# Lakonik/MVEdit

Hardware: AMD Instinct MI355X
Metric: multi-view denoise-steps/sec (32 views, 512^2) (higher is better)
Workload: dtype f16; 1 GPU; 32-view 512x512 get_noise_pred: 64 SD-1.5 UNet forwards (64x64 latents, ctx 77x768) + CFG per step; ControlNet residuals zero; views=32, latent=64, cfg=True, parallelism=views/1

## Files before the change

include/mvedit_amd.h:

```cpp
#ifndef MVEDIT_AMD_H
#define MVEDIT_AMD_H

#include <stdint.h>
#include <stddef.h>

#ifdef __cplusplus
extern "C" {
#endif

#define MVE_API __attribute__((visibility("default")))

typedef enum {
    MVE_OK = 0,
    MVE_ERR_ARG = -1,
    MVE_ERR_HIP = -2,
    MVE_ERR_STATE = -3,
    MVE_ERR_NOMEM = -4
} mve_status;

typedef enum {
    MVE_F32 = 0,
    MVE_F16 = 1,
    MVE_BF16 = 2,
    MVE_I32 = 3,
// ... 238 lines not shown
                             const void* d_ctx, int B, int H, int W, int ctx_len, int num_cross_attn_imgs,
                             const void* const* down_residuals, const void* d_mid_residual, int residuals_nhwc,
                             void* d_out, void* d_workspace, size_t workspace_bytes, float* op_ms, void* stream);
MVE_API int mve_controlnet_create(void** handle, int dtype, int in_channels, int conditioning_channels, int n_levels,
                                  const int* block_out_channels, int layers_per_block, const int* down_attn, const int* num_heads,
                                  const int* transformer_layers, int cross_attention_dim, int norm_num_groups, float norm_eps,
                                  int use_linear_projection);
MVE_API int mve_controlnet_set_cond_repeat(void* handle, int repeat);
MVE_API int mve_controlnet_forward(void* handle, const void* d_sample, int io_dtype, const float* d_timesteps, const void* d_ctx,
                                   const void* d_cond, int B, int H, int W, int ctx_len, float conditioning_scale, int accumulate,
                                   void* const* d_outputs, void* d_workspace, size_t workspace_bytes,
                                   float* op_ms , void* stream);

MVE_API int mve_vae_create(void** handle, int dtype, int half, int in_channels, int out_channels, int n_levels,
                           const int* block_out_channels, int layers_per_block, int norm_num_groups, float norm_eps);
MVE_API int mve_vae_plan(void* handle, int B, int H, int W, int io_dtype, size_t* workspace_bytes, int* n_ops, double* flops);
MVE_API int mve_vae_forward(void* handle, const void* d_in, int io_dtype, int B, int H, int W, void* d_out, void* d_workspace,
                            size_t workspace_bytes, float* op_ms, void* stream);

MVE_API int mve_srvgg_create(void** handle, int dtype, int num_in_ch, int num_out_ch, int num_feat, int num_conv, int upscale);
MVE_API int mve_srvgg_plan(void* handle, int B, int H, int W, int io_dtype, size_t* workspace_bytes, int* n_ops, double* flops);
MVE_API int mve_srvgg_forward(void* handle, const void* d_in, int io_dtype, int B, int H, int W, void* d_out, void* d_workspace,
                              size_t workspace_bytes, float* op_ms, void* stream);
MVE_API int mve_lpips_create(void** handle, int dtype, int normalize_inputs);
MVE_API int mve_lpips_plan(void* handle, int B, int H, int W, int io_dtype, size_t* workspace_bytes, int* n_ops, int* n_forward_ops,
                           double* flops);
MVE_API int mve_lpips_forward(void* handle, const void* d_pred, const void* d_target, int io_dtype, int B, int H, int W, float* d_loss,
                              void* d_workspace, size_t workspace_bytes, void* stream);
MVE_API int mve_lpips_backward(void* handle, const float* d_grad_loss, int io_dtype, int B, int H, int W, void* d_grad_pred,
                               void* d_workspace, size_t workspace_bytes, void* stream);
MVE_API int mve_lpips_scale(int dtype, int io_dtype, const void* d_pred, const void* d_target, int B, int H, int W, const float* d_shift3,
                            const float* d_scale3, int normalize, void* d_out, void* stream);
MVE_API int mve_lpips_input_grad(int dtype, int io_dtype, const void* d_g8, int B, int H, int W, const float* d_scale3, int normalize,
                                 void* d_out, void* stream);
MVE_API int mve_maxpool2x2(int dtype, const void* d_x, int B, int H, int W, int C, void* d_y, void* stream);
MVE_API int mve_maxpool2x2_backward(int dtype, const void* d_x, const void* d_grad_y, int B, int H, int W, int C, void* d_grad_x,
                                    void* stream);
MVE_API int mve_relu_backward(int dtype, void* d_grad, const void* d_out, size_t n, void* stream);
MVE_API size_t mve_lpips_layer_scratch_bytes(int B, int HW);
MVE_API int mve_lpips_layer(int dtype, const void* d_feat, const float* d_lin_w, int B, int HW, int C, int accumulate, float* d_loss,
                            void* d_scratch, void* stream);
MVE_API int mve_lpips_layer_backward(int dtype, const void* d_feat, const float* d_lin_w, const float* d_grad_loss, int B, int HW, int C,
                                     void* d_grad_feat, void* stream);
MVE_API int mve_prelu(int dtype, const void* d_x, const float* d_slope, int C, void* d_y, size_t n, void* stream);
MVE_API int mve_pixel_shuffle_add(int io_dtype, const float* d_src, int ld, const void* d_base, int B, int C, int H, int W, int r,
                                  void* d_out, void* stream);

MVE_API int mve_unet_tune(int fuse_shortcut);
MVE_API int mve_unet_graph(void* handle, int enable);

MVE_API int mve_unet_set_attention(void* handle, int ip_tokens, float ip_scale, int ref_mode, int ref_H, int ref_W, int ref_skip,
                                   void* d_ref_store, size_t ref_store_bytes);
MVE_API int mve_unet_set_residual_mode(void* handle, int pair);
MVE_API int mve_unet_set_addition_embed(void* handle, int addition_type, int addition_time_embed_dim, int projection_input_dim);
MVE_API int mve_unet_bind_added_cond(void* handle, const void* d_text_embeds, int text_dtype, int text_dim, const float* d_time_ids, int n_ids,
                                     int B);
MVE_API size_t mve_unet_ref_store_bytes(void* handle, int B, int ref_H, int ref_W, int ref_skip);

MVE_API int mve_unet_op_info(void* handle, int i, int* cls, double* flops, char* label, int label_len);


MVE_API int mve_hashgrid_mlp_decode(const float* d_xyz, uint32_t M, const float* d_table, int n_levels,
                                    const float* level_scale, const uint32_t* level_res, const uint32_t* level_offset,
                                    const uint32_t* level_size, const float* d_w1, const float* d_b1, const float* d_w2,
                                    const float* d_b2, int hidden, float bound, float blob_density, float blob_radius,
                                    float sigmoid_saturation, float* d_sigmas, float* d_rgbs, void* stream);

MVE_API size_t mve_hashgrid_mlp_backward_workspace_bytes(uint32_t M, int n_levels);
MVE_API int mve_hashgrid_mlp_backward(const float* d_xyz, uint32_t M, const float* d_table, int n_levels, const float* level_scale,
                                      const uint32_t* level_res, const uint32_t* level_offset, const uint32_t* level_size,
                                      const float* d_w1, const float* d_b1, const float* d_w2, const float* d_b2, int hidden, float bound,
                                      float blob_density, float blob_radius, float sigmoid_saturation, const float* d_grad_sigma,
                                      const float* d_grad_rgb, float* d_grad_table, float* d_grad_w1, float* d_grad_b1,
                                      float* d_grad_w2, float* d_grad_b2, void* d_workspace, size_t workspace_bytes, void* stream);
MVE_API int mve_adam_step(float* d_param, const float* d_grad, float* d_exp_avg, float* d_exp_avg_sq, size_t n, float lr, float beta1,
                          float beta2, float eps, int step, void* stream);

MVE_API int mve_nerf_render_rays(const float* d_rays_o, const float* d_rays_d, uint32_t N, const uint8_t* d_bitfield,
                                 uint32_t grid_size, const float* d_aabb, float bound, float min_near, float dt_gamma,
                                 uint32_t max_steps, float T_thresh, const float* d_table, int n_levels,
                                 const float* level_scale, const uint32_t* level_res, const uint32_t* level_offset,
                                 const uint32_t* level_size, const float* d_w1, const float* d_b1, const float* d_w2,
                                 const float* d_b2, int hidden, float blob_density, float blob_radius,
                                 float sigmoid_saturation, float* d_weights_sum, float* d_depth, float* d_image,
                                 int32_t* d_n_samples, void* stream);

MVE_API int mve_camera_rays(const float* d_intrinsics, const float* d_poses, int n_views, int h, int w, float* d_rays_o,
                            float* d_rays_d, float* d_dir_norm, void* stream);

MVE_API int mve_depth_to_normal(const float* d_depth, const float* d_alpha, int alpha_stride, const float* d_intrinsics,
                                int n_views, int h, int w, const float* normal_bg3, float* d_normal_fg, float* d_normal,
                                void* stream);

MVE_API int mve_normalize_depth(const float* d_depths, const float* d_alphas, int n_views, int hw, float far_depth,
                                float alpha_clip, float eps, float* d_out, void* stream);

#define MVE_INTERP_LINEAR 0
#define MVE_INTERP_SMOOTHSTEP 1
MVE_API int mve_hashgrid_encode(const float* d_x, uint32_t N, const float* d_table, uint32_t n_rows, int n_features, int n_levels,
                                const float* level_scale, const uint32_t* level_res, const uint32_t* level_offset,
                                const uint32_t* level_size, int interpolation, float* d_out, void* stream);
MVE_API int mve_hashgrid_encode_backward(const float* d_x, uint32_t N, const float* d_table, uint32_t n_rows, int n_features,
                                         int n_levels, const float* level_scale, const uint32_t* level_res,
                                         const uint32_t* level_offset, const uint32_t* level_size, int interpolation,
                                         const float* d_grad_enc, float* d_grad_table, float* d_grad_x, void* stream);

// ... 146 lines not shown
```

mvedit_amd/csrc/attention.hip:

```cpp
#include "common.h"

#include <stdlib.h>
#include <type_traits>

namespace {

constexpr int NT = 256;

struct AttnParams {
    const void* Q; const void* K; const void* V; const void* K2; const void* V2; void* O;
    int ldq, ldk, ldv, ldk2, ldv2, ldo;
    int B, Lq, Lk, Lk2, heads;
    float scale_log2e;
    int prescaled;
};

template <int DP, bool KSW2> __device__ __forceinline__ int k_perm(int row, int pc) {
    if constexpr (DP == 64) return pc ^ ((row >> 1) & 7);
    else if constexpr (KSW2) return pc ^ (((row >> 3) & 1) << 1);
    else return pc ^ ((row >> 2) & 3);
}
template <int DP, bool KSW2> __device__ __forceinline__ int k_swz(int row, int chunk) {
    return row * (DP * 2) + (k_perm<DP, KSW2>(row, chunk) << 4);
}

typedef __attribute__((address_space(3))) void* lds_ptr_t;
typedef const __attribute__((address_space(1))) void* gbl_ptr_t;
typedef float f32x8 __attribute__((ext_vector_type(8)));

__device__ __attribute__((aligned(16))) unsigned int g_attn_zero_page[4] = {0u, 0u, 0u, 0u};

template <int KB2, bool VSW2> __device__ __forceinline__ int v_swz2(int row, int chunk) {
    if constexpr (KB2 == 128) return row * 256 + ((chunk ^ (row & 15) ^ (VSW2 ? (row >> 3) & 7 : 0)) << 4);
    else return row * 128 + ((chunk ^ ((row >> 1) & 7) ^ (VSW2 ? (row >> 4) & 7 : 0)) << 4);
}

template <class Tag, int D, bool SEG2, int QF = 2, int KB2X = 0, int OCC = 0, bool KSW2 = false, bool VSW2 = false>
__global__ __launch_bounds__(NT, (OCC ? OCC : (D > 80 ? 1 : 2))) void k_attention2(const AttnParams p) {
    constexpr int QB = 64 * QF;
    constexpr int DP = (D + 31) / 32 * 32;
    constexpr int KS = DP / 32;
    constexpr int DC = D / 8;
    constexpr int DVF = (D + 15) / 16;
    constexpr int KB2 = KB2X ? KB2X : (D > 64 ? 64 : 128);
    constexpr int NH = KB2 / 64;
    constexpr int CPR = DP / 8;
    constexpr int KROW = DP * 2;
    constexpr int VROW = KB2 * 2;
    constexpr int K_BYTES = KB2 * KROW;
    constexpr int V_BYTES = DVF * 16 * VROW;
    constexpr int K_INSTR = K_BYTES / 1024 / 4;
    static_assert((K_BYTES / 1024) % 4 == 0, "K tile must split evenly over 4 waves");
    constexpr int V_TASKS = (KB2 / 2) * DC;
    constexpr int V_PER_T = (V_TASKS + NT - 1) / NT;
    constexpr bool ONES = (D % 16) != 0;
    constexpr int L_G = (D % 16) / 4, L_R = (D % 16) % 4;
    typedef typename Tag::V8 V8;
    typedef typename Tag::T T;

    __shared__ __attribute__((aligned(16))) unsigned char smem[2 * K_BYTES + 2 * V_BYTES];
    unsigned char* Kbuf = smem;
    unsigned char* Vbuf = smem + 2 * K_BYTES;

    const int tid = threadIdx.x, lane = tid & 63, wid = tid >> 6;
    const int g = lane >> 4, l16 = lane & 15;

    const int q_tiles = (p.Lq + QB - 1) / QB;
    const unsigned nblk = (unsigned)(q_tiles * p.heads * p.B);
    const unsigned bid = mve_xcd_remap(blockIdx.x, nblk);
    const int qt = bid % q_tiles;
    const int h = (bid / q_tiles) % p.heads;
    const int b = bid / (q_tiles * p.heads);
    const int Ltot = p.Lk + p.Lk2;

    const T* Qp = reinterpret_cast<const T*>(p.Q);
    const T* zero = reinterpret_cast<const T*>(g_attn_zero_page);
    const T* kb1 = reinterpret_cast<const T*>(p.K) + (size_t)b * p.Lk * p.ldk + h * D;
    const T* vb1 = reinterpret_cast<const T*>(p.V) + (size_t)b * p.Lk * p.ldv + h * D;
    const T* kb2 = SEG2 ? reinterpret_cast<const T*>(p.K2) + (size_t)b * p.Lk2 * p.ldk2 + h * D : nullptr;
    const T* vb2 = SEG2 ? reinterpret_cast<const T*>(p.V2) + (size_t)b * p.Lk2 * p.ldv2 + h * D : nullptr;
    auto k_row = [&](int j) -> const T* {
        if constexpr (SEG2) { if (j >= p.Lk) return kb2 + (size_t)(j - p.Lk) * p.ldk2; }
        return kb1 + (size_t)j * p.ldk;
    };
    auto v_row = [&](int j) -> const T* {
        if constexpr (SEG2) { if (j >= p.Lk) return vb2 + (size_t)(j - p.Lk) * p.ldv2; }
        return vb1 + (size_t)j * p.ldv;
    };

    for (int i = tid; i < 2 * V_BYTES / 16; i += NT) reinterpret_cast<u32x4*>(Vbuf)[i] = u32x4{0u, 0u, 0u, 0u};
    __syncthreads();
    if constexpr (ONES) {
        const unsigned short one = __builtin_bit_cast(unsigned short, Tag::from_f32(1.0f));
        const unsigned two = (unsigned)one | ((unsigned)one << 16);
        for (int i = tid; i < 2 * (VROW / 4); i += NT) {
            const int buf = i / (VROW / 4), wofs = i - buf * (VROW / 4);
            *reinterpret_cast<unsigned*>(Vbuf + buf * V_BYTES + D * VROW + wofs * 4) = two;
        }
    }

    V8 qf[QF][KS];
    const int q_base = qt * QB + wid * (16 * QF);
#pragma unroll
    for (int f = 0; f < QF; ++f) {
        int q = q_base + f * 16 + l16;
        q = q < p.Lq ? q : p.Lq - 1;
        const T* row = Qp + ((size_t)b * p.Lq + q) * p.ldq + h * D;
#pragma unroll
        for (int ks = 0; ks < KS; ++ks) {
            const int c = ks * 4 + g;
            u32x4 v = {0u, 0u, 0u, 0u};
            if (c < DC) v = *reinterpret_cast<const u32x4*>(row + c * 8);
            qf[f][ks] = __builtin_bit_cast(V8, v);
        }
    }

    int kd_row[K_INSTR], kd_col[K_INSTR];
#pragma unroll
    for (int i = 0; i < K_INSTR; ++i) {
        const int pos = (wid * K_INSTR + i) * 64 + lane;
        const int row = pos / CPR, pc = pos - row * CPR;
        const int c = k_perm<DP, KSW2>(row, pc);
        kd_row[i] = row;
        kd_col[i] = c < DC ? c * 8 : -1;
    }
// ... 202 lines not shown
        if (q < p.Lq) {
            T* orow = reinterpret_cast<T*>(p.O) + ((size_t)b * p.Lq + q) * p.ldo + h * D;
#pragma unroll
            for (int i = 0; i < DVF; ++i) {
                const int dv = i * 16 + g * 4;
                if (dv < D) {
                    T4 pk;
#pragma unroll
                    for (int r = 0; r < 4; ++r) pk[r] = Tag::from_f32(oacc[i][f][r] * inv);
                    *reinterpret_cast<T4*>(orow + dv) = pk;
                }
            }
        }
    }
}

__device__ __attribute__((aligned(16))) unsigned short g_attn_ones_f16[8] = {0x3C00u, 0, 0, 0, 0, 0, 0, 0};
__device__ __attribute__((aligned(16))) unsigned short g_attn_ones_bf16[8] = {0x3F80u, 0, 0, 0, 0, 0, 0, 0};

__device__ unsigned long long g_attn_prof[4] = {0ull, 0ull, 0ull, 0ull};

typedef short s16x4 __attribute__((ext_vector_type(4)));
typedef short s16x8 __attribute__((ext_vector_type(8)));
typedef float f32x2 __attribute__((ext_vector_type(2)));

__device__ __forceinline__ void attn_dma16(const void* gsrc, unsigned lds_dst) {
    unsigned keep;
    asm volatile("s_mov_b32 %0, m0\n\ts_mov_b32 m0, %2\n\ts_nop 0\n\tglobal_load_lds_dwordx4 %1, off\n\ts_mov_b32 m0, %0"
                 : "=&s"(keep) : "v"(gsrc), "s"(lds_dst) : "memory");
}

template <class Tag, bool SEG2, int NW, int NST, int WPS, bool PRE, bool PIPE, int ABL = 0>
__global__ __launch_bounds__(64 * NW, WPS) void k_attention3(const AttnParams p) {
    constexpr int D = 40, KB = 64, QB = 32 * NW;
    constexpr int K_ROW = 80, V_ROW = 96;
    constexpr int K_BYTES = KB * K_ROW, V_BYTES = KB * V_ROW, STAGE = K_BYTES + V_BYTES;
    constexpr int N_DMA = STAGE / 1024, K_DMA = K_BYTES / 1024, DMA_PER_WAVE = (N_DMA + NW - 1) / NW;
    static_assert(STAGE % 1024 == 0 && K_BYTES % 1024 == 0, "stage must split into whole LDS-DMA instructions");
    static_assert(NST >= 2 && NST <= 4, "2 to 4 LDS stages");
    typedef typename Tag::V8 V8;
    typedef typename Tag::T T;
    typedef T T2 __attribute__((ext_vector_type(2)));
    typedef T T4 __attribute__((ext_vector_type(4)));

    __shared__ __attribute__((aligned(16))) unsigned char smem[NST * STAGE];

    const int tid = threadIdx.x, lane = tid & 63, wid = tid >> 6;
    const int l32 = lane & 31, hi = lane >> 5, l16 = lane & 15, g = lane >> 4;
    unsigned long long prof_t0 = 0, prof_r0 = 0;
    if constexpr ((ABL & 1024) != 0) asm volatile("s_memtime %0\n\ts_memrealtime %1\n\ts_waitcnt lgkmcnt(0)" : "=s"(prof_t0), "=s"(prof_r0) :: "memory");

    const int q_tiles = (p.Lq + QB - 1) / QB;
    const unsigned nblk = (unsigned)(q_tiles * p.heads * p.B);
    const unsigned bid = mve_xcd_remap(blockIdx.x, nblk);
    const int qt = bid % q_tiles;
    const int h = (bid / q_tiles) % p.heads;
    const int b = bid / (q_tiles * p.heads);
    const int Ltot = p.Lk + p.Lk2;

    const T* kb1 = reinterpret_cast<const T*>(p.K) + (size_t)b * p.Lk * p.ldk + h * D;
    const T* vb1 = reinterpret_cast<const T*>(p.V) + (size_t)b * p.Lk * p.ldv + h * D;
    const T* kb2 = SEG2 ? reinterpret_cast<const T*>(p.K2) + (size_t)b * p.Lk2 * p.ldk2 + h * D : nullptr;
    const T* vb2 = SEG2 ? reinterpret_cast<const T*>(p.V2) + (size_t)b * p.Lk2 * p.ldv2 + h * D : nullptr;
    const T* ones = reinterpret_cast<const T*>(std::is_same<T, f16>::value ? g_attn_ones_f16 : g_attn_ones_bf16);
    auto k_row = [&](int j) -> const T* {
        if constexpr (SEG2) { if (j >= p.Lk) return kb2 + (size_t)(j - p.Lk) * p.ldk2; }
        return kb1 + (size_t)j * p.ldk;
    };
    auto v_row = [&](int j) -> const T* {
        if constexpr (SEG2) { if (j >= p.Lk) return vb2 + (size_t)(j - p.Lk) * p.ldv2; }
        return vb1 + (size_t)j * p.ldv;
    };

    const int q_base = qt * QB + wid * 32;
    V8 qf[3];
    {
        int q = q_base + l32;
        q = q < p.Lq ? q : p.Lq - 1;
        const T* row = reinterpret_cast<const T*>(p.Q) + ((size_t)b * p.Lq + q) * p.ldq + h * D;
        qf[0] = __builtin_bit_cast(V8, *reinterpret_cast<const u32x4*>(row + 8 * hi));
        qf[1] = __builtin_bit_cast(V8, *reinterpret_cast<const u32x4*>(row + 16 + 8 * hi));
        u32x4 t = {0u, 0u, 0u, 0u};
        if (hi == 0) t = *reinterpret_cast<const u32x4*>(row + 32);
        qf[2] = __builtin_bit_cast(V8, t);
    }

    const int wv = __builtin_amdgcn_readfirstlane(wid);
    const unsigned smem_base = (unsigned)(uintptr_t)(lds_ptr_t)smem;
    int d_key[DMA_PER_WAVE], d_col[DMA_PER_WAVE];
    const T* d_src[DMA_PER_WAVE];
    int d_ld[DMA_PER_WAVE];
#pragma unroll
    for (int i = 0; i < DMA_PER_WAVE; ++i) {
        const int inst = wv + NW * i;
        const int o = inst * 1024 + lane * 16;
        if (inst < K_DMA) {
            const int c = o >> 4;
            d_key[i] = c / 5; d_col[i] = (c - d_key[i] * 5) * 8;
            d_ld[i] = p.ldk;
            d_src[i] = kb1 + (size_t)d_key[i] * p.ldk + d_col[i];
        } else {
            const int c = (o - K_BYTES) >> 4;
            const int r = c / 6, col = c - r * 6;
            d_key[i] = (r & ~12) | ((r & 4) << 1) | ((r & 8) >> 1);
            d_col[i] = col < 5 ? col * 8 : -1;
            d_ld[i] = col < 5 ? p.ldv : 0;
            d_src[i] = col < 5 ? vb1 + (size_t)d_key[i] * p.ldv + d_col[i] : ones;
        }
    }
    auto dma_fast = [&](int stage_off) {
// ... 368 lines not shown

template <class Tag>
int dispatch_d(const AttnParams& p, int d, hipStream_t s) {
    switch (d) {
        case 40: return launch<Tag, 40>(p, s);
        case 64: return launch<Tag, 64>(p, s);
        case 80: return launch<Tag, 80>(p, s);
        case 160: return launch<Tag, 160>(p, s);
        default:
            mve_set_error("attention: unsupported head dim %d (supported: 40, 64, 80, 160)", d);
            return MVE_ERR_ARG;
    }
}

}

extern "C" int mve_attention_profile(unsigned long long* out4) {
    MVE_CHECK(out4, MVE_ERR_ARG, "attention_profile: null pointer");
#ifndef MVE_ATTN_LAB
    mve_set_error("attention_profile: the timing-only ablation kernels are compiled into development builds only (MVE_ATTN_LAB=1 python -m mvedit_amd.build)");
    return MVE_ERR_STATE;
#endif
    MVE_HIP(hipDeviceSynchronize());
    MVE_HIP(hipMemcpyFromSymbol(out4, HIP_SYMBOL(g_attn_prof), 4 * sizeof(unsigned long long)));
    const unsigned long long z[4] = {0ull, 0ull, 0ull, 0ull};
    MVE_HIP(hipMemcpyToSymbol(HIP_SYMBOL(g_attn_prof), z, sizeof(z)));
    return MVE_OK;
}

extern "C" int mve_attention_tune(int variant) {
    const int old = g_attn_variant | (g_attn_ablate << 8);
#ifndef MVE_ATTN_LAB
    if (variant >= 256) { mve_set_error("attention_tune: ablation bits (8-19) need a development build (MVE_ATTN_LAB=1)"); return MVE_ERR_ARG; }
#endif
    if (variant >= 0) { g_attn_variant = variant & 255; g_attn_ablate = (variant >> 8) & 4095; }
    return old;
}

static int attention_entry(int dtype, const void* Q, int ldq, const void* K, int ldk, const void* V, int ldv,
                           const void* K2, int ldk2, const void* V2, int ldv2, void* O, int ldo, int B, int Lq,
                           int Lk, int Lk2, int heads, int head_dim, float scale, int prescaled, void* stream) {
    if (B == 0 || Lq == 0) return MVE_OK;
    MVE_CHECK(Q && K && V && O, MVE_ERR_ARG, "attention: null pointer");
    MVE_CHECK(Lk > 0 && Lk2 >= 0 && heads > 0, MVE_ERR_ARG, "attention: bad sizes Lk=%d Lk2=%d heads=%d", Lk, Lk2, heads);
    MVE_CHECK(Lk2 == 0 || (K2 && V2), MVE_ERR_ARG, "attention: second KV segment has null pointers");
    MVE_CHECK(ldq % 8 == 0 && ldk % 8 == 0 && ldv % 8 == 0 && ldo % 4 == 0 && (Lk2 == 0 || (ldk2 % 8 == 0 && ldv2 % 8 == 0)),
              MVE_ERR_ARG, "attention: leading dimensions must be multiples of 8");
    AttnParams p;
    p.Q = Q; p.K = K; p.V = V; p.K2 = K2; p.V2 = V2; p.O = O;
    p.ldq = ldq; p.ldk = ldk; p.ldv = ldv; p.ldk2 = ldk2; p.ldv2 = ldv2; p.ldo = ldo;
    p.B = B; p.Lq = Lq; p.Lk = Lk; p.Lk2 = Lk2; p.heads = heads;
    p.scale_log2e = prescaled ? 1.0f : scale * 1.4426950408889634f;
    p.prescaled = prescaled;
    if (dtype == MVE_F16) return dispatch_d<F16Tag>(p, head_dim, (hipStream_t)stream);
    if (dtype == MVE_BF16) return dispatch_d<BF16Tag>(p, head_dim, (hipStream_t)stream);
    mve_set_error("attention: unsupported dtype %d", dtype);
    return MVE_ERR_ARG;
}

extern "C" int mve_attention(int dtype, const void* Q, int ldq, const void* K, int ldk, const void* V, int ldv,
                             const void* K2, int ldk2, const void* V2, int ldv2, void* O, int ldo, int B, int Lq,
                             int Lk, int Lk2, int heads, int head_dim, float scale, void* stream) {
    return attention_entry(dtype, Q, ldq, K, ldk, V, ldv, K2, ldk2, V2, ldv2, O, ldo, B, Lq, Lk, Lk2, heads, head_dim, scale, 0, stream);
}

extern "C" int mve_attention_prescaled(int dtype, const void* Q, int ldq, const void* K, int ldk, const void* V, int ldv,
                                       const void* K2, int ldk2, const void* V2, int ldv2, void* O, int ldo, int B, int Lq,
                                       int Lk, int Lk2, int heads, int head_dim, void* stream) {
    return attention_entry(dtype, Q, ldq, K, ldk, V, ldv, K2, ldk2, V2, ldv2, O, ldo, B, Lq, Lk, Lk2, heads, head_dim, 1.0f, 1, stream);
}
```

mvedit_amd/csrc/builder_unet.h:

```cpp
#pragma once
#include "executor_builder.h"

namespace {

int Builder::build(int B_, int H, int W, int n_img, int has_res, int io_dtype, int res_nhwc) {
    B = B_; dt = c.dtype;
    const int Bb = B_;
    { const AttnOpts keep = pl.ao; pl = Plan(); pl.ao = keep; }
    pl.B = Bb; pl.H = H; pl.W = W; pl.n_img = n_img; pl.has_res = has_res; pl.io_dtype = io_dtype; pl.res_nhwc = res_nhwc;
    pl.add_type = c.add_type;
    const int e = 2, n = c.n_levels, L = c.layers_per_block, T = c.temb_dim();
    const int d = dt;
    ld_temb = u.sum_temb; ld_kv = u.sum_kv;
    MVE_CHECK(Bb % n_img == 0, MVE_ERR_ARG, "unet: batch %d not divisible by num_cross_attn_imgs %d", Bb, n_img);
    MVE_CHECK((H % (1 << (n - 1))) == 0 && (W % (1 << (n - 1))) == 0, MVE_ERR_ARG,
              "unet: latent size %dx%d must be divisible by %d", H, W, 1 << (n - 1));
    for (int i = 0; i < n; ++i) {
        const int hd = c.ch[i] / c.heads[i];
        MVE_CHECK(!c.attn[i] || hd == 40 || hd == 64 || hd == 80 || hd == 160, MVE_ERR_ARG, "unet: unsupported head dim %d", hd);
    }
    const int M0 = Bb * H * W;
    Ref x_in = ws((size_t)M0 * 8 * e);
    {
        Ref src; src.kind = Ref::SAMPLE;
// ... 82 lines not shown
    if (ao.ref_mode) {
        MVE_CHECK(n_img == 1, MVE_ERR_ARG, "unet: reference attention and cross-image attention are exclusive (adapter3d_mixin.py:194)");
        MVE_CHECK(ao.ref_skip >= 0 && ao.ref_skip < Bb, MVE_ERR_ARG, "unet: ref_skip %d out of range", ao.ref_skip);
        if (ao.ref_mode == 2)
            MVE_CHECK(ao.ref_H > 0 && ao.ref_W > 0 && ao.ref_H % (1 << (n - 1)) == 0 && ao.ref_W % (1 << (n - 1)) == 0, MVE_ERR_ARG,
                      "unet: bad reference latent size %dx%d", ao.ref_H, ao.ref_W);
    }
    ctxkv = ws((size_t)ctxB * Lt * ld_kv * e);
    gemm(ctx_in, c.ctx_dim, wt("ctx_kv.w"), c.ctx_dim, ctxkv, ld_kv, ctxB * Lt, ld_kv, c.ctx_dim, Ref(), Ref(), 0, 0, Ref(), 0, 0,
         "cross-attention K,V (all layers, one GEMM)");
    struct Skip { Ref r; int C, H, W; };
    std::vector<Skip> skips;
    Ref x = ws_stream((size_t)M0 * c.ch[0] * e);
    if (c.controlnet) {
        const int Hc = 8 * H, Wc = 8 * W, cc = c.cond_ch;
        const int R = pl.ao.cn_cond_repeat > 1 ? pl.ao.cn_cond_repeat : 1;
        MVE_CHECK(Bb % R == 0, MVE_ERR_ARG, "controlnet: batch %d is not a multiple of the conditioning repeat %d", Bb, R);
        MVE_CHECK(R == 1 || !pl.ao.residual_pair, MVE_ERR_ARG, "controlnet: shared conditioning images are not combined with the residual-pair mode");
        const int Bc = Bb / R;
        Ref cimg = ws((size_t)Bc * Hc * Wc * 8 * e);
        {
            Ref src; src.kind = Ref::CNCOND;
            op(OC_OTHER, 0, "cond nchw->nhwc", [=](const Run& r) { return mve_nchw_to_nhwc(d, io_dtype, r.p(src), Bc, cc, Hc, Wc, 8, r.p(cimg), r.stream); });
        }
        const std::string en = "controlnet_cond_embedding.";
        int hc = Hc, wc = Wc, ci = 8;
        Ref cur = cimg;
        auto emb_conv = [&](const std::string& nm, int co, int stride, bool act) {
            const int ho = (hc - 1) / stride + 1, wo = (wc - 1) / stride + 1;
            Ref y = ws((size_t)Bc * ho * wo * co * e);
            conv(cur, ci, Bc, hc, wc, stride, 0, wt(nm + ".w"), co, y, wt(nm + ".b"), Ref(), 0, Ref(), 0, "cond_embedding.conv");
            rel(cur);
            if (act) {
                const size_t nel = (size_t)Bc * ho * wo * co;
                op(OC_OTHER, 0, "silu", [=](const Run& r) { return mve_silu(d, r.p(y), r.p(y), nel, r.stream); });
            }
            cur = y; hc = ho; wc = wo; ci = co;
        };
        emb_conv(en + "conv_in", CN_EMB[0], 1, true);
        for (int k = 0; k < 6; ++k) emb_conv(en + "blocks." + std::to_string(k), CN_EMB[(k + 1) / 2], (k & 1) ? 2 : 1, true);
        emb_conv(en + "conv_out", c.ch[0], 1, false);
        MVE_CHECK(hc == H && wc == W, MVE_ERR_ARG, "controlnet: conditioning image must be 8x the latent size");
        for (int rep = 0; rep < R; ++rep) {
            Ref xi = x_in, xo = x;
            xi.off += (size_t)rep * Bc * H * W * 8 * e;
            xo.off += (size_t)rep * Bc * H * W * c.ch[0] * e;
            conv(xi, 8, Bc, H, W, 1, 0, wt("conv_in.w"), c.ch[0], xo, wt("conv_in.b"), Ref(), 0, cur, 0, "conv_in + cond_embedding");
        }
        rel(cur);
    } else {
        conv(x_in, 8, Bb, H, W, 1, 0, wt("conv_in.w"), c.ch[0], x, wt("conv_in.b"), Ref(), 0, Ref(), 0, "conv_in");
    }
    rel(x_in);
    skips.push_back({x, c.ch[0], H, W});
    int h = H, w = W, cin = c.ch[0];
    for (int i = 0; i < n; ++i) {
        for (int j = 0; j < L; ++j) {
            const std::string rn = "down_blocks." + std::to_string(i) + ".resnets." + std::to_string(j);
            Ref y = resnet(rn, x, cin, Ref(), 0, c.ch[i], h, w);
            cin = c.ch[i];
            if (c.attn[i]) {
                Ref z = transformer("down_blocks." + std::to_string(i) + ".attentions." + std::to_string(j), y, cin, c.heads[i], c.tlayers[i], h, w);
                rel(y);
                y = z;
            }
            x = y;
            skips.push_back({x, cin, h, w});
        }
        if (i + 1 < n) {
            const std::string dn = "down_blocks." + std::to_string(i) + ".downsamplers.0.conv";
            Ref y = ws_stream((size_t)Bb * (h / 2) * (w / 2) * cin * e);
            conv(x, cin, Bb, h, w, 2, 0, wt(dn + ".w"), cin, y, wt(dn + ".b"), Ref(), 0, Ref(), 0, "downsample");
            h /= 2; w /= 2;
            x = y;
            skips.push_back({x, cin, h, w});
        }
    }
    pl.enc_end = pl.ops.size();
    if (c.controlnet) {
        const int C = c.ch[n - 1];
        for (size_t i = 0; i < skips.size(); ++i)
            zero_conv(skips[i].r, skips[i].C, Bb * skips[i].H * skips[i].W, skips[i].H * skips[i].W, "controlnet_down_blocks." + std::to_string(i), (int)i);
        Ref y = resnet("mid_block.resnets.0", x, C, Ref(), 0, C, h, w);
        Ref z = transformer("mid_block.attentions.0", y, C, c.heads[n - 1], c.tlayers[n - 1], h, w);
        rel(y);
        Ref m = resnet("mid_block.resnets.1", z, C, Ref(), 0, C, h, w);
        rel(z);
        zero_conv(m, C, Bb * h * w, h * w, "controlnet_mid_block", (int)skips.size());
        pl.ws_bytes = ar.peak + 256;
        pl.ref_store_bytes = ref_off;
        if (!u.err.empty()) { mve_set_error("controlnet plan: %s", u.err.c_str()); u.err.clear(); return MVE_ERR_STATE; }
        return MVE_OK;
    }
    if (has_res) {
        for (size_t i = 0; i < skips.size(); ++i) {
            Skip& sk = skips[i];
            const size_t elems = (size_t)Bb * sk.H * sk.W * sk.C;
            Ref src; src.kind = Ref::DOWNRES; src.idx = (int)i;
            Ref sum = ws_stream(elems * e);
            Ref a = sk.r;
            const Ref a_lo = lo(a), sum_lo = lo(sum);
            const int C = sk.C, sh = sk.H, sw = sk.W;
            if (res_nhwc) {
                op(OC_OTHER, 0, "skip += controlnet residual", [=](const Run& r) { return mve_axpy_pair(d, r.p(a), r.p(a_lo), r.p(src), 1.0f, r.p(sum), r.p(sum_lo), elems, r.stream); });
            } else {
                Ref tmp = ws(elems * e);
                op(OC_OTHER, 0, "residual nchw->nhwc", [=](const Run& r) { return mve_nchw_to_nhwc(d, io_dtype, r.p(src), Bb, C, sh, sw, C, r.p(tmp), r.stream); });
                op(OC_OTHER, 0, "skip += controlnet residual", [=](const Run& r) { return mve_axpy_pair(d, r.p(a), r.p(a_lo), r.p(tmp), 1.0f, r.p(sum), r.p(sum_lo), elems, r.stream); });
                rel(tmp);
            }
            sk.r = sum;
        }
    }
    {
        const int C = c.ch[n - 1];
        Ref y = resnet("mid_block.resnets.0", x, C, Ref(), 0, C, h, w);
        Ref z = transformer("mid_block.attentions.0", y, C, c.heads[n - 1], c.tlayers[n - 1], h, w);
        rel(y);
        Ref m = resnet("mid_block.resnets.1", z, C, Ref(), 0, C, h, w);
        rel(z);
        x = m;
        if (has_res) {
            const size_t elems = (size_t)Bb * h * w * C;
            Ref src; src.kind = Ref::MIDRES;
            Ref sum = ws_stream(elems * e);
            const Ref m_lo = lo(m), sum_lo = lo(sum);
            const int hh = h, ww = w;
            if (res_nhwc) {
                op(OC_OTHER, 0, "mid += controlnet residual", [=](const Run& r) { return mve_axpy_pair(d, r.p(m), r.p(m_lo), r.p(src), 1.0f, r.p(sum), r.p(sum_lo), elems, r.stream); });
            } else {
                Ref tmp = ws(elems * e);
                op(OC_OTHER, 0, "residual nchw->nhwc", [=](const Run& r) { return mve_nchw_to_nhwc(d, io_dtype, r.p(src), Bb, C, hh, ww, C, r.p(tmp), r.stream); });
                op(OC_OTHER, 0, "mid += controlnet residual", [=](const Run& r) { return mve_axpy_pair(d, r.p(m), r.p(m_lo), r.p(tmp), 1.0f, r.p(sum), r.p(sum_lo), elems, r.stream); });
                rel(tmp);
            }
            rel(m);
            x = sum;
        }
    }
    int cur = c.ch[n - 1];
    for (int i = 0; i < n; ++i) {
        const int lvl = n - 1 - i, cout = c.ch[lvl];
        for (int j = 0; j < L + 1; ++j) {
            Skip sk = skips.back();
            skips.pop_back();
            const std::string rn = "up_blocks." + std::to_string(i) + ".resnets." + std::to_string(j);
            Ref y = resnet(rn, x, cur, sk.r, sk.C, cout, h, w);
            rel(x);
            if (has_res) rel(sk.r);
            cur = cout;
            if (c.attn[lvl]) {
                Ref z = transformer("up_blocks." + std::to_string(i) + ".attentions." + std::to_string(j), y, cout, c.heads[lvl], c.tlayers[lvl], h, w);
                rel(y);
                y = z;
            }
            x = y;
        }
        if (i + 1 < n) {
            const std::string un = "up_blocks." + std::to_string(i) + ".upsamplers.0.conv";
            Ref y = ws_stream((size_t)Bb * (2 * h) * (2 * w) * cout * e);
            upsample_conv(x, cout, Bb, h, w, un, y);
            rel(x);
            h *= 2; w *= 2;
            x = y;
        }
    }
    Ref hn = ws((size_t)M0 * c.ch[0] * e);
    gn(x, c.ch[0], Ref(), 0, Bb, H * W, c.eps, wt("norm_out.g"), wt("norm_out.b"), 1, hn, "conv_norm_out+silu");
    rel(x);
    Ref o8 = ws((size_t)M0 * 8 * 4);
    conv(hn, c.ch[0], Bb, H, W, 1, 0, wt("conv_out.w"), 8, o8, wt("conv_out.b"), Ref(), 0, Ref(), MVE_GEMM_OUT_F32, "conv_out");
    rel(hn);
    {
        Ref dst; dst.kind = Ref::OUT;
        const int oc = c.out_ch;
        op(OC_OTHER, 0, "nhwc->nchw", [=](const Run& r) { return mve_nhwc_to_nchw(io_dtype, MVE_F32, r.p(o8), 8, Bb, oc, H, W, r.p(dst), r.stream); });
    }
    pl.ws_bytes = ar.peak + 256;
    pl.ref_store_bytes = ref_off;
    if (!u.err.empty()) { mve_set_error("unet plan: %s", u.err.c_str()); u.err.clear(); return MVE_ERR_STATE; }
    return MVE_OK;
}

}
```

mvedit_amd/csrc/common.h:

```cpp
#pragma once
#include <hip/hip_runtime.h>
#include <hip/hip_fp16.h>
#include <hip/hip_bf16.h>
#include <stdint.h>
#include <stdio.h>
#include <stdarg.h>
#include <string.h>

#include "../../include/mvedit_amd.h"

void mve_set_error(const char* fmt, ...);

#define MVE_CHECK(cond, code, ...)                                     \
    do {                                                               \
        if (!(cond)) {                                                 \
            mve_set_error(__VA_ARGS__);                                \
            return (code);                                             \
        }                                                              \
    } while (0)

#define MVE_HIP(expr)                                                  \
    do {                                                               \
        hipError_t _e = (expr);                                        \
        if (_e != hipSuccess) {                                        \
            mve_set_error("%s failed: %s (%s:%d)", #expr,              \
                          hipGetErrorString(_e), __FILE__, __LINE__);  \
            return MVE_ERR_HIP;                                        \
        }                                                              \
    } while (0)

#define MVE_LAUNCH_CHECK()                                             \
    do {                                                               \
        hipError_t _e = hipGetLastError();                             \
        if (_e != hipSuccess) {                                        \
            mve_set_error("kernel launch failed: %s (%s:%d)",          \
                          hipGetErrorString(_e), __FILE__, __LINE__);  \
            return MVE_ERR_HIP;                                        \
        }                                                              \
    } while (0)

static inline unsigned mve_cdiv(unsigned long long a, unsigned long long b) {
    return (unsigned)((a + b - 1) / b);
}

typedef _Float16 f16;
typedef __bf16 bf16;

typedef f16 f16x8 __attribute__((ext_vector_type(8)));
typedef f16 f16x4 __attribute__((ext_vector_type(4)));
typedef bf16 bf16x8 __attribute__((ext_vector_type(8)));
typedef bf16 bf16x4 __attribute__((ext_vector_type(4)));
typedef float f32x4 __attribute__((ext_vector_type(4)));
typedef float f32x16 __attribute__((ext_vector_type(16)));
typedef unsigned short u16;
typedef u16 u16x8 __attribute__((ext_vector_type(8)));
typedef u16 u16x4 __attribute__((ext_vector_type(4)));
typedef unsigned int u32x4 __attribute__((ext_vector_type(4)));
typedef unsigned int u32x2 __attribute__((ext_vector_type(2)));

struct F16Tag {
    typedef f16 T;
    typedef f16x8 V8;
    static constexpr int dtype = MVE_F16;
    static __device__ __forceinline__ float to_f32(T v) { return (float)v; }
    static __device__ __forceinline__ T from_f32(float v) { return (T)v; }
    static __device__ __forceinline__ f32x4 mfma16(V8 a, V8 b, f32x4 c) {
        return __builtin_amdgcn_mfma_f32_16x16x32_f16(a, b, c, 0, 0, 0);
    }
    static __device__ __forceinline__ f32x16 mfma32(V8 a, V8 b, f32x16 c) {
        return __builtin_amdgcn_mfma_f32_32x32x16_f16(a, b, c, 0, 0, 0);
    }
};

struct BF16Tag {
    typedef bf16 T;
    typedef bf16x8 V8;
    static constexpr int dtype = MVE_BF16;
    static __device__ __forceinline__ float to_f32(T v) { return (float)v; }
    static __device__ __forceinline__ T from_f32(float v) { return (T)v; }
    static __device__ __forceinline__ f32x4 mfma16(V8 a, V8 b, f32x4 c) {
        return __builtin_amdgcn_mfma_f32_16x16x32_bf16(a, b, c, 0, 0, 0);
    }
    static __device__ __forceinline__ f32x16 mfma32(V8 a, V8 b, f32x16 c) {
        return __builtin_amdgcn_mfma_f32_32x32x16_bf16(a, b, c, 0, 0, 0);
    }
};

__device__ __forceinline__ float mve_lo8_scaled(float r) {
    const float s = __builtin_amdgcn_fmed3f(r * 256.f, -57344.f, 57344.f);
    return s == s ? s : 0.f;
}
template <bool CLAMP = false>
// ... 2 lines not shown
    if constexpr (CLAMP) {
        p = __builtin_amdgcn_cvt_pk_bf8_f32(mve_lo8_scaled(a), mve_lo8_scaled(b), 0, false);
        p = __builtin_amdgcn_cvt_pk_bf8_f32(mve_lo8_scaled(c), mve_lo8_scaled(d), p, true);
    } else {
        p = __builtin_amdgcn_cvt_pk_bf8_f32(a * 256.f, b * 256.f, 0, false);
        p = __builtin_amdgcn_cvt_pk_bf8_f32(c * 256.f, d * 256.f, p, true);
    }
    return (unsigned)p;
}
__device__ __forceinline__ void mve_lo8_unpack4(unsigned p, float (&o)[4]) {
    const auto a = __builtin_amdgcn_cvt_pk_f32_bf8((int)p, false), b = __builtin_amdgcn_cvt_pk_f32_bf8((int)p, true);
    o[0] = a[0] * 0.00390625f; o[1] = a[1] * 0.00390625f; o[2] = b[0] * 0.00390625f; o[3] = b[1] * 0.00390625f;
}
template <class Tag>
__device__ __forceinline__ void mve_pair_load8(const typename Tag::V8& h, u32x2 l, float (&v)[8]) {
    float a[4], b[4];
    mve_lo8_unpack4(l[0], a);
    mve_lo8_unpack4(l[1], b);
#pragma unroll
    for (int e = 0; e < 4; ++e) { v[e] = Tag::to_f32(h[e]) + a[e]; v[4 + e] = Tag::to_f32(h[4 + e]) + b[e]; }
}
template <class Tag>
__device__ __forceinline__ u32x2 mve_pair_split8(const float (&v)[8], typename Tag::V8& hi) {
#pragma clang fp contract(off)
    float r[8];
#pragma unroll
    for (int e = 0; e < 8; ++e) { hi[e] = Tag::from_f32(v[e]); r[e] = v[e] - Tag::to_f32(hi[e]); }
    constexpr bool CL = Tag::dtype == MVE_BF16;
    return u32x2{mve_lo8_pack4<CL>(r[0], r[1], r[2], r[3]), mve_lo8_pack4<CL>(r[4], r[5], r[6], r[7])};
}

#define MVE_DISPATCH_16(dtype, FN, ...)                                \
    ((dtype) == MVE_F16 ? FN<F16Tag>(__VA_ARGS__)                      \
     : (dtype) == MVE_BF16 ? FN<BF16Tag>(__VA_ARGS__)                  \
                           : (mve_set_error("unsupported dtype %d", (int)(dtype)), MVE_ERR_ARG))

__device__ __forceinline__ float mve_max_xor16(float x) {
    const auto r = __builtin_amdgcn_permlane16_swap(__float_as_uint(x), __float_as_uint(x), false, false);
    return fmaxf(__uint_as_float(r[0]), __uint_as_float(r[1]));
}
__device__ __forceinline__ float mve_max_xor32(float x) {
    const auto r = __builtin_amdgcn_permlane32_swap(__float_as_uint(x), __float_as_uint(x), false, false);
    return fmaxf(__uint_as_float(r[0]), __uint_as_float(r[1]));
}

__device__ __forceinline__ unsigned mve_xcd_remap(unsigned bid, unsigned nblk) {
    const unsigned nx = 8u;
    if (nblk < nx * 2u) return bid;
    const unsigned q = nblk / nx, r = nblk % nx;
    const unsigned xcd = bid % nx, k = bid / nx;
    const unsigned base = (xcd < r) ? xcd * (q + 1u) : r * (q + 1u) + (xcd - r) * q;
    return base + k;
}
```

mvedit_amd/csrc/common.hip:

```cpp
#include "common.h"

static thread_local char g_err[1024] = "";

void mve_set_error(const char* fmt, ...) {
    va_list ap;
    va_start(ap, fmt);
    vsnprintf(g_err, sizeof(g_err), fmt, ap);
    va_end(ap);
}

extern "C" {

const char* mve_last_error(void) { return g_err; }

int mve_version(void) { return 1; }

int mve_device_info(int* n_cu, int* wave_size, char* arch, int arch_len) {
    int dev = 0;
    MVE_HIP(hipGetDevice(&dev));
    hipDeviceProp_t prop;
    MVE_HIP(hipGetDeviceProperties(&prop, dev));
    if (n_cu) *n_cu = prop.multiProcessorCount;
    if (wave_size) *wave_size = prop.warpSize;
    if (arch && arch_len > 0) {
        strncpy(arch, prop.gcnArchName, (size_t)arch_len - 1);
        arch[arch_len - 1] = 0;
    }
    return MVE_OK;
}

}
```

mvedit_amd/csrc/executor.h:

```cpp
#pragma once
#include "common.h"

#include <functional>
#include <map>
#include <memory>
#include <string>
#include <vector>

extern "C" {
int mve_gemm(int, const void*, int, const void*, int, void*, int, int, int, int, const float*, const float*, int, int,
             const void*, int, int, float, void*, size_t, int, void*);
int mve_gemm_pair(int, const void*, int, const void*, int, void*, int, int, int, int, const float*, const float*, int, int,
                  const void*, int, int, float, void*, size_t, int, const void*, void*, void*);
int mve_gemm_pair_ln(int, const void*, int, const void*, int, void*, int, int, int, int, const float*, const void*, int, void*, size_t, int,
                     const void*, void*, void*, int, const float*, const float*, float, void*);
int mve_conv3x3_pair(int, const void*, int, const void*, int, int, int, int, int, int, const void*, int, void*, int,
                     const float*, const float*, int, const void*, int, int, float, void*, size_t, const void*, void*, void*);
int mve_conv3x3_shortcut_pair(int, const void*, int, const void*, int, const void*, int, int, int, int, const void*, int, void*, int,
                              const float*, const float*, int, float, void*, size_t, void*, void*);
int mve_groupnorm_silu_pair(int, const void*, int, const void*, int, int, int, int, float, const float*, const float*, int, void*,
                            void*, const void*, const void*, void*);
int mve_layernorm_pair(int, const void*, int, void*, int, int, int, const float*, const float*, float, const void*, void*);
int mve_axpy_pair(int, const void*, const void*, const void*, float, void*, void*, size_t, void*);
int mve_conv3x3(int, const void*, int, const void*, int, int, int, int, int, int, const void*, int, void*, int,
// ... 104 lines not shown
};

enum OpClass { OC_CONV = 0, OC_LINEAR = 1, OC_ATTN = 2, OC_NORM = 3, OC_OTHER = 4, OC_COUNT = 5 };

struct Ref {
    enum Kind { NUL, WS, WT, SAMPLE, TIMESTEPS, CTX, OUT, DOWNRES, MIDRES, REFSTORE, CNCOND, CNOUT } kind = NUL;
    size_t off = 0;
    int idx = 0;
};

struct Run {
    unsigned char* ws; unsigned char* wt;
    const void* sample; const float* timesteps; const void* ctx; void* out;
    const void* const* down_res; const void* mid_res;
    unsigned char* ref_store;
    const void* cn_cond = nullptr;
    void* const* cn_out = nullptr;
    float cn_scale = 1.0f;
    int cn_accum = 0;
    const void* add_text = nullptr;
    const float* add_ids = nullptr;
    int add_text_dtype = 0, add_text_dim = 0, add_n_ids = 0;
    hipStream_t stream;
    void* p(const Ref& r) const {
        switch (r.kind) {
            case Ref::WS: return ws + r.off;
            case Ref::WT: return wt + r.off;
            case Ref::SAMPLE: return (void*)((const unsigned char*)sample + r.off);
            case Ref::TIMESTEPS: return (void*)timesteps;
            case Ref::CTX: return (void*)((const unsigned char*)ctx + r.off);
            case Ref::OUT: return out;
            case Ref::DOWNRES: return (void*)down_res[r.idx];
            case Ref::MIDRES: return (void*)mid_res;
            case Ref::REFSTORE: return ref_store + r.off;
            case Ref::CNCOND: return (void*)cn_cond;
            case Ref::CNOUT: return cn_out[r.idx];
            default: return nullptr;
        }
    }
};

struct Op {
    int cls;
    double flops;
    const char* what;
    std::function<int(const Run&)> fn;
};

struct AttnOpts {
    int ip_tokens = 0; float ip_scale = 1.0f;
    int ref_mode = 0, ref_H = 0, ref_W = 0, ref_skip = 0;
    int residual_pair = 0;
    int cn_cond_repeat = 1;
    bool operator==(const AttnOpts& o) const {
        return ip_tokens == o.ip_tokens && ip_scale == o.ip_scale && ref_mode == o.ref_mode && ref_H == o.ref_H && ref_W == o.ref_W &&
               ref_skip == o.ref_skip && residual_pair == o.residual_pair && cn_cond_repeat == o.cn_cond_repeat;
    }
};

struct Plan {
    int B = 0, H = 0, W = 0, n_img = 1, has_res = 0, io_dtype = 0, res_nhwc = 0, ctx_len = 0;
    int add_type = 0;
    AttnOpts ao;
    size_t ref_store_bytes = 0;
    unsigned long long last_use = 0;
    unsigned long long uid = 0;
    std::vector<Op> ops;
    size_t enc_end = 0;
    size_t ws_bytes = 0;
    double flops[OC_COUNT] = {0, 0, 0, 0, 0};
};

struct Arena {
    struct Blk { size_t off, size; bool free; };
    std::vector<Blk> b;
    size_t top = 0, peak = 0;
    size_t alloc(size_t bytes) {
        bytes = (bytes + 255) & ~(size_t)255;
        for (size_t i = 0; i < b.size(); ++i)
            if (b[i].free && b[i].size >= bytes) {
                if (b[i].size > bytes) {
                    Blk rest{b[i].off + bytes, b[i].size - bytes, true};
                    b[i].size = bytes;
                    b.insert(b.begin() + i + 1, rest);
                }
                b[i].free = false;
                return b[i].off;
            }
        if (!b.empty() && b.back().free) {
            top += bytes - b.back().size;
            b.back().size = bytes;
            b.back().free = false;
            peak = top > peak ? top : peak;
            return b.back().off;
        }
        b.push_back({top, bytes, false});
        top += bytes;
        peak = top > peak ? top : peak;
        return b.back().off;
    }
    void release(size_t off) {
        for (size_t i = 0; i < b.size(); ++i)
            if (b[i].off == off && !b[i].free) {
                b[i].free = true;
                if (i + 1 < b.size() && b[i + 1].free) { b[i].size += b[i + 1].size; b.erase(b.begin() + i + 1); }
                if (i > 0 && b[i - 1].free) { b[i - 1].size += b[i].size; b.erase(b.begin() + i); }
                return;
            }
    }
};

struct Unet {
    Config cfg;
    std::map<std::string, Param> params;
    std::map<std::string, bool> loaded;
    std::vector<std::string> expected;
    unsigned char* slab = nullptr;
    size_t slab_bytes = 0;
    int sum_temb = 0, sum_kv = 0;
    std::map<std::string, int> temb_off, kv_off;
    std::vector<std::unique_ptr<Plan>> plans;
    Plan* cur = nullptr;
    unsigned long long tick = 0;
    AttnOpts ao;
    unsigned char* ref_store = nullptr;
    size_t ref_store_bytes = 0;
    int n_ip_loaded = 0, n_xf_layers = 0;
    bool fuse_sc = false;
    std::map<std::string, int> sc_cin;
    std::string err;
    struct AddedCond { const void* text = nullptr; const float* ids = nullptr; int text_dtype = 0, text_dim = 0, n_ids = 0, B = 0; } added;
    struct GraphEntry {
        unsigned long long plan_uid = 0;
        int phase = 0, seen = 0;
        std::vector<const void*> ptrs;
        hipGraph_t graph = nullptr;
        hipGraphExec_t exec = nullptr;
        unsigned long long last_use = 0;
    };
    bool graph_mode = false;
    std::vector<GraphEntry> graphs;
    unsigned long long plan_counter = 0;
};

int esz(int dtype) { return dtype == MVE_F32 ? 4 : 2; }

constexpr int VGG_IDX[13] = {0, 2, 5, 7, 10, 12, 14, 17, 19, 21, 24, 26, 28};
constexpr int VGG_CIN[13] = {3, 64, 64, 128, 128, 256, 256, 256, 512, 512, 512, 512, 512};
constexpr int VGG_COUT[13] = {64, 64, 128, 128, 256, 256, 256, 512, 512, 512, 512, 512, 512};
constexpr int VGG_SLICE[13] = {1, 1, 2, 2, 3, 3, 3, 4, 4, 4, 5, 5, 5};
constexpr int VGG_BLK_FIRST[6] = {0, 2, 4, 7, 10, 13};
std::string vgg_name(int i) { return "net.slice" + std::to_string(VGG_SLICE[i]) + "." + std::to_string(VGG_IDX[i]); }

struct ResnetDesc { std::string name; int cin, cout; };
struct XfDesc { std::string name; int c, heads, layers; };

void enumerate(const Config& c, std::vector<ResnetDesc>& rs, std::vector<XfDesc>& xs) {
    const int n = c.n_levels, L = c.layers_per_block;
    if (c.sr || c.lpips) return;
    if (c.vae) {
        const int Cm = c.ch[n - 1];
        if (c.vae == 2) {
            int cin = c.ch[0];
            for (int i = 0; i < n; ++i) {
                for (int j = 0; j < L; ++j)
                    rs.push_back({"down_blocks." + std::to_string(i) + ".resnets." + std::to_string(j), j == 0 ? cin : c.ch[i], c.ch[i]});
                cin = c.ch[i];
            }
        }
        rs.push_back({"mid_block.resnets.0", Cm, Cm});
        rs.push_back({"mid_block.resnets.1", Cm, Cm});
        if (c.vae == 1) {
            int cin = Cm;
            for (int i = 0; i < n; ++i) {
                const int cout = c.ch[n - 1 - i];
                for (int j = 0; j < L + 1; ++j)
                    rs.push_back({"up_blocks." + std::to_string(i) + ".resnets." + std::to_string(j), j == 0 ? cin : cout, cout});
                cin = cout;
            }
        }
        return;
    }
    int cin = c.ch[0];
    for (int i = 0; i < n; ++i) {
        for (int j = 0; j < L; ++j) {
            rs.push_back({"down_blocks." + std::to_string(i) + ".resnets." + std::to_string(j), j == 0 ? cin : c.ch[i], c.ch[i]});
            if (c.attn[i]) xs.push_back({"down_blocks." + std::to_string(i) + ".attentions." + std::to_string(j), c.ch[i], c.heads[i], c.tlayers[i]});
        }
        cin = c.ch[i];
    }
    rs.push_back({"mid_block.resnets.0", c.ch[n - 1], c.ch[n - 1]});
    xs.push_back({"mid_block.attentions.0", c.ch[n - 1], c.heads[n - 1], c.tlayers[n - 1]});
// ... 18 lines not shown
```

mvedit_amd/csrc/executor_builder.h:

```cpp
#pragma once
#include "executor_params.h"

namespace {

struct Builder {
    Unet& u;
    Plan& pl;
    Arena ar;
    const Config& c;
    int B, dt;
    int ld_temb, ld_kv;
    Ref tproj, ctxkv, ipkv;
    int ctx_rows_per_img = 0, ctxB = 0;
    int Lt = 0;
    int H0 = 0;
    size_t ref_off = 0;

    Builder(Unet& u_, Plan& p) : u(u_), pl(p), c(u_.cfg) {}

    Ref ws(size_t bytes) { Ref r; r.kind = Ref::WS; r.off = ar.alloc(bytes); return r; }
    std::map<size_t, Ref> lo_of;
    Ref ws_stream(size_t bytes) {
        Ref r = ws(bytes);
        if (pl.ao.residual_pair) lo_of[r.off] = ws(bytes / 2);
        return r;
    }
    Ref lo(const Ref& r) const {
        if (r.kind != Ref::WS) return Ref();
        auto it = lo_of.find(r.off);
        return it == lo_of.end() ? Ref() : it->second;
    }
    void rel(const Ref& r) {
        if (r.kind != Ref::WS) return;
        auto it = lo_of.find(r.off);
        if (it != lo_of.end()) { ar.release(it->second.off); lo_of.erase(it); }
        ar.release(r.off);
    }
    Ref wt(const std::string& n, size_t elem_off = 0) {
        auto it = u.params.find(n);
        Ref r;
        if (it == u.params.end()) { u.err = "missing packed parameter " + n; return r; }
        r.kind = Ref::WT;
        r.off = it->second.off + elem_off * (it->second.f32 ? 4 : 2);
        return r;
    }
    static Ref at(Ref r, size_t bytes) { r.off += bytes; return r; }
    void live(const Ref& r, const char* what) {
        if (r.kind != Ref::WS) return;
        for (auto& blk : ar.b)
            if (!blk.free && r.off >= blk.off && r.off < blk.off + blk.size) return;
        if (u.err.empty()) u.err = std::string("operand used after release in ") + what;
    }
    void op(int cls, double flops, const char* what, std::function<int(const Run&)> fn) {
        pl.ops.push_back({cls, flops, what, std::move(fn)});
        pl.flops[cls] += flops;
    }

    int rows_img = 0;
    void gemm(Ref A, int lda, Ref W, int ldw, Ref out, int ldc, int M, int N, int K, Ref bias, Ref rowvec, int ldrv,
              int rpv, Ref res, int ldr, int flags, const char* what, float out_scale = 1.0f) {
        const int rimg = rows_img;
        const int d = dt;
        live(A, what); live(out, what); live(res, what); live(rowvec, what);
        const size_t skb = mve_gemm_workspace_bytes(M, N, K, rimg);
        Ref sk = skb ? ws(skb) : Ref();
        const Ref res_lo = lo(res), out_lo = lo(out);
        op(OC_LINEAR, 2.0 * M * N * K, what, [=](const Run& r) {
            return mve_gemm_pair(d, r.p(A), lda, r.p(W), ldw, r.p(out), ldc, M, N, K, (const float*)r.p(bias), (const float*)r.p(rowvec),
                                 ldrv, rpv, r.p(res), ldr, flags, out_scale, r.p(sk), skb, rimg, r.p(res_lo), r.p(out_lo), r.stream);
        });
        rel(sk);
    }
    void gemm_ln(Ref A, int lda, Ref W, int ldw, Ref out, int ldc, int M, int N, int K, Ref bias, Ref res, int ldr, Ref ln_out, Ref ln_g, Ref ln_b,
                 const char* what) {
        const int rimg = rows_img;
        const int d = dt;
        live(A, what); live(out, what); live(res, what); live(ln_out, what);
        const size_t skb = mve_gemm_workspace_bytes(M, N, K, rimg);
        Ref sk = skb ? ws(skb) : Ref();
        const Ref res_lo = lo(res), out_lo = lo(out);
        op(OC_LINEAR, 2.0 * M * N * K, what, [=](const Run& r) {
            return mve_gemm_pair_ln(d, r.p(A), lda, r.p(W), ldw, r.p(out), ldc, M, N, K, (const float*)r.p(bias), r.p(res), ldr, r.p(sk), skb, rimg,
                                    r.p(res_lo), r.p(out_lo), r.p(ln_out), N, (const float*)r.p(ln_g), (const float*)r.p(ln_b), 1e-5f, r.stream);
        });
        rel(sk);
    }
    void conv(Ref x, int C1, int Bn, int H, int W, int stride, int ups, Ref Wt, int Cout, Ref out, Ref bias, Ref rowvec,
              int ldrv, Ref res, int flags, const char* what) {
        const int d = dt;
        const int Hv = ups ? 2 * H : H, Wv = ups ? 2 * W : W;
        const int Ho = (Hv - 1) / stride + 1, Wo = (Wv - 1) / stride + 1;
        live(x, what); live(out, what); live(res, what); live(rowvec, what);
        const int fl = flags | (C1 % 64 == 0 ? MVE_CONV_W_CHUNK64 : 0);
        const size_t skb = mve_gemm_workspace_bytes(Bn * Ho * Wo, Cout, 9 * C1, Ho * Wo);
        Ref sk = skb ? ws(skb) : Ref();
        const Ref res_lo = lo(res), out_lo = (flags & MVE_GEMM_OUT_F32) ? Ref() : lo(out);
        op(OC_CONV, 2.0 * Bn * Ho * Wo * (double)Cout * 9 * C1, what, [=](const Run& r) {
            return mve_conv3x3_pair(d, r.p(x), C1, nullptr, 0, Bn, H, W, stride, ups, r.p(Wt), Cout, r.p(out), Cout,
                                    (const float*)r.p(bias), (const float*)r.p(rowvec), ldrv, r.p(res), Cout, fl, 1.0f, r.p(sk), skb, r.p(res_lo),
                                    r.p(out_lo), r.stream);
        });
        rel(sk);
    }
    static bool upsample_phases_on() {
        static int on = -1;
        if (on < 0) { const char* e = getenv("MVE_UPSAMPLE_PHASES"); on = e ? (atoi(e) != 0) : 1; }
        return on != 0;
    }
// ... 134 lines not shown
            gemm_ln(n0, C, wt(name + ".proj_in.w"), C, h, C, M, C, C, wt(name + ".proj_in.b"), Ref(), 0, n1_first, wt(b0 + ".norm1.g"), wt(b0 + ".norm1.b"),
                    "transformer.proj_in+norm1");
        } else {
            gemm(n0, C, wt(name + ".proj_in.w"), C, h, C, M, C, C, wt(name + ".proj_in.b"), Ref(), 0, 0, Ref(), 0, 0, "transformer.proj_in");
        }
        rel(n0);
        for (int k = 0; k < layers; ++k) {
            const std::string b = name + ".transformer_blocks." + std::to_string(k);
            Ref n1;
            if (fuse_ln && k == 0) n1 = n1_first;
            else {
                n1 = ws((size_t)M * C * e);
                ln(h, n1, M, C, wt(b + ".norm1.g"), wt(b + ".norm1.b"));
            }
            Ref qkv = ws((size_t)M * 3 * C * e);
            gemm(n1, C, wt(b + ".qkv.w"), C, qkv, 3 * C, M, 3 * C, C, Ref(), Ref(), 0, 0, Ref(), 0, 0, "attn1.qkv");
            rel(n1);
            Ref a = ws((size_t)M * C * e);
            const AttnOpts& ao = pl.ao;
            if (ao.ref_mode == 0) {
                attn(prescaled(qkv, b + ".qkv.w", hd), 3 * C, at(qkv, (size_t)C * e), 3 * C, at(qkv, (size_t)2 * C * e), 3 * C, a, C, nb, L, L, heads, hd);
            } else {
                const int div = H0 / H;
                const int Lref = ao.ref_mode == 1 ? L : (ao.ref_H / div) * (ao.ref_W / div);
                const int skip = ao.ref_skip, nr = nb - skip;
                Ref st; st.kind = Ref::REFSTORE; st.off = ref_off;
                ref_off += (size_t)nr * Lref * 2 * C * e;
                if (ao.ref_mode == 1) {
                    attn(prescaled(qkv, b + ".qkv.w", hd), 3 * C, at(qkv, (size_t)C * e), 3 * C, at(qkv, (size_t)2 * C * e), 3 * C, a, C, nb, L, L, heads, hd);
                    copy2d(st, (size_t)2 * C * e, at(qkv, ((size_t)skip * L * 3 * C + C) * e), (size_t)3 * C * e, (size_t)2 * C * e,
                           (size_t)nr * L, "reference K,V -> store");
                } else {
                    attn(prescaled(qkv, b + ".qkv.w", hd), 3 * C, at(qkv, (size_t)C * e), 3 * C, at(qkv, (size_t)2 * C * e), 3 * C, a, C, skip, L, L, heads, hd);
                    const size_t o = (size_t)skip * L * 3 * C * e;
                    attn(prescaled(at(qkv, o), b + ".qkv.w", hd), 3 * C, at(qkv, o + (size_t)C * e), 3 * C, at(qkv, o + (size_t)2 * C * e), 3 * C,
                         at(a, (size_t)skip * L * C * e), C, nr, L, L, heads, hd, st, 2 * C, at(st, (size_t)C * e), 2 * C, Lref,
                         "attention (+reference tokens)");
                }
            }
            rel(qkv);
            Ref h2 = ws_stream((size_t)M * C * e);
            Ref n2 = ws((size_t)M * C * e);
            if (fuse_ln) {
                gemm_ln(a, C, wt(b + ".o1.w"), C, h2, C, M, C, C, wt(b + ".o1.b"), h, C, n2, wt(b + ".norm2.g"), wt(b + ".norm2.b"), "attn1.to_out+residual+norm2");
                rel(a); rel(h); h = h2;
            } else {
                gemm(a, C, wt(b + ".o1.w"), C, h2, C, M, C, C, wt(b + ".o1.b"), Ref(), 0, 0, h, C, 0, "attn1.to_out+residual");
                rel(a); rel(h); h = h2;
                ln(h, n2, M, C, wt(b + ".norm2.g"), wt(b + ".norm2.b"));
            }
            Ref q = ws((size_t)M * C * e);
            gemm(n2, C, wt(b + ".q2.w"), C, q, C, M, C, C, Ref(), Ref(), 0, 0, Ref(), 0, 0, "attn2.to_q");
            rel(n2);
            Ref a2 = ws((size_t)M * C * e);
            const size_t ko = (size_t)u.kv_off[b] * e;
            attn(prescaled(q, b + ".q2.w", hd), C, at(ctxkv, ko), ld_kv, at(ctxkv, ko + (size_t)C * e), ld_kv, a2, C, nb, L, Lt, heads, hd);
            if (ao.ip_tokens > 0) {
                Ref aip = ws((size_t)M * C * e);
                attn(prescaled(q, b + ".q2.w", hd), C, at(ipkv, ko), ld_kv, at(ipkv, ko + (size_t)C * e), ld_kv, aip, C, nb, L, ao.ip_tokens, heads, hd, Ref(), 0, Ref(), 0,
                     0, "attention (ip tokens)");
                const int d = dt;
                const float sc = ao.ip_scale;
                const size_t nel = (size_t)M * C;
                op(OC_OTHER, 0, "attn2 += scale * ip", [=](const Run& r) { return mve_axpy(d, r.p(a2), r.p(aip), sc, r.p(a2), nel, r.stream); });
                rel(aip);
            }
            rel(q);
            Ref h3 = ws_stream((size_t)M * C * e);
            Ref n3 = ws((size_t)M * C * e);
            if (fuse_ln) {
                gemm_ln(a2, C, wt(b + ".o2.w"), C, h3, C, M, C, C, wt(b + ".o2.b"), h, C, n3, wt(b + ".norm3.g"), wt(b + ".norm3.b"), "attn2.to_out+residual+norm3");
                rel(a2); rel(h); h = h3;
            } else {
                gemm(a2, C, wt(b + ".o2.w"), C, h3, C, M, C, C, wt(b + ".o2.b"), Ref(), 0, 0, h, C, 0, "attn2.to_out+residual");
                rel(a2); rel(h); h = h3;
                ln(h, n3, M, C, wt(b + ".norm3.g"), wt(b + ".norm3.b"));
            }
            Ref f = ws((size_t)M * 4 * C * e);
            gemm(n3, C, wt(b + ".ff1.w"), C, f, 4 * C, M, 8 * C, C, wt(b + ".ff1.b"), Ref(), 0, 0, Ref(), 0, MVE_GEMM_GEGLU, "ff.geglu");
            rel(n3);
            Ref h4 = ws_stream((size_t)M * C * e);
            gemm(f, 4 * C, wt(b + ".ff2.w"), 4 * C, h4, C, M, C, 4 * C, wt(b + ".ff2.b"), Ref(), 0, 0, h, C, 0, "ff.out+residual");
            rel(f); rel(h); h = h4;
        }
        Ref out = ws_stream((size_t)M * C * e);
        gemm(h, C, wt(name + ".proj_out.w"), C, out, C, M, C, C, wt(name + ".proj_out.b"), Ref(), 0, 0, x, C, 0, "transformer.proj_out+residual");
        rel(h);
        return out;
    }

    Ref vae_attention(const std::string& name, Ref x, int C, int H, int W);
    int build_lpips(int B_, int H, int W, int io_dtype);
    int build_sr(int B_, int H, int W, int io_dtype);
    int build_vae(int B_, int H, int W, int io_dtype);
    int build(int B_, int H, int W, int n_img, int has_res, int io_dtype, int res_nhwc);
};

}
```

mvedit_amd/csrc/gemm.hip:

```cpp
#include "common.h"

#include <stdlib.h>

#include <map>
#include <mutex>
#include <utility>

#include "gemm_shared.h"

namespace {

constexpr int BM = 128;

}
long long mve_gemm_big_blocks(int M, int N, int splitk);
int mve_gemm_big_launch(int dtype, int mode, const void* params, void* stream);
int mve_gemm_pp_launch(int dtype, int mode, const void* params, void* stream);
void mve_gemm_pp_old_swizzle(int on);
bool mve_gemm_pp_ln_fused();
int mve_gemm_pp_ln_fuse_tune(int on);
extern "C" int mve_layernorm_pair(int, const void*, int, void*, int, int, int, const float*, const float*, float, const void*, void*);
namespace {

template <class Tag, int BN, int MODE, int NST, int BM = 128>
__device__ __forceinline__ void gemm_body(const GemmParams& p, unsigned char* smem) {
    static_assert(BM == 128 || BM == 64, "tile rows");
    constexpr int WN = BN / 2;
    constexpr int NF = WN / 16;
    constexpr int WM = BM / 2;
    constexpr int MF = WM / 16;
    constexpr int ROWS_PER_PASS = NT / 8;
    constexpr int A_PASSES = BM / ROWS_PER_PASS;
    constexpr int B_PASSES = BN / ROWS_PER_PASS;
    constexpr int A_STAGE = BM * ROW_BYTES;
    constexpr int B_STAGE = BN * ROW_BYTES;
    constexpr int STAGE = A_STAGE + B_STAGE;
    constexpr int CS_LD = BN + 4;
    typedef typename Tag::V8 V8;
    typedef typename Tag::T T;

    const int tid = threadIdx.x, lane = tid & 63, wid = tid >> 6;
    const int wm = wid >> 1, wn = wid & 1;

    const int tiles_n = (p.N + BN - 1) / BN;
    const int tiles_m = (p.M + BM - 1) / BM;
    const int S = p.splitk > 1 ? p.splitk : 1;
    const unsigned lin = mve_xcd_remap(blockIdx.x, (unsigned)(tiles_m * tiles_n * S));
    int kslice, tm, tn;
    if (p.w_major) {
        tm = (int)(lin % (unsigned)tiles_m);
        const unsigned rest = lin / (unsigned)tiles_m;
        kslice = (int)(rest % (unsigned)S);
        tn = (int)(rest / (unsigned)S);
    } else {
        kslice = lin % S;
        const unsigned tile = lin / S;
        tm = tile / tiles_n; tn = tile % tiles_n;
    }
    const int m0 = tm * BM, n0 = tn * BN;

    const int lr = tid >> 3;
    const int lc = (tid & 7) ^ ((lr >> 1) & 7);
    const T* __restrict__ Wp = reinterpret_cast<const T*>(p.W);

    const T* a_row[A_PASSES];
    int cb[A_PASSES], cy[A_PASSES], cx[A_PASSES];
    if constexpr (MODE == 0) {
#pragma unroll
        for (int j = 0; j < A_PASSES; ++j) {
            int m = m0 + lr + j * ROWS_PER_PASS;
            m = m < p.M ? m : p.M - 1;
            a_row[j] = reinterpret_cast<const T*>(p.A) + (size_t)m * p.lda;
        }
    } else {
        const int hw = p.g.Ho * p.g.Wo;
#pragma unroll
        for (int j = 0; j < A_PASSES; ++j) {
            int m = m0 + lr + j * ROWS_PER_PASS;
            m = m < p.M ? m : p.M - 1;
            const int b = m / hw, r = m - b * hw;
            const int y = r / p.g.Wo;
            cb[j] = b;
            cy[j] = y * p.g.stride - p.g.pad;
            cx[j] = (r - y * p.g.Wo) * p.g.stride - p.g.pad_x;
        }
    }
    const T* w_row[B_PASSES];
#pragma unroll
    for (int j = 0; j < B_PASSES; ++j) {
        int n = n0 + lr + j * ROWS_PER_PASS;
        n = n < p.N ? n : p.N - 1;
        w_row[j] = Wp + (size_t)n * p.ldw;
    }

    const int nk_all = (p.K + BK - 1) / BK;
    const int kt_begin = (int)((long long)nk_all * kslice / S), kt_end = (int)((long long)nk_all * (kslice + 1) / S);
    const int Ctot = p.g.C1 + p.g.C2;
    int tap = 0, cin = 0;
    if constexpr (MODE == 1) {
        if (!p.g.chunk64) {
            const int k0 = kt_begin * BK + lc * 8;
            tap = k0 / Ctot;
            cin = k0 - tap * Ctot;
        }
    }
    const T* zero = reinterpret_cast<const T*>(g_zero_page);

    auto a_src = [&](int kt, int j, bool kin) -> const T* {
        if constexpr (MODE == 0) {
            return kin ? a_row[j] + kt * BK + lc * 8 : nullptr;
        } else {
            int t_ = tap, c_ = cin;
// ... 203 lines not shown
#pragma unroll
                for (int e = 0; e < 4; ++e) { v[e] = lo[e]; v[4 + e] = hi[e]; }
                if (p.splitk > 1 && p.sk_sync) {
                    const unsigned off = (unsigned)((((size_t)kslice * p.M + m) * p.N + n) * 4);
                    const __amdgpu_buffer_rsrc_t rs = __builtin_amdgcn_make_buffer_rsrc(p.partial, 0, (int)0xFFFFFFF0u, 0x00020000);
                    __builtin_amdgcn_raw_buffer_store_b128(u32x4{__float_as_uint(v[0]), __float_as_uint(v[1]), __float_as_uint(v[2]), __float_as_uint(v[3])}, rs, off, 0, 16);
                    __builtin_amdgcn_raw_buffer_store_b128(u32x4{__float_as_uint(v[4]), __float_as_uint(v[5]), __float_as_uint(v[6]), __float_as_uint(v[7])}, rs, off + 16, 0, 16);
                    continue;
                }
                if (p.splitk > 1) {
                    float* pp = p.partial + ((size_t)kslice * p.M + m) * p.N + n;
                    *reinterpret_cast<f32x4*>(pp) = f32x4{v[0], v[1], v[2], v[3]};
                    *reinterpret_cast<f32x4*>(pp + 4) = f32x4{v[4], v[5], v[6], v[7]};
                    continue;
                }
                gemm_epilogue_store<Tag>(p, m, n, v, res_in_acc);
            }
            __syncthreads();
        }
    }
    if (p.splitk > 1 && p.sk_sync) gemm_reduce_slices<Tag, BN, BM, NT>(p, (unsigned)(tm * tiles_n + tn), kslice, S, m0, n0, tid);
}

template <int BN, int NST, int BMT = BM>
constexpr int gemm_smem_bytes() {
    return (NST * (BMT + BN) * ROW_BYTES > 64 * (BN + 4) * 4) ? NST * (BMT + BN) * ROW_BYTES : 64 * (BN + 4) * 4;
}

template <class Tag, int BN, int MODE>
__global__ __launch_bounds__(NT, 2) void k_gemm(const GemmParams p) {
    __shared__ __attribute__((aligned(16))) unsigned char smem[gemm_smem_bytes<BN, 2>()];
    gemm_body<Tag, BN, MODE, 2>(p, smem);
}

template <class Tag, int BN, int MODE>
__global__ __launch_bounds__(NT, 2) void k_gemm64(const GemmParams p) {
    __shared__ __attribute__((aligned(16))) unsigned char smem[gemm_smem_bytes<BN, 2, 64>()];
    gemm_body<Tag, BN, MODE, 2, 64>(p, smem);
}

constexpr int DEEP_NST = 4;
template <class Tag, int BN, int MODE>
__global__ __launch_bounds__(NT, 1) void k_gemm_deep(const GemmParams p) {
    extern __shared__ __attribute__((aligned(16))) unsigned char dyn_smem[];
    gemm_body<Tag, BN, MODE, DEEP_NST>(p, dyn_smem);
}

template <class Tag>
__global__ __launch_bounds__(256) void k_splitk_reduce(const GemmParams p) {
    const size_t chunks_n = p.N / 8;
    const size_t i = (size_t)blockIdx.x * 256 + threadIdx.x;
    if (i >= (size_t)p.M * chunks_n) return;
    const int m = (int)(i / chunks_n), n = (int)(i - (size_t)m * chunks_n) * 8;
    float v[8] = {0.f, 0.f, 0.f, 0.f, 0.f, 0.f, 0.f, 0.f};
    for (int s = 0; s < p.splitk; ++s) {
        const float* pp = p.partial + ((size_t)s * p.M + m) * p.N + n;
        const f32x4 lo = *reinterpret_cast<const f32x4*>(pp), hi = *reinterpret_cast<const f32x4*>(pp + 4);
#pragma unroll
        for (int e = 0; e < 4; ++e) { v[e] += lo[e]; v[4 + e] += hi[e]; }
    }
    gemm_epilogue_store<Tag>(p, m, n, v);
}

template <class Tag>
int splitk_reduce_launch(const GemmParams& p, hipStream_t s) {
    if (p.splitk > 1 && !p.sk_sync) {
        k_splitk_reduce<Tag><<<mve_cdiv((size_t)p.M * (p.N / 8), 256), 256, 0, s>>>(p);
        MVE_LAUNCH_CHECK();
    }
    return MVE_OK;
}

int g_splitk_policy = -1;
int choose_splitk(int rows_per_image, int N, int K) {
    if (g_splitk_policy < 0) {
        const char* e = getenv("MVE_GEMM_SPLITK");
        g_splitk_policy = e ? atoi(e) : 1;
    }
    if (rows_per_image <= 0 || g_splitk_policy == 0) return 1;
    const int bn = (N % 160 == 0) ? 160 : (N % 128 == 0 ? 128 : (N <= 64 ? 64 : 128));
    const long long t1 = (long long)mve_cdiv(rows_per_image, BM) * mve_cdiv(N, bn);
    const int nk = (K + BK - 1) / BK;
    long long s = (64 + t1 - 1) / t1;
    if (s > nk / 8) s = nk / 8;
    if (s > 16) s = 16;
    return s < 2 ? 1 : (int)s;
}

int gemm_red_mode();
int* gemm_sk_sync(hipStream_t s);
constexpr int SK_SYNC_TILES = 8192;

int g_w_major = -1;
bool gemm_w_major_on() {
    if (g_w_major < 0) {
        const char* e = getenv("MVE_GEMM_WMAJOR");
        g_w_major = e ? atoi(e) : 1;
    }
    return g_w_major != 0;
}

int g_small_bn = -1, g_small_bn_max = -1;
int gemm_small_bn() {
    if (g_small_bn < 0) {
        const char* e = getenv("MVE_GEMM_SMALL_BN");
        g_small_bn = e ? atoi(e) : 64;
// ... 392 lines not shown
             float out_scale, void* workspace, size_t workspace_bytes, int rows_per_image, void* stream) {
    return mve_gemm_pair(dtype, A, lda, W, ldw, out, ldc, M, N, K, bias, rowvec, ldrv, rows_per_vec, residual, ldr, flags, out_scale, workspace,
                         workspace_bytes, rows_per_image, nullptr, nullptr, stream);
}

static int gemm_pair_impl(int dtype, const void* A, int lda, const void* W, int ldw, void* out, int ldc, int M, int N, int K,
                          const float* bias, const float* rowvec, int ldrv, int rows_per_vec, const void* residual, int ldr, int flags,
                          float out_scale, void* workspace, size_t workspace_bytes, int rows_per_image, const void* residual_lo, void* out_lo,
                          void* stream, void* ln_out, int ld_ln, const float* ln_gamma, const float* ln_beta, float ln_eps);

int mve_gemm_pair(int dtype, const void* A, int lda, const void* W, int ldw, void* out, int ldc, int M, int N, int K,
                  const float* bias, const float* rowvec, int ldrv, int rows_per_vec, const void* residual, int ldr, int flags,
                  float out_scale, void* workspace, size_t workspace_bytes, int rows_per_image, const void* residual_lo, void* out_lo,
                  void* stream) {
    return gemm_pair_impl(dtype, A, lda, W, ldw, out, ldc, M, N, K, bias, rowvec, ldrv, rows_per_vec, residual, ldr, flags, out_scale, workspace,
                          workspace_bytes, rows_per_image, residual_lo, out_lo, stream, nullptr, 0, nullptr, nullptr, 0.f);
}

int mve_gemm_pair_ln(int dtype, const void* A, int lda, const void* W, int ldw, void* out, int ldc, int M, int N, int K,
                     const float* bias, const void* residual, int ldr, void* workspace, size_t workspace_bytes, int rows_per_image,
                     const void* residual_lo, void* out_lo, void* ln_out, int ld_ln, const float* ln_gamma, const float* ln_beta, float ln_eps,
                     void* stream) {
    MVE_CHECK(ln_out && ln_gamma && ln_beta && ld_ln >= N && ld_ln % 8 == 0, MVE_ERR_ARG, "gemm_pair_ln: LayerNorm output / parameters missing or ld_ln (%d) bad", ld_ln);
    (void)mve_gemm_pp_ln_fused();
    const int rc = gemm_pair_impl(dtype, A, lda, W, ldw, out, ldc, M, N, K, bias, nullptr, 0, 0, residual, ldr, 0, 1.0f, workspace, workspace_bytes,
                                  rows_per_image, residual_lo, out_lo, stream, ln_out, ld_ln, ln_gamma, ln_beta, ln_eps);
    if (rc != MVE_OK || M == 0) return rc;
    if (mve_gemm_pp_ln_fused()) return MVE_OK;
    return mve_layernorm_pair(dtype, out, ldc, ln_out, ld_ln, M, N, ln_gamma, ln_beta, ln_eps, out_lo, stream);
}

int mve_gemm_ln_fuse_tune(int on) { return mve_gemm_pp_ln_fuse_tune(on); }

static int gemm_pair_impl(int dtype, const void* A, int lda, const void* W, int ldw, void* out, int ldc, int M, int N, int K,
                          const float* bias, const float* rowvec, int ldrv, int rows_per_vec, const void* residual, int ldr, int flags,
                          float out_scale, void* workspace, size_t workspace_bytes, int rows_per_image, const void* residual_lo, void* out_lo,
                          void* stream, void* ln_out, int ld_ln, const float* ln_gamma, const float* ln_beta, float ln_eps) {
    GemmParams p;
    memset(&p, 0, sizeof(p));
    p.ln_out = ln_out; p.ld_ln = ld_ln; p.ln_gamma = ln_gamma; p.ln_beta = ln_beta; p.ln_eps = ln_eps;
    p.A = A; p.W = W; p.out = out; p.bias = bias; p.rowvec = rowvec; p.residual = residual;
    p.residual_lo = residual_lo; p.out_lo = out_lo;
    p.M = M; p.N = N; p.K = K; p.lda = lda; p.ldw = ldw; p.ldc = ldc; p.ldr = ldr; p.ldrv = ldrv;
    p.rows_per_vec = rows_per_vec;
    p.geglu = (flags & MVE_GEMM_GEGLU) ? 1 : 0;
    p.out_f32 = (flags & MVE_GEMM_OUT_F32) ? 1 : 0;
    p.out_scale = out_scale;
    p.res_after_scale = (flags & MVE_GEMM_RES_AFTER_SCALE) ? 1 : 0;
    if (M == 0) return MVE_OK;
    int rc = check_common(p, "gemm");
    if (rc) return rc;
    MVE_CHECK(A && lda % 8 == 0 && lda >= K, MVE_ERR_ARG, "gemm: bad A/lda (%d)", lda);
    p.w_major = gemm_w_major_on() && M < N;
    p.splitk = 1;
    if (workspace && !(flags & MVE_GEMM_NO_SPLITK)) {
        const int sk = choose_splitk(rows_per_image, N, K);
        if (sk > 1 && workspace_bytes >= (size_t)sk * M * N * sizeof(float)) { p.splitk = sk; p.partial = (float*)workspace; }
    }
    if (dtype == MVE_F16) return launch_gemm<F16Tag, 0>(p, (hipStream_t)stream);
    if (dtype == MVE_BF16) return launch_gemm<BF16Tag, 0>(p, (hipStream_t)stream);
    mve_set_error("gemm: unsupported dtype %d", dtype);
    return MVE_ERR_ARG;
}

static int conv3x3_impl(int dtype, const void* x1, int C1, const void* x2, int C2, const void* x3, int C3, const void* x4, int C4, int B,
                        int Hs, int Ws, int stride, int upsample, const void* W, int Cout, void* out, int ldc, const float* bias,
                        const float* rowvec, int ldrv, const void* residual, int ldr, int flags, float out_scale, void* workspace,
                        size_t workspace_bytes, void* stream, const void* residual_lo = nullptr, void* out_lo = nullptr) {
    GemmParams p;
    memset(&p, 0, sizeof(p));
    MVE_CHECK(stride == 1 || stride == 2, MVE_ERR_ARG, "conv3x3: stride must be 1 or 2");
    MVE_CHECK(!(upsample && stride != 1), MVE_ERR_ARG, "conv3x3: upsample requires stride 1");
    MVE_CHECK(C1 > 0 && C1 % 8 == 0 && C2 >= 0 && C2 % 8 == 0, MVE_ERR_ARG,
              "conv3x3: channel counts must be multiples of 8 (C1=%d C2=%d)", C1, C2);
    MVE_CHECK(x1 && (C2 == 0 || x2), MVE_ERR_ARG, "conv3x3: null input");
    if (B == 0) return MVE_OK;
    p.g.Hs = Hs; p.g.Ws = Ws;
    p.g.ups = upsample ? 1 : 0;
    p.g.Hv = Hs << p.g.ups; p.g.Wv = Ws << p.g.ups;
    p.g.stride = stride;
    p.g.pad = p.g.pad_x = (flags & MVE_CONV_PAD_BR) ? 0 : 1;
    MVE_CHECK(p.g.pad == 1 || (stride == 2 && !upsample && Hs % 2 == 0 && Ws % 2 == 0), MVE_ERR_ARG,
              "conv3x3: MVE_CONV_PAD_BR is the stride-2 downsampler of an even-sized input");
    p.g.Ho = (p.g.Hv + 2 - 3) / stride + 1;
    p.g.Wo = (p.g.Wv + 2 - 3) / stride + 1;
    p.g.C1 = C1; p.g.C2 = C2;
    p.g.chunk64 = (flags & MVE_CONV_W_CHUNK64) ? 1 : 0;
    MVE_CHECK(!p.g.chunk64 || (C1 % 64 == 0 && C2 % 64 == 0), MVE_ERR_ARG,
              "conv3x3: MVE_CONV_W_CHUNK64 needs channel counts that are multiples of 64 (C1=%d C2=%d)", C1, C2);
    p.A = x1; p.A2 = x2; p.W = W; p.out = out; p.bias = bias; p.rowvec = rowvec; p.residual = residual;
    p.residual_lo = residual_lo; p.out_lo = out_lo;
    p.M = B * p.g.Ho * p.g.Wo; p.N = Cout; p.K = 9 * (C1 + C2);
    if (C3 > 0) {
        MVE_CHECK(p.g.chunk64 && !upsample && stride == 1 && C3 % 64 == 0 && C4 >= 0 && C4 % 64 == 0 && x3 && (C4 == 0 || x4), MVE_ERR_ARG,
                  "conv3x3_shortcut: needs MVE_CONV_W_CHUNK64, stride 1, no upsample and shortcut channel counts that are multiples of 64");
        p.g.nk_main = p.K / BK;
        p.g.C3 = C3; p.g.C4 = C4;
        p.A3 = x3; p.A4 = x4;
        p.K += C3 + C4;
    }
    p.ldc = ldc; p.ldr = ldr; p.ldrv = ldrv; p.ldw = p.K;
    p.rows_per_vec = p.g.Ho * p.g.Wo;
    p.geglu = 0;
    p.out_f32 = (flags & MVE_GEMM_OUT_F32) ? 1 : 0;
    p.out_scale = out_scale;
    p.res_after_scale = (flags & MVE_GEMM_RES_AFTER_SCALE) ? 1 : 0;
    int rc = check_common(p, "conv3x3");
    if (rc) return rc;
    p.w_major = gemm_w_major_on() && (long long)p.M * (C1 + C2) < (long long)p.N * p.K;
    p.splitk = 1;
    if (workspace && !(flags & MVE_GEMM_NO_SPLITK)) {
        const int sk = choose_splitk(p.g.Ho * p.g.Wo, p.N, p.K);
        if (sk > 1 && workspace_bytes >= (size_t)sk * p.M * p.N * sizeof(float)) { p.splitk = sk; p.partial = (float*)workspace; }
    }
    if (dtype == MVE_F16) return launch_gemm<F16Tag, 1>(p, (hipStream_t)stream);
    if (dtype == MVE_BF16) return launch_gemm<BF16Tag, 1>(p, (hipStream_t)stream);
    mve_set_error("conv3x3: unsupported dtype %d", dtype);
    return MVE_ERR_ARG;
}

int mve_conv3x3(int dtype, const void* x1, int C1, const void* x2, int C2, int B, int Hs, int Ws, int stride,
                int upsample, const void* W, int Cout, void* out, int ldc, const float* bias, const float* rowvec,
                int ldrv, const void* residual, int ldr, int flags, float out_scale, void* workspace, size_t workspace_bytes,
                void* stream) {
    return conv3x3_impl(dtype, x1, C1, x2, C2, nullptr, 0, nullptr, 0, B, Hs, Ws, stride, upsample, W, Cout, out, ldc, bias, rowvec, ldrv,
                        residual, ldr, flags, out_scale, workspace, workspace_bytes, stream);
}

int mve_conv3x3_pair(int dtype, const void* x1, int C1, const void* x2, int C2, int B, int Hs, int Ws, int stride,
                     int upsample, const void* W, int Cout, void* out, int ldc, const float* bias, const float* rowvec,
                     int ldrv, const void* residual, int ldr, int flags, float out_scale, void* workspace, size_t workspace_bytes,
                     const void* residual_lo, void* out_lo, void* stream) {
    return conv3x3_impl(dtype, x1, C1, x2, C2, nullptr, 0, nullptr, 0, B, Hs, Ws, stride, upsample, W, Cout, out, ldc, bias, rowvec, ldrv,
                        residual, ldr, flags, out_scale, workspace, workspace_bytes, stream, residual_lo, out_lo);
}


int mve_pack_upsample_phase_weights(int src_dtype, int dst_dtype, const void* w_oihw, int Cout, int C, void* W4, void* stream) {
    MVE_CHECK(w_oihw && W4 && Cout > 0 && C > 0 && C % 64 == 0, MVE_ERR_ARG, "pack_upsample_phase_weights: needs C %% 64 == 0 (Cout=%d C=%d)", Cout, C);
    const size_t n = (size_t)16 * Cout * C;
    const unsigned grid = (unsigned)mve_cdiv(n, 256);
    hipStream_t s = (hipStream_t)stream;
#define MVE_PPW(ST, TAG) k_pack_phase_weights<ST, TAG><<<grid, 256, 0, s>>>((const ST*)w_oihw, (typename TAG::T*)W4, Cout, C)
    if (dst_dtype == MVE_F16) {
        if (src_dtype == MVE_F32) MVE_PPW(float, F16Tag); else if (src_dtype == MVE_F16) MVE_PPW(f16, F16Tag); else if (src_dtype == MVE_BF16) MVE_PPW(bf16, F16Tag);
        else { mve_set_error("pack_upsample_phase_weights: unsupported source dtype %d", src_dtype); return MVE_ERR_ARG; }
    } else if (dst_dtype == MVE_BF16) {
        if (src_dtype == MVE_F32) MVE_PPW(float, BF16Tag); else if (src_dtype == MVE_F16) MVE_PPW(f16, BF16Tag); else if (src_dtype == MVE_BF16) MVE_PPW(bf16, BF16Tag);
        else { mve_set_error("pack_upsample_phase_weights: unsupported source dtype %d", src_dtype); return MVE_ERR_ARG; }
    } else { mve_set_error("pack_upsample_phase_weights: unsupported destination dtype %d", dst_dtype); return MVE_ERR_ARG; }
#undef MVE_PPW
    MVE_LAUNCH_CHECK();
    return MVE_OK;
}

int mve_upsample_conv_phases_supported(int C, int Cout, int B, int Hs, int Ws) {
    if (C <= 0 || C % 64 != 0 || Cout <= 0 || B <= 0 || Hs <= 0 || Ws <= 0 || (Ws & (Ws - 1)) != 0) return 0;
    if (Cout % 320 != 0 && Cout % 256 != 0 && Cout % 128 != 0) return 0;
    if (!gemm_pp_on() || (long long)B * Hs * Ws < 64 || (long long)B * Hs * Ws > 0x7fffffffll / 4) return 0;
    const unsigned long long lim = 0xFFFFFF00ull - 65536ull;
    if (((unsigned long long)B * Hs * Ws + 2ull * Ws + 4) * (unsigned long long)C * 2 >= lim) return 0;
    if ((unsigned long long)Cout * 4 * C * 2 >= lim) return 0;
// ... 80 lines not shown
```

mvedit_amd/csrc/gemm_big.hip:

```cpp
#include "common.h"

#include "gemm_shared.h"
#include "gemm_big_epilogue.h"

namespace {

constexpr int BM2 = 256, NTH = 512;
constexpr int WAVES_N = 4;
constexpr int WTM = 128;
constexpr int MF = WTM / 16;
constexpr int RPP = NTH / 8;
constexpr int A_PASSES = BM2 / RPP;
constexpr int A_STAGE = BM2 * ROW_BYTES;
constexpr int smem_big(int bn2) { return 2 * (A_STAGE + bn2 * ROW_BYTES); }
static_assert(64 * (320 + 4) * 4 <= smem_big(320) && 64 * (256 + 4) * 4 <= smem_big(256), "epilogue staging must fit");

template <class Tag, int MODE, bool SEQ, bool FAST, int BN2>
__global__ __launch_bounds__(NTH, 2) void k_gemm_big(const GemmParams p) {
    typedef typename Tag::V8 V8;
    typedef typename Tag::T T;
    constexpr int WTN = BN2 / WAVES_N, NF = WTN / 16;
    constexpr int B_PASSES = BN2 / RPP;
    constexpr int STAGE = A_STAGE + BN2 * ROW_BYTES;
    extern __shared__ __attribute__((aligned(16))) unsigned char smem[];

    const int tid = threadIdx.x, lane = tid & 63, wid = tid >> 6;
    const int wm = wid / WAVES_N, wn = wid % WAVES_N;

    const int tiles_n = (p.N + BN2 - 1) / BN2;
    const int tiles_m = (p.M + BM2 - 1) / BM2;
    const int S = p.splitk > 1 ? p.splitk : 1;
    const unsigned lin = mve_xcd_remap(blockIdx.x, (unsigned)(tiles_m * tiles_n * S));
    const int kslice = lin % S;
    const unsigned tile = lin / S;
    const int tm = tile / tiles_n, tn = tile % tiles_n;
    const int m0 = tm * BM2, n0 = tn * BN2;

    const int lr = tid >> 3;
    const int lc = (tid & 7) ^ ((lr >> 1) & 7);
    const T* __restrict__ Wp = reinterpret_cast<const T*>(p.W);

    const T* a_row[A_PASSES];
    int cb[A_PASSES], cy[A_PASSES], cx[A_PASSES];
    int pix[A_PASSES];
    unsigned vmask[A_PASSES];
    if constexpr (MODE == 0) {
#pragma unroll
        for (int j = 0; j < A_PASSES; ++j) {
            int m = m0 + lr + j * RPP;
            m = m < p.M ? m : p.M - 1;
            a_row[j] = reinterpret_cast<const T*>(p.A) + (size_t)m * p.lda;
        }
    } else {
        const int hw = p.g.Ho * p.g.Wo;
#pragma unroll
        for (int j = 0; j < A_PASSES; ++j) {
            int m = m0 + lr + j * RPP;
            m = m < p.M ? m : p.M - 1;
            const int b = m / hw, r = m - b * hw;
            const int y = r / p.g.Wo;
            cb[j] = b;
            cy[j] = y * p.g.stride - p.g.pad;
            cx[j] = (r - y * p.g.Wo) * p.g.stride - p.g.pad_x;
            if constexpr (FAST) {
                pix[j] = (cb[j] * p.g.Hs + (cy[j] >> p.g.ups)) * p.g.Ws + (cx[j] >> p.g.ups);
                unsigned mk = 0;
#pragma unroll
                for (int t = 0; t < 9; ++t) {
                    const int yi = cy[j] + t / 3, xi = cx[j] + t % 3;
                    if (yi >= 0 && yi < p.g.Hv && xi >= 0 && xi < p.g.Wv) mk |= 1u << t;
                }
                if (p.g.ups) mk |= ((unsigned)(cy[j] & 1) << 9) | ((unsigned)(cx[j] & 1) << 10);
                vmask[j] = mk;
            }
        }
    }
    const T* w_row[B_PASSES];
#pragma unroll
    for (int j = 0; j < B_PASSES; ++j) {
        int n = n0 + lr + j * RPP;
        n = n < p.N ? n : p.N - 1;
        w_row[j] = Wp + (size_t)n * p.ldw;
    }

    const int nk_all = (p.K + BK - 1) / BK;
    const int kt_begin = (int)((long long)nk_all * kslice / S), kt_end = (int)((long long)nk_all * (kslice + 1) / S);
    const int Ctot = p.g.C1 + p.g.C2;
    int tap = 0, cin = 0;
    if constexpr (MODE == 1) {
// ... 167 lines not shown
```

mvedit_amd/csrc/gemm_pp.hip:

```cpp
#include "common.h"

#include <type_traits>

#include "gemm_shared.h"
#include "gemm_big_epilogue.h"

namespace {

typedef int i32x4 __attribute__((ext_vector_type(4)));

constexpr int PBM = 256, PNTH = 512;
constexpr int PROWB = 64;
constexpr int PNSLOT = 4;
constexpr int P_A_SLOT = PBM * PROWB;
constexpr unsigned P_NUMREC = 0xFFFFFF00u;
constexpr int pp_slot_bytes(int bn) { return P_A_SLOT + bn * PROWB; }
constexpr int pp_smem(int bn, int nsl = PNSLOT) { return nsl * pp_slot_bytes(bn) + (bn == 160 ? 1024 : 0); }
static_assert(2 * pp_smem(160, 3) <= 160 * 1024, "two blocks of the three-slot 256 x 160 tile per CU");
static_assert(64 * (320 + 4) * 4 <= pp_smem(320) && 64 * (256 + 4) * 4 <= pp_smem(256) && 64 * (128 + 4) * 4 <= pp_smem(128) &&
              64 * (160 + 4) * 4 <= pp_smem(160), "epilogue staging must fit");

__device__ __forceinline__ i32x4 pp_rsrc(unsigned long long base, bool live) {
    i32x4 r;
    r[0] = __builtin_amdgcn_readfirstlane((int)(unsigned)base);
// ... 107 lines not shown
            for (int j = 0; j < NF; ++j)
                *reinterpret_cast<f32x4*>(Cs + (lane & 15) * P2_CS_LD + j * 16 + (lane >> 4) * 4) = acc[j][i];
#pragma unroll
            for (int k = 0; k < 3; ++k) {
                const int rel = k == 0 ? 0 : (k == 1 ? 6 : rel2);
                const bool ok = act && (k < 2 || r0 < 4);
                const float* cs = Cs + (r0 + rel) * P2_CS_LD + ch * 8;
                const f32x4 lo = *reinterpret_cast<const f32x4*>(cs), hi = *reinterpret_cast<const f32x4*>(cs + 4);
                float v[8];
#pragma unroll
                for (int e = 0; e < 4; ++e) { v[e] = lo[e] + fb0[e]; v[4 + e] = hi[e] + fb1[e]; }
                if constexpr (RES) {
                    const V8 res = fr[k];
                    if (i + 1 < MF) fr[k] = *reinterpret_cast<const V8*>(resb + (size_t)((i + 1) * 16 + rel) * p.ldr);
#pragma unroll
                    for (int e = 0; e < 8; ++e) v[e] += Tag::to_f32(res[e]);
                }
                V8 pk;
#pragma unroll
                for (int e = 0; e < 8; ++e) pk[e] = Tag::from_f32(v[e]);
                if (ok) *reinterpret_cast<V8*>(outb + (size_t)(i * 16 + rel) * p.ldc) = pk;
            }
        }
    };
    if (has_res) run(std::true_type()); else run(std::false_type());
}

__device__ unsigned long long* g_pp_prof = nullptr;

template <int V> struct PInt { static constexpr int value = V; };

template <class Tag, int MODE, bool SEQ, int BN2, bool PROF = false, int NSL = PNSLOT, bool PAIR = false, bool RED = false, bool LNF = false>
__global__ __launch_bounds__(PNTH, NSL == 3 ? 4 : 2) void k_gemm_pp(const GemmParams p) {
    typedef typename Tag::V8 V8;
    constexpr int WAVES_N = (BN2 == 128 || BN2 == 160) ? 2 : 4, WAVES_M = 8 / WAVES_N;
    constexpr int WTM = PBM / WAVES_M, MF = WTM / 16;
    constexpr int WTN = BN2 / WAVES_N, NF = WTN / 16;
    constexpr int NPB_ALL = BN2 / 16, NPB_BASE = NPB_ALL / 4, NPB_REM = NPB_ALL % 4;
    constexpr int NPB = NPB_BASE + (NPB_REM ? 1 : 0);
    constexpr int NPA = 4;
    constexpr int SLOT = pp_slot_bytes(BN2);
    constexpr int DIST = NSL - 1;
    static_assert(NSL == 4 || (NSL == 3 && BN2 == 160 && MODE == 0 && !SEQ), "three slots: the two-blocks-per-CU GEMM tile only");
    extern __shared__ __attribute__((aligned(16))) unsigned char smem[];

    const int tid = threadIdx.x, lane = tid & 63;
    const int wid = __builtin_amdgcn_readfirstlane(tid >> 6);
    const int role = wid >> 2, widx = wid & 3;
    const int wm = wid / WAVES_N, wn = wid % WAVES_N;

    const int tiles_n = (p.N + BN2 - 1) / BN2;
    const int tiles_m = (p.M + PBM - 1) / PBM;
    const int S = p.splitk > 1 ? p.splitk : 1;
    const unsigned lin = mve_xcd_remap(blockIdx.x, (unsigned)(tiles_m * tiles_n * S));
    int kslice, tm, tn;
    if (p.w_major) {
        tm = __builtin_amdgcn_readfirstlane((int)(lin % (unsigned)tiles_m));
        const unsigned rest = lin / (unsigned)tiles_m;
        kslice = __builtin_amdgcn_readfirstlane((int)(rest % (unsigned)S));
        tn = __builtin_amdgcn_readfirstlane((int)(rest / (unsigned)S));
    } else {
        kslice = lin % S;
        const unsigned t_ = lin / S;
        tm = t_ / tiles_n; tn = t_ % tiles_n;
    }
    const unsigned tile = (unsigned)(tm * tiles_n + tn);
    const int m0 = tm * PBM, n0 = tn * BN2;

    const int nk_all = p.K / BK;
    const int kt_begin = __builtin_amdgcn_readfirstlane((int)((long long)nk_all * kslice / S));
    const int kt_end = __builtin_amdgcn_readfirstlane((int)((long long)nk_all * (kslice + 1) / S));
    const int nsteps = 2 * (kt_end - kt_begin);

    f32x4 acc[NF][MF];
#pragma unroll
    for (int j = 0; j < NF; ++j)
#pragma unroll
        for (int i = 0; i < MF; ++i) acc[j][i] = f32x4{0.f, 0.f, 0.f, 0.f};
    unsigned long long prof_v[8] = {0, 0, 0, 0, 0, 0, 0, 0}, prof_start = 0, prof_loop0 = 0, prof_end_loop = 0;
    if constexpr (PROF) prof_start = __builtin_readcyclecounter();
    auto run = [&](auto role_c) {
    constexpr int ROLE = decltype(role_c)::value;
    if constexpr (PAIR) {
        if (p.residual && p.splitk <= 1) {
            typedef typename Tag::T T;
            typedef T T4 __attribute__((ext_vector_type(4)));
            const T* rh = reinterpret_cast<const T*>(p.residual);
            const unsigned char* rl = reinterpret_cast<const unsigned char*>(p.residual_lo);
            const int col = n0 + wn * WTN + (lane >> 4) * 4;
#pragma unroll
            for (int i = 0; i < MF; ++i) {
                int m = m0 + wm * WTM + i * 16 + (lane & 15);
                m = m < p.M ? m : p.M - 1;
                const size_t ro = (size_t)m * p.ldr + col;
                T4 h[NF];
                unsigned l[NF];
#pragma unroll
                for (int j = 0; j < NF; ++j) {
                    h[j] = *reinterpret_cast<const T4*>(rh + ro + j * 16);
                    l[j] = rl ? *reinterpret_cast<const unsigned*>(rl + ro + j * 16) : 0u;
                }
#pragma unroll
                for (int j = 0; j < NF; ++j) {
                    f32x4 a;
                    float lf[4];
                    mve_lo8_unpack4(l[j], lf);
#pragma unroll
                    for (int e = 0; e < 4; ++e) a[e] = Tag::to_f32(h[j][e]) + lf[e];
                    acc[j][i] = a;
                }
                __builtin_amdgcn_sched_barrier(0);
                asm volatile("" ::: "memory");
                __builtin_amdgcn_sched_barrier(0);
            }
            asm volatile("s_waitcnt vmcnt(0)" ::: "memory");
        }
    }
    constexpr int NPM = ROLE == 0 ? NPB : NPA;
    const int prow = lane >> 2;
    const unsigned c16 = (unsigned)(((lane & 3) ^ ((lane >> (p.old_swizzle ? 4 : 3)) & 3)) << 4);
// ... 441 lines not shown
```

mvedit_amd/csrc/gemm_shared.h:

```cpp
#pragma once
#include "common.h"

namespace {

constexpr int BK = 64;
constexpr int NT = 256;
constexpr int ROW_BYTES = BK * 2;

typedef __attribute__((address_space(3))) void* lds_ptr_t;
typedef const __attribute__((address_space(1))) void* gbl_ptr_t;

__device__ __attribute__((aligned(16))) unsigned int g_zero_page[4] = {0u, 0u, 0u, 0u};

struct ConvGeom {
    int Hs, Ws, Hv, Wv, Ho, Wo;
    int C1, C2;
    int stride;
    int pad;
    int ups;
    int chunk64;
    int nk_main, C3, C4;
    int kw;
    int pad_x;
    int phase_rows;
};

__device__ __forceinline__ int conv_phase_of(int m, int R) { return R > 0 ? (int)(m >= R) + (int)(m >= 2 * R) + (int)(m >= 3 * R) : 0; }

struct GemmParams {
    const void* A;
    const void* A2;
    const void* A3;
    const void* A4;
    const void* W;
    void* out;
    const float* bias;
    const float* rowvec;
    const void* residual;
    const void* residual_lo;
    void* out_lo;
    int M, N, K;
    int lda, ldw, ldc, ldr, ldrv;
    int rows_per_vec;
    int geglu;
    int out_f32;
    float out_scale;
    int res_after_scale;
    int splitk;
    float* partial;
    int splitk_seq;
    int tile_n;
    int old_swizzle;
    int dbg;
    int orow_shift, orow_extra;
    int* sk_sync;
    int w_major;
    void* ln_out;
    const float* ln_gamma;
    const float* ln_beta;
    float ln_eps;
    int ld_ln;
    ConvGeom g;
};

__device__ __forceinline__ int swz(int row, int chunk) { return row * ROW_BYTES + ((chunk ^ ((row >> 1) & 7)) << 4); }

__device__ __forceinline__ float gelu_erf(float x) {
    const float t = __builtin_amdgcn_fmed3f(x, -5.0f, 5.0f);
    const float u = t * t;
    const float P = __builtin_fmaf(__builtin_fmaf(__builtin_fmaf(2.99665181e-05f, u, 0.00375327937f), u, 0.0294303672f), u, 0.398879537f);
    const float Q = __builtin_fmaf(__builtin_fmaf(__builtin_fmaf(0.00109351574f, u, 0.0246359949f), u, 0.240117083f), u, 1.0f);
    return x * __builtin_fmaf(t * P, __builtin_amdgcn_rcpf(Q), 0.5f);
}

template <class T>
__device__ __forceinline__ const T* conv_src(const GemmParams& p, int cb, int cy, int cx, int tap, int cin, bool kin) {
    const int dy = tap / 3, dx = tap - dy * 3;
    const int yi = cy + dy, xi = cx + dx;
    const bool ok = kin && yi >= 0 && yi < p.g.Hv && xi >= 0 && xi < p.g.Wv;
    if (!ok) return nullptr;
    const bool second = cin >= p.g.C1;
    const T* src = reinterpret_cast<const T*>(second ? p.A2 : p.A);
    const int cs = second ? p.g.C2 : p.g.C1;
    const int ch = second ? cin - p.g.C1 : cin;
    const int ys = yi >> p.g.ups, xs = xi >> p.g.ups;
    return src + (((size_t)cb * p.g.Hs + ys) * p.g.Ws + xs) * cs + ch;
}


template <class Tag, bool PAIR = true, bool RES_DONE = false>
__device__ __forceinline__ void gemm_epilogue_tail(const GemmParams& p, int m, int n, float (&v)[8], const typename Tag::V8& rr, bool ok = true) {
#pragma clang fp contract(off)
    typedef typename Tag::T T;
    typedef typename Tag::V8 V8;
    if (!RES_DONE && p.residual && !p.res_after_scale) {
        if (PAIR && p.residual_lo) {
            const u32x2 rl = *reinterpret_cast<const u32x2*>(reinterpret_cast<const unsigned char*>(p.residual_lo) + (size_t)m * p.ldr + n);
            float r8[8];
            mve_pair_load8<Tag>(rr, rl, r8);
#pragma unroll
            for (int e = 0; e < 8; ++e) v[e] += r8[e];
        } else {
#pragma unroll
            for (int e = 0; e < 8; ++e) v[e] += Tag::to_f32(rr[e]);
        }
    }
    if (p.out_scale != 1.0f) {
#pragma unroll
        for (int e = 0; e < 8; ++e) v[e] *= p.out_scale;
    }
    if (!RES_DONE && p.residual && p.res_after_scale) {
#pragma unroll
        for (int e = 0; e < 8; ++e) v[e] += Tag::to_f32(rr[e]);
    }
    size_t orow;
    if (p.g.phase_rows > 0) {
// ... 108 lines not shown
```

mvedit_amd/csrc/norm.hip:

```cpp
#include "common.h"
#include "ln_core.h"

namespace {

constexpr int GN_THREADS = 256;

template <class Tag>
__device__ __forceinline__ void load8(const typename Tag::T* p, float (&v)[8]) {
    const typename Tag::V8 x = *reinterpret_cast<const typename Tag::V8*>(p);
#pragma unroll
    for (int e = 0; e < 8; ++e) v[e] = Tag::to_f32(x[e]);
}

struct GNSrc {
    const void* x1; const void* x2;
    int C1, C2;
    int HW, B;
    const void* x1_lo; const void* x2_lo;
};

template <class Tag>
__device__ __forceinline__ const typename Tag::T* gn_chunk_ptr(const GNSrc& s, int b, int r, int chunk) {
    typedef typename Tag::T T;
    const int ch = chunk * 8;
    if (ch < s.C1) return reinterpret_cast<const T*>(s.x1) + ((size_t)b * s.HW + r) * s.C1 + ch;
    return reinterpret_cast<const T*>(s.x2) + ((size_t)b * s.HW + r) * s.C2 + (ch - s.C1);
}

template <class Tag, bool PAIR>
__device__ __forceinline__ void gn_load8(const GNSrc& s, int b, int r, int chunk, float (&v)[8]) {
    typedef typename Tag::T T;
    const T* ph = gn_chunk_ptr<Tag>(s, b, r, chunk);
    load8<Tag>(ph, v);
    if constexpr (PAIR) {
        const int ch = chunk * 8;
        const T* base_h = reinterpret_cast<const T*>(ch < s.C1 ? s.x1 : s.x2);
        const unsigned char* base_l = reinterpret_cast<const unsigned char*>(ch < s.C1 ? s.x1_lo : s.x2_lo);
        if (base_l) {
            const u32x2 l = *reinterpret_cast<const u32x2*>(base_l + (ph - base_h));
            float a[4], b[4];
            mve_lo8_unpack4(l[0], a);
            mve_lo8_unpack4(l[1], b);
#pragma unroll
            for (int e = 0; e < 4; ++e) { v[e] += a[e]; v[4 + e] += b[e]; }
        }
    }
}

template <class Tag, int GN_TX, bool PAIR = false>
__global__ __launch_bounds__(GN_THREADS) void k_gn_partial(GNSrc s, int nsplit, float* __restrict__ partial) {
    constexpr int GN_TY = GN_THREADS / GN_TX;
    __shared__ float red[GN_TY][GN_TX][16];
    const int C = s.C1 + s.C2;
    const int chunk = blockIdx.y * GN_TX + threadIdx.x;
    const int b = blockIdx.z, split = blockIdx.x;
    const int rows_per = (s.HW + nsplit - 1) / nsplit;
    const int r0 = split * rows_per, r1 = min(s.HW, r0 + rows_per);
    float sum[8], sq[8];
#pragma unroll
    for (int e = 0; e < 8; ++e) { sum[e] = 0.f; sq[e] = 0.f; }
    const bool active = chunk * 8 < C;
    if (active) {
        int r = r0 + threadIdx.y;
        for (; r + 3 * GN_TY < r1; r += 4 * GN_TY) {
            float v[4][8];
#pragma unroll
            for (int k = 0; k < 4; ++k) gn_load8<Tag, PAIR>(s, b, r + k * GN_TY, chunk, v[k]);
#pragma unroll
            for (int k = 0; k < 4; ++k)
#pragma unroll
                for (int e = 0; e < 8; ++e) { sum[e] += v[k][e]; sq[e] += v[k][e] * v[k][e]; }
        }
        for (; r < r1; r += GN_TY) {
            float v[8];
            gn_load8<Tag, PAIR>(s, b, r, chunk, v);
#pragma unroll
            for (int e = 0; e < 8; ++e) { sum[e] += v[e]; sq[e] += v[e] * v[e]; }
        }
    }
#pragma unroll
    for (int e = 0; e < 8; ++e) { red[threadIdx.y][threadIdx.x][e] = sum[e]; red[threadIdx.y][threadIdx.x][8 + e] = sq[e]; }
    __syncthreads();
    if (threadIdx.y == 0 && active) {
        float* out = partial + (((size_t)b * nsplit + split) * C + chunk * 8) * 2;
#pragma unroll
        for (int e = 0; e < 8; ++e) {
            float a = 0.f, q = 0.f;
#pragma unroll
            for (int y = 0; y < GN_TY; ++y) { a += red[y][threadIdx.x][e]; q += red[y][threadIdx.x][8 + e]; }
            out[2 * e] = a;
            out[2 * e + 1] = q;
        }
    }
}

__global__ void k_gn_finalize(const float* __restrict__ partial, int B, int nsplit, int C, int G, int HW, float eps,
                              float* __restrict__ stats ) {
    const int i = blockIdx.x * (blockDim.x >> 6) + (threadIdx.x >> 6);
    if (i >= B * G) return;
    const int lane = threadIdx.x & 63;
    const int b = i / G, g = i - b * G, cpg = C / G;
    double a = 0.0, q = 0.0;
    for (int t = lane; t < nsplit * cpg; t += 64) {
        const int sp = t / cpg, c = t - sp * cpg;
        const float* p = partial + (((size_t)b * nsplit + sp) * C + (size_t)g * cpg + c) * 2;
        a += (double)p[0];
        q += (double)p[1];
    }
#pragma unroll
    for (int d = 32; d >= 1; d >>= 1) { a += __shfl_xor(a, d, 64); q += __shfl_xor(q, d, 64); }
    if (lane != 0) return;
    const double n = (double)cpg * HW;
    const double mean = a / n;
    double var = q / n - mean * mean;
    var = var > 0.0 ? var : 0.0;
    stats[2 * i] = (float)mean;
    stats[2 * i + 1] = (float)(1.0 / sqrt(var + (double)eps));
}

template <class Tag, int GN_TX, bool PAIR = false>
__global__ __launch_bounds__(GN_THREADS) void k_gn_apply(GNSrc s, int nsplit, int G, const float* __restrict__ stats,
                                                         const float* __restrict__ gamma, const float* __restrict__ beta,
                                                         int silu, void* __restrict__ out) {
    constexpr int GN_TY = GN_THREADS / GN_TX;
    typedef typename Tag::T T;
    typedef typename Tag::V8 V8;
    const int C = s.C1 + s.C2;
    const int chunk = blockIdx.y * GN_TX + threadIdx.x;
    if (chunk * 8 >= C) return;
    const int b = (int)gridDim.z - 1 - (int)blockIdx.z, split = (int)gridDim.x - 1 - (int)blockIdx.x;
    const int rows_per = (s.HW + nsplit - 1) / nsplit;
    const int r0 = split * rows_per, r1 = min(s.HW, r0 + rows_per);
    const int cpg = C / G;
    float sc[8], sh[8];
#pragma unroll
    for (int e = 0; e < 8; ++e) {
        const int c = chunk * 8 + e;
        const int g = c / cpg;
        const float mean = stats[2 * (b * G + g)], rstd = stats[2 * (b * G + g) + 1];
        sc[e] = rstd * gamma[c];
        sh[e] = beta[c] - mean * sc[e];
    }
    T* o = reinterpret_cast<T*>(out);
    auto finish = [&](const float (&v)[8], int r) {
        V8 pk;
#pragma unroll
        for (int e = 0; e < 8; ++e) {
            float y = v[e] * sc[e] + sh[e];
            if (silu) y = y / (1.0f + __expf(-y));
            pk[e] = Tag::from_f32(y);
        }
        *reinterpret_cast<V8*>(o + ((size_t)b * s.HW + r) * C + chunk * 8) = pk;
    };
    int r = r0 + threadIdx.y;
    for (; r + 3 * GN_TY < r1; r += 4 * GN_TY) {
        float v[4][8];
#pragma unroll
        for (int k = 0; k < 4; ++k) gn_load8<Tag, PAIR>(s, b, r + k * GN_TY, chunk, v[k]);
#pragma unroll
        for (int k = 0; k < 4; ++k) finish(v[k], r + k * GN_TY);
    }
    for (; r < r1; r += GN_TY) {
        float v[8];
        gn_load8<Tag, PAIR>(s, b, r, chunk, v);
        finish(v, r);
    }
}

constexpr int GNF_MAX_GROUPS = 4;

template <int NT>
__device__ __forceinline__ void gnf_block_sum(float (&v)[GNF_MAX_GROUPS], float* red ) {
#pragma unroll
    for (int g = 0; g < GNF_MAX_GROUPS; ++g) {
#pragma unroll
        for (int d = 32; d >= 1; d >>= 1) v[g] += __shfl_xor(v[g], d, 64);
    }
    __syncthreads();
    if ((threadIdx.x & 63) == 0) {
#pragma unroll
        for (int g = 0; g < GNF_MAX_GROUPS; ++g) red[(threadIdx.x >> 6) * GNF_MAX_GROUPS + g] = v[g];
    }
    __syncthreads();
#pragma unroll
    for (int g = 0; g < GNF_MAX_GROUPS; ++g) {
        float a = 0.f;
        for (int w = 0; w < NT / 64; ++w) a += red[w * GNF_MAX_GROUPS + g];
        v[g] = a;
    }
}

template <class Tag, int NT, int MAXI, bool PAIR = false>
__global__ __launch_bounds__(NT) void k_gn_fused(GNSrc s, int G, int W8, int nchunk, int xcd_map, float eps, const float* __restrict__ gamma,
                                                 const float* __restrict__ beta, int silu, void* __restrict__ out) {
    typedef typename Tag::T T;
    typedef typename Tag::V8 V8;
    __shared__ float red[(NT / 64) * GNF_MAX_GROUPS];
    __shared__ float tab[2][128];
    const int C = s.C1 + s.C2, cpg = C / G, cg = W8 * 8 / cpg;
    int b, chunk;
    if (xcd_map) {
        const int id = blockIdx.x;
        b = 8 * (id / (8 * nchunk)) + (id & 7);
        chunk = (id >> 3) % nchunk;
    } else {
        b = blockIdx.x / nchunk;
        chunk = blockIdx.x - b * nchunk;
    }
    const int total = s.HW * W8;
    V8 raw[MAXI];
    auto vals = [&](int it, int row, int c8, float (&v)[8]) {
#pragma unroll
        for (int e = 0; e < 8; ++e) v[e] = Tag::to_f32(raw[it][e]);
        if constexpr (PAIR) {
            const int ch = (chunk * W8 + c8) * 8;
            const bool first = ch < s.C1;
            const unsigned char* base = reinterpret_cast<const unsigned char*>(first ? s.x1_lo : s.x2_lo);
            if (base) {
                const u32x2 l = *reinterpret_cast<const u32x2*>(base + ((size_t)b * s.HW + row) * (first ? s.C1 : s.C2) + (first ? ch : ch - s.C1));
                float a4[4], b4[4];
                mve_lo8_unpack4(l[0], a4);
                mve_lo8_unpack4(l[1], b4);
#pragma unroll
                for (int e = 0; e < 4; ++e) { v[e] += a4[e]; v[4 + e] += b4[e]; }
            }
        }
    };
    float acc[GNF_MAX_GROUPS] = {0.f, 0.f, 0.f, 0.f};
#pragma unroll
    for (int it = 0; it < MAXI; ++it) {
        const int i = threadIdx.x + it * NT;
        if (i < total) {
            const int row = i / W8, c8 = i - row * W8;
            raw[it] = *reinterpret_cast<const V8*>(gn_chunk_ptr<Tag>(s, b, row, chunk * W8 + c8));
            const int g0 = (c8 * 8) / cpg, eb = (g0 + 1) * cpg - c8 * 8;
            float lo = 0.f, hi = 0.f;
            float x8[8];
            vals(it, row, c8, x8);
#pragma unroll
            for (int e = 0; e < 8; ++e) { const float v = x8[e]; if (e < eb) lo += v; else hi += v; }
#pragma unroll
            for (int g = 0; g < GNF_MAX_GROUPS; ++g) acc[g] += (g == g0 ? lo : 0.f) + (g == g0 + 1 ? hi : 0.f);
        }
    }
    gnf_block_sum<NT>(acc, red);
    const float inv_n = 1.0f / ((float)cpg * (float)s.HW);
    float mean[GNF_MAX_GROUPS];
#pragma unroll
    for (int g = 0; g < GNF_MAX_GROUPS; ++g) { mean[g] = acc[g] * inv_n; acc[g] = 0.f; }
#pragma unroll
    for (int it = 0; it < MAXI; ++it) {
        const int i = threadIdx.x + it * NT;
        if (i < total) {
            const int row = i / W8, c8 = i - row * W8;
            const int g0 = (c8 * 8) / cpg, eb = (g0 + 1) * cpg - c8 * 8;
            float m0 = 0.f, m1 = 0.f;
#pragma unroll
            for (int g = 0; g < GNF_MAX_GROUPS; ++g) { m0 = g == g0 ? mean[g] : m0; m1 = g == g0 + 1 ? mean[g] : m1; }
            float lo = 0.f, hi = 0.f;
            float x8[8];
            vals(it, row, c8, x8);
// ... 21 lines not shown
    T* o = reinterpret_cast<T*>(out);
#pragma unroll
    for (int it = 0; it < MAXI; ++it) {
        const int i = threadIdx.x + it * NT;
        if (i < total) {
            const int row = i / W8, c8 = i - row * W8;
            V8 pk;
            float x8[8];
            vals(it, row, c8, x8);
#pragma unroll
            for (int e = 0; e < 8; ++e) {
                float y = __builtin_fmaf(x8[e], tab[0][c8 * 8 + e], tab[1][c8 * 8 + e]);
                if (silu) y = y / (1.0f + __expf(-y));
                pk[e] = Tag::from_f32(y);
            }
            *reinterpret_cast<V8*>(o + ((size_t)b * s.HW + row) * C + (size_t)(chunk * W8 + c8) * 8) = pk;
        }
    }
}

int g_gn_fused_max_hw = -1;
int g_gn_fused_pair_max_hw = -1;
int gn_fused_pair_max_hw() {
    if (g_gn_fused_pair_max_hw < 0) {
        const char* e = getenv("MVE_GN_FUSED_PAIR_MAX_HW");
        g_gn_fused_pair_max_hw = e ? atoi(e) : 256;
    }
    return g_gn_fused_pair_max_hw;
}

int gnf_plan(int HW, int C, int G, int* nt, int* maxi) {
    if (g_gn_fused_max_hw < 0) {
        const char* e = getenv("MVE_GN_FUSED_MAX_HW");
        g_gn_fused_max_hw = e ? atoi(e) : 1024;
    }
    if (HW > g_gn_fused_max_hw || G <= 0 || C % G) return 0;
    const int cpg = C / G;
    int ch = cpg;
    while (ch % 8) ch += cpg;
    if (cpg < 8 || ch > 128 || C % ch || ch / cpg > GNF_MAX_GROUPS) return 0;
    const int W8 = ch / 8;
    const long long total = (long long)HW * W8;
    if (total <= 256 * 20) *nt = 256;
    else if (total <= 1024 * 20) *nt = 1024;
    else return 0;
    const int per = (int)((total + *nt - 1) / *nt);
    *maxi = per <= 4 ? 4 : (per <= 8 ? 8 : (per <= 12 ? 12 : (per <= 16 ? 16 : 20)));
    return W8;
}

template <class Tag, int NT, bool PAIR = false>
int gnf_launch(const GNSrc& s, int G, int W8, int maxi, float eps, const float* gamma, const float* beta, int silu, void* out, hipStream_t st) {
    const int nchunk = (s.C1 + s.C2) / (W8 * 8);
    const int xcd = (s.B % 8 == 0) ? 1 : 0;
    const unsigned grid = (unsigned)(s.B * nchunk);
    switch (maxi) {
        case 4: k_gn_fused<Tag, NT, 4, PAIR><<<grid, NT, 0, st>>>(s, G, W8, nchunk, xcd, eps, gamma, beta, silu, out); break;
        case 8: k_gn_fused<Tag, NT, 8, PAIR><<<grid, NT, 0, st>>>(s, G, W8, nchunk, xcd, eps, gamma, beta, silu, out); break;
        case 12: k_gn_fused<Tag, NT, 12, PAIR><<<grid, NT, 0, st>>>(s, G, W8, nchunk, xcd, eps, gamma, beta, silu, out); break;
        case 16: k_gn_fused<Tag, NT, 16, PAIR><<<grid, NT, 0, st>>>(s, G, W8, nchunk, xcd, eps, gamma, beta, silu, out); break;
        default: k_gn_fused<Tag, NT, 20, PAIR><<<grid, NT, 0, st>>>(s, G, W8, nchunk, xcd, eps, gamma, beta, silu, out); break;
    }
    MVE_LAUNCH_CHECK();
    return MVE_OK;
}

template <class Tag, int MAXC8, int R>
__global__ __launch_bounds__(256) void k_layernorm(const void* __restrict__ x, int ldx, void* __restrict__ y, int ldy, int M,
                                                   int C, const float* __restrict__ gamma, const float* __restrict__ beta,
                                                   float eps, const void* __restrict__ x_lo) {
    typedef typename Tag::T T;
    typedef typename Tag::V8 V8;
    const int lane = threadIdx.x & 63;
    const int row0 = (blockIdx.x * 4 + (threadIdx.x >> 6)) * R;
    if (row0 >= M) return;
    const int nchunk = C / 8;
    V8 raw[R][MAXC8];
    u32x2 rawl[R][MAXC8];
#pragma unroll
    for (int r = 0; r < R; ++r) {
        const int row = row0 + r < M ? row0 + r : M - 1;
#pragma unroll
        for (int i = 0; i < MAXC8; ++i) {
            const int c = lane + i * 64;
            if (c < nchunk) {
                raw[r][i] = *reinterpret_cast<const V8*>(reinterpret_cast<const T*>(x) + (size_t)row * ldx + c * 8);
                if (x_lo) rawl[r][i] = *reinterpret_cast<const u32x2*>(reinterpret_cast<const unsigned char*>(x_lo) + (size_t)row * ldx + c * 8);
            }
        }
    }
#pragma unroll
    for (int r = 0; r < R; ++r) {
        const int row = row0 + r;
        if (row >= M) break;
        float v[MAXC8][8];
        float s = 0.f;
#pragma unroll
        for (int i = 0; i < MAXC8; ++i) {
            const int c = lane + i * 64;
            if (c < nchunk) {
#pragma unroll
                for (int e = 0; e < 8; ++e) v[i][e] = Tag::to_f32(raw[r][i][e]);
                if (x_lo) {
                    float a[4], b[4];
                    mve_lo8_unpack4(rawl[r][i][0], a);
                    mve_lo8_unpack4(rawl[r][i][1], b);
#pragma unroll
                    for (int e = 0; e < 4; ++e) { v[i][e] += a[e]; v[i][4 + e] += b[e]; }
                }
                s = mve_ln_sum8(v[i], s);
            }
        }
        s = mve_ln_wave_sum(s);
        const float mean = s / (float)C;
        float q = 0.f;
#pragma unroll
        for (int i = 0; i < MAXC8; ++i) {
            const int c = lane + i * 64;
            if (c < nchunk) q = mve_ln_sq8(v[i], mean, q);
        }
        q = mve_ln_wave_sum(q);
        const float rstd = rsqrtf(q / (float)C + eps);
        T* yr = reinterpret_cast<T*>(y) + (size_t)row * ldy;
#pragma unroll
        for (int i = 0; i < MAXC8; ++i) {
            const int c = lane + i * 64;
            if (c < nchunk) *reinterpret_cast<V8*>(yr + c * 8) = mve_ln_out8<Tag>(v[i], mean, rstd, gamma + c * 8, beta + c * 8);
        }
    }
}

int gn_tx(int C) {
    if (C <= 128) return 16;
    if (C <= 256) return 32;
    const int ch = C / 8;
    return ch % 64 == 0 ? 64 : (ch % 32 == 0 ? 32 : (ch % 40 == 0 ? 40 : (ch % 16 == 0 ? 16 : 64)));
}

int gn_nsplit(int B, int HW, int C) {
    if (C <= 256) {
        const int ns = HW / 512;
        return ns < 1 ? 1 : (ns > 512 ? 512 : ns);
    }
    (void)B;
    const int ns = HW / (16 * (GN_THREADS / gn_tx(C)));
    return ns < 1 ? 1 : (ns > 64 ? 64 : ns);
}

template <class Tag>
int gn_run(const GNSrc& s, int G, float eps, const float* gamma, const float* beta, int silu, void* out, float* ws,
           hipStream_t st) {
    const int C = s.C1 + s.C2;
    int nt = 0, maxi = 0;
    const bool pair = s.x1_lo || s.x2_lo;
    if (pair) {
        const int W8 = s.HW <= gn_fused_pair_max_hw() ? gnf_plan(s.HW, C, G, &nt, &maxi) : 0;
        if (W8 && !(nt == 1024 && maxi > 8))
            return nt == 256 ? gnf_launch<Tag, 256, true>(s, G, W8, maxi, eps, gamma, beta, silu, out, st)
                             : gnf_launch<Tag, 1024, true>(s, G, W8, maxi, eps, gamma, beta, silu, out, st);
        const int tx = gn_tx(C);
        const int ncg = (C / 8 + tx - 1) / tx;
        const int ns = gn_nsplit(s.B, s.HW, C);
        float* partial = ws;
        float* stats = ws + (size_t)s.B * ns * C * 2;
        dim3 grid(ns, ncg, s.B), block(tx, GN_THREADS / tx);
        if (tx == 40) k_gn_partial<Tag, 40, true><<<grid, block, 0, st>>>(s, ns, partial);
        else if (tx == 16) k_gn_partial<Tag, 16, true><<<grid, block, 0, st>>>(s, ns, partial);
        else if (tx == 32) k_gn_partial<Tag, 32, true><<<grid, block, 0, st>>>(s, ns, partial);
        else k_gn_partial<Tag, 64, true><<<grid, block, 0, st>>>(s, ns, partial);
        MVE_LAUNCH_CHECK();
        k_gn_finalize<<<mve_cdiv(s.B * G, 4), 256, 0, st>>>(partial, s.B, ns, C, G, s.HW, eps, stats);
        MVE_LAUNCH_CHECK();
        if (tx == 40) k_gn_apply<Tag, 40, true><<<grid, block, 0, st>>>(s, ns, G, stats, gamma, beta, silu, out);
        else if (tx == 16) k_gn_apply<Tag, 16, true><<<grid, block, 0, st>>>(s, ns, G, stats, gamma, beta, silu, out);
        else if (tx == 32) k_gn_apply<Tag, 32, true><<<grid, block, 0, st>>>(s, ns, G, stats, gamma, beta, silu, out);
        else k_gn_apply<Tag, 64, true><<<grid, block, 0, st>>>(s, ns, G, stats, gamma, beta, silu, out);
        MVE_LAUNCH_CHECK();
        return MVE_OK;
    }
    if (const int W8 = gnf_plan(s.HW, C, G, &nt, &maxi))
        return nt == 256 ? gnf_launch<Tag, 256>(s, G, W8, maxi, eps, gamma, beta, silu, out, st)
                         : gnf_launch<Tag, 1024>(s, G, W8, maxi, eps, gamma, beta, silu, out, st);
    const int tx = gn_tx(C);
    const int ncg = (C / 8 + tx - 1) / tx;
    const int ns = gn_nsplit(s.B, s.HW, C);
    float* partial = ws;
    float* stats = ws + (size_t)s.B * ns * C * 2;
    dim3 grid(ns, ncg, s.B), block(tx, GN_THREADS / tx);
    if (tx == 40) k_gn_partial<Tag, 40><<<grid, block, 0, st>>>(s, ns, partial);
    else if (tx == 16) k_gn_partial<Tag, 16><<<grid, block, 0, st>>>(s, ns, partial);
    else if (tx == 32) k_gn_partial<Tag, 32><<<grid, block, 0, st>>>(s, ns, partial);
    else k_gn_partial<Tag, 64><<<grid, block, 0, st>>>(s, ns, partial);
    MVE_LAUNCH_CHECK();
    k_gn_finalize<<<mve_cdiv(s.B * G, 4), 256, 0, st>>>(partial, s.B, ns, C, G, s.HW, eps, stats);
    MVE_LAUNCH_CHECK();
    if (tx == 40) k_gn_apply<Tag, 40><<<grid, block, 0, st>>>(s, ns, G, stats, gamma, beta, silu, out);
    else if (tx == 16) k_gn_apply<Tag, 16><<<grid, block, 0, st>>>(s, ns, G, stats, gamma, beta, silu, out);
    else if (tx == 32) k_gn_apply<Tag, 32><<<grid, block, 0, st>>>(s, ns, G, stats, gamma, beta, silu, out);
    else k_gn_apply<Tag, 64><<<grid, block, 0, st>>>(s, ns, G, stats, gamma, beta, silu, out);
    MVE_LAUNCH_CHECK();
    return MVE_OK;
}

template <class Tag>
int ln_run(const void* x, int ldx, void* y, int ldy, int M, int C, const float* gamma, const float* beta, float eps,
           hipStream_t st, const void* x_lo) {
    const int per_lane = (C / 8 + 63) / 64;
    if (per_lane <= 1) k_layernorm<Tag, 1, 4><<<mve_cdiv(M, 16), 256, 0, st>>>(x, ldx, y, ldy, M, C, gamma, beta, eps, x_lo);
    else if (per_lane == 2) k_layernorm<Tag, 2, 2><<<mve_cdiv(M, 8), 256, 0, st>>>(x, ldx, y, ldy, M, C, gamma, beta, eps, x_lo);
    else if (per_lane == 3) k_layernorm<Tag, 3, 1><<<mve_cdiv(M, 4), 256, 0, st>>>(x, ldx, y, ldy, M, C, gamma, beta, eps, x_lo);
    else k_layernorm<Tag, 4, 1><<<mve_cdiv(M, 4), 256, 0, st>>>(x, ldx, y, ldy, M, C, gamma, beta, eps, x_lo);
    MVE_LAUNCH_CHECK();
    return MVE_OK;
}

}

extern "C" {

int mve_groupnorm_tune(int fused_max_hw) {
    int nt, maxi;
    (void)gnf_plan(1, 8, 1, &nt, &maxi);
    const int prev = g_gn_fused_max_hw;
    if (fused_max_hw >= 0) g_gn_fused_max_hw = fused_max_hw;
    return prev;
}

size_t mve_groupnorm_workspace_bytes(int B, int HW, int C, int G) {
    if (B <= 0 || HW <= 0 || C <= 0) return 64;
    const int ns = gn_nsplit(B, HW, C);
    return sizeof(float) * ((size_t)B * ns * C * 2 + (size_t)B * G * 2 + 16);
}

int mve_groupnorm_silu(int dtype, const void* x1, int C1, const void* x2, int C2, int B, int HW, int G, float eps,
                       const float* gamma, const float* beta, int silu, void* out, void* workspace, void* stream) {
    return mve_groupnorm_silu_pair(dtype, x1, C1, x2, C2, B, HW, G, eps, gamma, beta, silu, out, workspace, nullptr, nullptr, stream);
}

int mve_groupnorm_silu_pair(int dtype, const void* x1, int C1, const void* x2, int C2, int B, int HW, int G, float eps,
                            const float* gamma, const float* beta, int silu, void* out, void* workspace, const void* x1_lo, const void* x2_lo,
                            void* stream) {
    if (B == 0 || HW == 0) return MVE_OK;
    const int C = C1 + C2;
    MVE_CHECK(x1 && out && gamma && beta && workspace && (C2 == 0 || x2), MVE_ERR_ARG, "groupnorm: null pointer");
    MVE_CHECK(C1 % 8 == 0 && C2 % 8 == 0 && G > 0 && C % G == 0, MVE_ERR_ARG,
              "groupnorm: C1=%d C2=%d must be multiples of 8 and C divisible by G=%d", C1, C2, G);
    GNSrc s;
    s.x1 = x1; s.x2 = x2; s.C1 = C1; s.C2 = C2; s.HW = HW; s.B = B;
    s.x1_lo = x1_lo; s.x2_lo = C2 ? x2_lo : nullptr;
    if (dtype == MVE_F16) return gn_run<F16Tag>(s, G, eps, gamma, beta, silu, out, (float*)workspace, (hipStream_t)stream);
    if (dtype == MVE_BF16) return gn_run<BF16Tag>(s, G, eps, gamma, beta, silu, out, (float*)workspace, (hipStream_t)stream);
    mve_set_error("groupnorm: unsupported dtype %d", dtype);
    return MVE_ERR_ARG;
}

int mve_layernorm(int dtype, const void* x, int ldx, void* y, int ldy, int M, int C, const float* gamma, const float* beta,
                  float eps, void* stream) {
    return mve_layernorm_pair(dtype, x, ldx, y, ldy, M, C, gamma, beta, eps, nullptr, stream);
}

int mve_layernorm_pair(int dtype, const void* x, int ldx, void* y, int ldy, int M, int C, const float* gamma, const float* beta,
                       float eps, const void* x_lo, void* stream) {
    if (M == 0) return MVE_OK;
    MVE_CHECK(x && y && gamma && beta, MVE_ERR_ARG, "layernorm: null pointer");
    MVE_CHECK(C % 8 == 0 && C <= 2048 && ldx % 8 == 0 && ldy % 8 == 0, MVE_ERR_ARG,
              "layernorm: C=%d must be a multiple of 8 and <= 2048", C);
    if (dtype == MVE_F16) return ln_run<F16Tag>(x, ldx, y, ldy, M, C, gamma, beta, eps, (hipStream_t)stream, x_lo);
    if (dtype == MVE_BF16) return ln_run<BF16Tag>(x, ldx, y, ldy, M, C, gamma, beta, eps, (hipStream_t)stream, x_lo);
    mve_set_error("layernorm: unsupported dtype %d", dtype);
    return MVE_ERR_ARG;
}

}
```

mvedit_amd/csrc/unet.hip:

```cpp
#include "executor_builder.h"
#include "builder_unet.h"
#include "builder_vae.h"
#include "builder_sr.h"
#include "builder_lpips.h"

namespace {

int ensure_plan(Unet& u, int B, int H, int W, int n_img, int has_res, int io_dtype, int res_nhwc, int ctx_len) {
    ++u.tick;
    for (auto& pp : u.plans) {
        const Plan& p = *pp;
        if (p.B == B && p.H == H && p.W == W && p.n_img == n_img && p.has_res == has_res && p.io_dtype == io_dtype &&
            p.res_nhwc == res_nhwc && p.ctx_len == ctx_len && p.add_type == u.cfg.add_type && p.ao == u.ao) {
            pp->last_use = u.tick;
            u.cur = pp.get();
            return MVE_OK;
        }
    }
    std::unique_ptr<Plan> np(new Plan());
    np->ao = u.ao;
    Builder b(u, *np);
    b.ctx_rows_per_img = ctx_len;
    u.cur = nullptr;
    const int rc = u.cfg.lpips ? b.build_lpips(B, H, W, io_dtype) : u.cfg.sr ? b.build_sr(B, H, W, io_dtype) : u.cfg.vae ? b.build_vae(B, H, W, io_dtype) : b.build(B, H, W, n_img, has_res, io_dtype, res_nhwc);
// ... 350 lines not shown
int mve_unet_missing_params(void* handle, char* buf, int buf_len) {
    MVE_CHECK(handle, MVE_ERR_ARG, "unet_missing_params: null handle");
    Unet* u = (Unet*)handle;
    int missing = 0;
    std::string first;
    for (auto& n : u->expected)
        if (!u->loaded.count(n)) { if (!missing) first = n; ++missing; }
    if (buf && buf_len > 0) { strncpy(buf, first.c_str(), (size_t)buf_len - 1); buf[buf_len - 1] = 0; }
    return missing;
}

int mve_unet_plan(void* handle, int B, int H, int W, int ctx_len, int num_cross_attn_imgs, int has_residuals, int io_dtype,
                  int residuals_nhwc, size_t* workspace_bytes, int* n_ops, double* flops ) {
    MVE_CHECK(handle && B > 0 && H > 0 && W > 0 && ctx_len > 0 && num_cross_attn_imgs >= 1, MVE_ERR_ARG, "unet_plan: bad arguments");
    Unet* u = (Unet*)handle;
    int rc = ensure_plan(*u, B, H, W, num_cross_attn_imgs, has_residuals, io_dtype, residuals_nhwc, ctx_len);
    if (rc) return rc;
    if (workspace_bytes) *workspace_bytes = u->cur->ws_bytes;
    if (n_ops) *n_ops = (int)u->cur->ops.size();
    if (flops) for (int i = 0; i < OC_COUNT; ++i) flops[i] = u->cur->flops[i];
    return MVE_OK;
}

int mve_unet_forward(void* handle, int phase, const void* d_sample, int io_dtype, const float* d_timesteps, const void* d_ctx,
                     int B, int H, int W, int ctx_len, int num_cross_attn_imgs, const void* const* down_residuals,
                     const void* d_mid_residual, int residuals_nhwc, void* d_out, void* d_workspace, size_t workspace_bytes,
                     float* op_ms , void* stream) {
    MVE_CHECK(handle, MVE_ERR_ARG, "unet_forward: null handle");
    Unet* u = (Unet*)handle;
    MVE_CHECK(!u->cfg.controlnet && !u->cfg.vae && !u->cfg.sr && !u->cfg.lpips, MVE_ERR_ARG, "unet_forward: handle is a ControlNet / VAE / SRVGG (use their own forward calls)");
    {
        char first[256];
        const int miss = mve_unet_missing_params(handle, first, sizeof(first));
        MVE_CHECK(miss == 0, MVE_ERR_STATE, "unet_forward: %d parameters not loaded (first: %s)", miss, first);
    }
    const int has_res = (down_residuals && d_mid_residual) ? 1 : 0;
    int rc = ensure_plan(*u, B, H, W, num_cross_attn_imgs, has_res, io_dtype, residuals_nhwc, ctx_len);
    if (rc) return rc;
    const Plan& pl = *u->cur;
    MVE_CHECK(d_workspace && workspace_bytes >= pl.ws_bytes, MVE_ERR_NOMEM, "unet_forward: workspace %zu < required %zu",
              workspace_bytes, pl.ws_bytes);
    MVE_CHECK(d_timesteps && d_ctx && (phase == 1 || d_out) && (phase == 2 || d_sample), MVE_ERR_ARG, "unet_forward: null pointer");
    Run r;
    r.ws = (unsigned char*)d_workspace; r.wt = u->slab;
    r.sample = d_sample; r.timesteps = d_timesteps; r.ctx = d_ctx; r.out = d_out;
    r.down_res = down_residuals; r.mid_res = d_mid_residual;
    r.ref_store = u->ref_store;
    MVE_CHECK(pl.ref_store_bytes == 0 || (u->ref_store && u->ref_store_bytes >= pl.ref_store_bytes), MVE_ERR_NOMEM,
              "unet_forward: reference store %zu < required %zu bytes", u->ref_store_bytes, pl.ref_store_bytes);
    r.stream = (hipStream_t)stream;
    if (phase != 2) {
        rc = take_added_cond(*u, B, r, "unet_forward");
        if (rc) return rc;
    }
    const size_t lo = phase == 2 ? pl.enc_end : 0, hi = phase == 1 ? pl.enc_end : pl.ops.size();
    if (u->graph_mode && !op_ms) {
        MVE_CHECK(stream != nullptr, MVE_ERR_ARG,
                  "unet_forward: hipGraph replay cannot capture the legacy default stream -- run under a non-default stream (torch.cuda.stream(...))");
        std::vector<const void*> key = {d_sample, d_timesteps, d_ctx, d_out, d_workspace, d_mid_residual, u->ref_store, stream};
        if (has_res) for (int i = 0; i < u->cfg.n_levels * (u->cfg.layers_per_block + 1); ++i) key.push_back(down_residuals[i]);
        if (r.add_text) {
            key.push_back(r.add_text); key.push_back(r.add_ids);
            key.push_back((const void*)(size_t)(((size_t)r.add_text_dim << 32) | ((size_t)r.add_n_ids << 8) | (size_t)r.add_text_dtype));
        }
        Unet::GraphEntry* ge = nullptr;
        for (auto& g : u->graphs)
            if (g.plan_uid == pl.uid && g.phase == phase && g.ptrs == key) { ge = &g; break; }
        if (ge && ge->exec) {
            ge->last_use = u->tick;
            MVE_HIP(hipGraphLaunch(ge->exec, r.stream));
            return MVE_OK;
        }
        if (ge) {
            MVE_HIP(hipStreamBeginCapture(r.stream, hipStreamCaptureModeRelaxed));
            for (size_t i = lo; i < hi && rc == MVE_OK; ++i) rc = pl.ops[i].fn(r);
            hipGraph_t graph = nullptr;
            const hipError_t ce = hipStreamEndCapture(r.stream, &graph);
            if (rc) { if (graph) (void)hipGraphDestroy(graph); return rc; }
            MVE_HIP(ce);
            MVE_HIP(hipGraphInstantiate(&ge->exec, graph, nullptr, nullptr, 0));
            ge->graph = graph;
            ge->last_use = u->tick;
            MVE_HIP(hipGraphLaunch(ge->exec, r.stream));
            return MVE_OK;
        }
        if (u->graphs.size() >= 8) {
            size_t lru = 0;
            for (size_t i = 1; i < u->graphs.size(); ++i) if (u->graphs[i].last_use < u->graphs[lru].last_use) lru = i;
            if (u->graphs[lru].exec) (void)hipGraphExecDestroy(u->graphs[lru].exec);
            if (u->graphs[lru].graph) (void)hipGraphDestroy(u->graphs[lru].graph);
            u->graphs.erase(u->graphs.begin() + lru);
        }
        Unet::GraphEntry ne;
        ne.plan_uid = pl.uid; ne.phase = phase; ne.seen = 1; ne.ptrs = key; ne.last_use = u->tick;
        u->graphs.push_back(ne);
    }
    std::vector<hipEvent_t> ev;
    if (op_ms) {
        ev.resize(hi - lo + 1);
        for (auto& e : ev) MVE_HIP(hipEventCreate(&e));
        MVE_HIP(hipEventRecord(ev[0], r.stream));
    }
    for (size_t i = lo; i < hi; ++i) {
        rc = pl.ops[i].fn(r);
        if (rc) return rc;
        if (op_ms) MVE_HIP(hipEventRecord(ev[i - lo + 1], r.stream));
    }
    if (op_ms) {
        MVE_HIP(hipStreamSynchronize(r.stream));
        for (size_t i = lo; i < hi; ++i) MVE_HIP(hipEventElapsedTime(&op_ms[i], ev[i - lo], ev[i - lo + 1]));
        for (auto& e : ev) (void)hipEventDestroy(e);
    }
    return MVE_OK;
}

int mve_unet_graph(void* handle, int enable) {
    MVE_CHECK(handle, MVE_ERR_ARG, "unet_graph: null handle");
    Unet* u = (Unet*)handle;
    const int old = u->graph_mode ? 1 : 0;
    if (enable >= 0) {
        u->graph_mode = enable != 0;
        if (!u->graph_mode) {
            for (auto& g : u->graphs) { if (g.exec) (void)hipGraphExecDestroy(g.exec); if (g.graph) (void)hipGraphDestroy(g.graph); }
            u->graphs.clear();
        }
    }
    return old;
}

int mve_unet_set_attention(void* handle, int ip_tokens, float ip_scale, int ref_mode, int ref_H, int ref_W, int ref_skip,
                           void* d_ref_store, size_t ref_store_bytes) {
    MVE_CHECK(handle && ip_tokens >= 0 && ref_mode >= 0 && ref_mode <= 2 && ref_skip >= 0, MVE_ERR_ARG, "unet_set_attention: bad arguments");
    Unet* u = (Unet*)handle;
    u->ao.ip_tokens = ip_tokens; u->ao.ip_scale = ip_tokens ? ip_scale : 1.0f;
    u->ao.ref_mode = ref_mode; u->ao.ref_skip = ref_mode ? ref_skip : 0;
    u->ao.ref_H = ref_mode == 2 ? ref_H : 0; u->ao.ref_W = ref_mode == 2 ? ref_W : 0;
    u->ref_store = (unsigned char*)d_ref_store; u->ref_store_bytes = ref_store_bytes;
    return MVE_OK;
}

int mve_unet_set_residual_mode(void* handle, int pair) {
    MVE_CHECK(handle, MVE_ERR_ARG, "unet_set_residual_mode: null handle");
    Unet* u = (Unet*)handle;
    MVE_CHECK(!u->cfg.vae && !u->cfg.sr && !u->cfg.lpips, MVE_ERR_ARG, "unet_set_residual_mode: a UNet / ControlNet handle is needed");
    const int old = u->ao.residual_pair;
    if (pair >= 0) u->ao.residual_pair = pair ? 1 : 0;
    return old;
}

int mve_unet_set_addition_embed(void* handle, int addition_type, int addition_time_embed_dim, int projection_input_dim) {
    MVE_CHECK(handle, MVE_ERR_ARG, "unet_set_addition_embed: null handle");
    Unet* u = (Unet*)handle;
    Config& c = u->cfg;
    MVE_CHECK(!c.vae && !c.sr && !c.lpips, MVE_ERR_ARG, "unet_set_addition_embed: a UNet / ControlNet handle is needed");
    MVE_CHECK(addition_type == 0 || addition_type == 1, MVE_ERR_ARG, "unet_set_addition_embed: addition type %d (0 = none, 1 = text_time)", addition_type);
    MVE_CHECK(!u->slab && u->loaded.empty(), MVE_ERR_STATE, "unet_set_addition_embed: parameters are already loaded; declare the embedding right after create");
    MVE_CHECK(!c.add_type, MVE_ERR_STATE, "unet_set_addition_embed: the handle already has an addition embedding");
    if (addition_type == 0) return MVE_OK;
    MVE_CHECK(addition_time_embed_dim > 0 && addition_time_embed_dim % 2 == 0, MVE_ERR_ARG, "unet_set_addition_embed: addition_time_embed_dim %d must be even",
              addition_time_embed_dim);
    MVE_CHECK(projection_input_dim > addition_time_embed_dim && projection_input_dim % 8 == 0, MVE_ERR_ARG,
              "unet_set_addition_embed: projection input width %d must be a multiple of 8 above addition_time_embed_dim", projection_input_dim);
    c.add_type = addition_type; c.add_time_dim = addition_time_embed_dim; c.add_P = projection_input_dim;
    layout_addition_embed(*u);
    return MVE_OK;
}

int mve_unet_bind_added_cond(void* handle, const void* d_text_embeds, int text_dtype, int text_dim, const float* d_time_ids, int n_ids, int B) {
    MVE_CHECK(handle, MVE_ERR_ARG, "unet_bind_added_cond: null handle");
    Unet* u = (Unet*)handle;
    const Config& c = u->cfg;
    MVE_CHECK(c.add_type == 1, MVE_ERR_STATE, "unet_bind_added_cond: the handle has no addition embedding (mve_unet_set_addition_embed)");
    if (!d_text_embeds && !d_time_ids) { u->added = Unet::AddedCond(); return MVE_OK; }
    MVE_CHECK(d_text_embeds && d_time_ids, MVE_ERR_ARG, "unet_bind_added_cond: text_embeds and time_ids come together");
    MVE_CHECK(text_dtype == MVE_F32 || text_dtype == MVE_F16 || text_dtype == MVE_BF16, MVE_ERR_ARG, "unet_bind_added_cond: bad text_embeds dtype %d", text_dtype);
    MVE_CHECK(B > 0 && text_dim > 0 && n_ids > 0, MVE_ERR_ARG, "unet_bind_added_cond: bad shape");
    MVE_CHECK((long long)text_dim + (long long)n_ids * c.add_time_dim == c.add_P, MVE_ERR_ARG,
              "unet_bind_added_cond: text width %d + %d time ids x %d != projection input width %d", text_dim, n_ids, c.add_time_dim, c.add_P);
    u->added.text = d_text_embeds; u->added.ids = d_time_ids; u->added.text_dtype = text_dtype; u->added.text_dim = text_dim;
    u->added.n_ids = n_ids; u->added.B = B;
    return MVE_OK;
}

int mve_controlnet_set_cond_repeat(void* handle, int repeat) {
    MVE_CHECK(handle, MVE_ERR_ARG, "controlnet_set_cond_repeat: null handle");
    Unet* u = (Unet*)handle;
    MVE_CHECK(u->cfg.controlnet, MVE_ERR_ARG, "controlnet_set_cond_repeat: a ControlNet handle is needed");
    const int old = u->ao.cn_cond_repeat;
    if (repeat >= 1) u->ao.cn_cond_repeat = repeat;
    return old;
}

size_t mve_unet_ref_store_bytes(void* handle, int B, int ref_H, int ref_W, int ref_skip) {
    if (!handle || B <= ref_skip) return 0;
    const Config& c = ((Unet*)handle)->cfg;
    std::vector<ResnetDesc> rs;
    std::vector<XfDesc> xs;
    enumerate(c, rs, xs);
    size_t total = 0;
    for (auto& x : xs) {
// ... 23 lines not shown
```

mvedit_amd/unet.py:

```python
import ctypes
import os
from types import SimpleNamespace

import torch

from . import _lib
from .ops import dt as _dt

SD15_CONFIG = dict(
    in_channels=4, out_channels=4, block_out_channels=(320, 640, 1280, 1280), layers_per_block=2,
    down_attn=(True, True, True, False), num_heads=(8, 8, 8, 8), cross_attention_dim=768, norm_num_groups=32,
    norm_eps=1e-5, transformer_layers=(1, 1, 1, 1), use_linear_projection=False)

SD21_CONFIG = dict(
    in_channels=4, out_channels=4, block_out_channels=(320, 640, 1280, 1280), layers_per_block=2,
    down_attn=(True, True, True, False), num_heads=(5, 10, 20, 20), cross_attention_dim=1024, norm_num_groups=32,
    norm_eps=1e-5, transformer_layers=(1, 1, 1, 1), use_linear_projection=True)

SDXL_CONFIG = dict(
    in_channels=4, out_channels=4, block_out_channels=(320, 640, 1280), layers_per_block=2,
    down_attn=(False, True, True), num_heads=(5, 10, 20), cross_attention_dim=2048, norm_num_groups=32,
    norm_eps=1e-5, transformer_layers=(0, 2, 10), use_linear_projection=True,
    addition_embed_type='text_time', addition_time_embed_dim=256, projection_class_embeddings_input_dim=2816)

# ... 57 lines not shown

    def _declare_addition_embed(self):
        add = self.cfg.get('addition_embed_type')
        if add not in ADDITION_TYPES:
            raise NotImplementedError(f'addition_embed_type={add!r} is not implemented by the engine')
        self._ack_keep = None
        if add is not None:
            _lib.call('mve_unet_set_addition_embed', self._h, ADDITION_TYPES[add], int(self.cfg['addition_time_embed_dim']),
                      int(self.cfg['projection_class_embeddings_input_dim']))

    def _bind_added_cond(self, added_cond_kwargs, B):
        add = self.cfg.get('addition_embed_type')
        if add is None:
            if added_cond_kwargs:
                raise ValueError('added_cond_kwargs given to an engine without an addition embedding (config addition_embed_type is None)')
            return
        if not added_cond_kwargs:
            raise ValueError("this engine has addition_embed_type='text_time': added_cond_kwargs={'text_embeds', 'time_ids'} is required")
        for key in ('text_embeds', 'time_ids'):
            if key not in added_cond_kwargs:
                raise ValueError(f"added_cond_kwargs lacks '{key}' (addition_embed_type='text_time' needs text_embeds and time_ids)")
        text, ids = added_cond_kwargs['text_embeds'], added_cond_kwargs['time_ids']
        td, P = int(self.cfg['addition_time_embed_dim']), int(self.cfg['projection_class_embeddings_input_dim'])
        for key, t in (('text_embeds', text), ('time_ids', ids)):
            if not torch.is_tensor(t) or t.dim() != 2 or not t.is_floating_point():
                raise ValueError(f"added_cond_kwargs['{key}'] must be a 2-D floating-point tensor [batch, width]")
            if t.shape[0] != B:
                raise ValueError(f"added_cond_kwargs['{key}'] has batch {t.shape[0]}, the sample has {B}")
        if text.shape[1] + ids.shape[1] * td != P:
            raise ValueError(f'added_cond_kwargs widths: text_embeds {text.shape[1]} + time_ids {ids.shape[1]} x {td} != '
                             f'projection_class_embeddings_input_dim {P}')
        if text.dtype not in (torch.float32, torch.float16, torch.bfloat16):
            text = text.float()
        text = text.to(self.device).contiguous()
        ids = ids.to(device=self.device, dtype=torch.float32).contiguous()
        self._ack_keep = (text, ids)
        _lib.call('mve_unet_bind_added_cond', self._h, _lib.ptr(text), _dt(text), text.shape[1], _lib.ptr(ids), ids.shape[1], B)

    def __del__(self):
        h = getattr(self, '_h', None)
        if h:
            try:
                _lib.raw('mve_unet_destroy')(h)
            except Exception:
                pass
            self._h = None

    def set_residual_pair(self, flag=True):
        return bool(_lib.raw('mve_unet_set_residual_mode')(self._h, int(bool(flag))))

    @property
    def residual_pair(self):
        return bool(_lib.raw('mve_unet_set_residual_mode')(self._h, -1))

    def enable_graph(self, flag=True):
        return bool(_lib.raw('mve_unet_graph')(self._h, int(bool(flag))))

    @classmethod
    def from_state_dict(cls, state_dict, config=None, dtype=torch.float16, device='cuda'):
        eng = cls(config, dtype, device)
        eng.load_state_dict(state_dict)
        return eng

    def load_state_dict(self, state_dict, strict=True):
        with torch.cuda.device(self.device):
            s = _lib.stream_ptr(self.device)
            for name, t in state_dict.items():
                t = t.detach()
                if t.dtype not in (torch.float32, torch.float16, torch.bfloat16):
                    t = t.float()
                t = t.to(self.device).contiguous()
                shape = (ctypes.c_longlong * t.dim())(*t.shape)
                _lib.call('mve_unet_load_param', self._h, name.encode(), _lib.ptr(t), _dt(t), t.dim(), shape, s)
            torch.cuda.current_stream(self.device).synchronize()
        if strict:
            buf = ctypes.create_string_buffer(256)
            missing = _lib.raw('mve_unet_missing_params')(self._h, buf, 256)
            if missing:
                raise KeyError(f'{missing} UNet parameters missing from the state dict (first: {buf.value.decode()})')
        return self

    _REF_KEY = '__mvedit_amd_ref_store__'

    def set_ip_adapter(self, num_tokens=16, scale=1.0):
        self._ip = (int(num_tokens), float(scale))

    def _set_attention(self, cak, B, H, W):
        cak = cak or {}
        mode, ref_dict = cak.get('mode'), cak.get('ref_dict')
        skip = 1 if cak.get('is_cfg_guidance') else 0
        store, ref_mode, rH, rW = None, 0, 0, 0
        if mode is not None and ref_dict is not None:
            if mode == 'w':
                nbytes = _lib.raw('mve_unet_ref_store_bytes')(self._h, B, H, W, skip)
                store = torch.empty(nbytes, dtype=torch.uint8, device=self.device)
                ref_dict[self._REF_KEY] = (store, B, H, W, skip)
                ref_mode = 1
            elif mode in ('r', 'm'):
                store, Bs, rH, rW, sk = ref_dict.pop(self._REF_KEY) if mode == 'r' else ref_dict[self._REF_KEY]
                assert Bs == B and sk == skip, 'reference pass and read pass must have the same batch layout'
                ref_mode = 2
            else:
                raise AssertionError(mode)
        self._ref_keep = store
        _lib.call('mve_unet_set_attention', self._h, self._ip[0], self._ip[1], ref_mode, rH, rW, skip, _lib.ptr(store),
                  store.numel() if store is not None else 0)
# ... 155 lines not shown
```

Baseline: 16.40 denoise-steps/s.

## Skip duplicated CFG half in UNet prefix before first cross-attention

Under classifier-free guidance the conditional and unconditional halves of the batch share the same latent and timestep. The UNet prefix up to the first cross-attention query projection is therefore identical for both halves. A device-side probe compares the two halves of the sample and time embedding and sets a flag. While the flag is set, the GEMM, conv, norm and attention kernels in that prefix early-exit for blocks in the second half, and a broadcast kernel then copies the live boundary tensors from the first half to the second. This trades a probe, some broadcast copies and extra per-block predicate checks for skipping half of the early high-resolution work, including self-attention at 4096 tokens.

```diff
diff --git a/include/mvedit_amd.h b/include/mvedit_amd.h
--- a/include/mvedit_amd.h
+++ b/include/mvedit_amd.h
@@ -314,6 +314,8 @@
 MVE_API int mve_unet_set_attention(void* handle, int ip_tokens, float ip_scale, int ref_mode, int ref_H, int ref_W, int ref_skip,
                                    void* d_ref_store, size_t ref_store_bytes);
 MVE_API int mve_unet_set_residual_mode(void* handle, int pair);
+MVE_API int mve_unet_tune_cfg_prefix(void* handle, int on);
+MVE_API int mve_unet_cfg_prefix_state(void* handle);
 MVE_API int mve_unet_set_addition_embed(void* handle, int addition_type, int addition_time_embed_dim, int projection_input_dim);
 MVE_API int mve_unet_bind_added_cond(void* handle, const void* d_text_embeds, int text_dtype, int text_dim, const float* d_time_ids, int n_ids,
                                      int B);
diff --git a/mvedit_amd/csrc/attention.hip b/mvedit_amd/csrc/attention.hip
--- a/mvedit_amd/csrc/attention.hip
+++ b/mvedit_amd/csrc/attention.hip
@@ -13,6 +13,7 @@
     int B, Lq, Lk, Lk2, heads;
     float scale_log2e;
     int prescaled;
+    const int* skip_if;
 };
 
 template <int DP, bool KSW2> __device__ __forceinline__ int k_perm(int row, int pc) {
@@ -67,10 +68,11 @@
 
     const int q_tiles = (p.Lq + QB - 1) / QB;
     const unsigned nblk = (unsigned)(q_tiles * p.heads * p.B);
-    const unsigned bid = mve_xcd_remap(blockIdx.x, nblk);
+    const unsigned bid = p.skip_if ? mve_xcd_remap_halves(blockIdx.x, nblk, nblk / 2) : mve_xcd_remap(blockIdx.x, nblk);
     const int qt = bid % q_tiles;
     const int h = (bid / q_tiles) % p.heads;
     const int b = bid / (q_tiles * p.heads);
+    if (mve_second_half_skipped(p.skip_if, 2 * b >= p.B)) return;
     const int Ltot = p.Lk + p.Lk2;
 
     const T* Qp = reinterpret_cast<const T*>(p.Q);
@@ -379,10 +381,11 @@
 
     const int q_tiles = (p.Lq + QB - 1) / QB;
     const unsigned nblk = (unsigned)(q_tiles * p.heads * p.B);
-    const unsigned bid = mve_xcd_remap(blockIdx.x, nblk);
+    const unsigned bid = p.skip_if ? mve_xcd_remap_halves(blockIdx.x, nblk, nblk / 2) : mve_xcd_remap(blockIdx.x, nblk);
     const int qt = bid % q_tiles;
     const int h = (bid / q_tiles) % p.heads;
     const int b = bid / (q_tiles * p.heads);
+    if (mve_second_half_skipped(p.skip_if, 2 * b >= p.B)) return;
     const int Ltot = p.Lk + p.Lk2;
 
     const T* kb1 = reinterpret_cast<const T*>(p.K) + (size_t)b * p.Lk * p.ldk + h * D;
@@ -857,6 +860,8 @@
     p.B = B; p.Lq = Lq; p.Lk = Lk; p.Lk2 = Lk2; p.heads = heads;
     p.scale_log2e = prescaled ? 1.0f : scale * 1.4426950408889634f;
     p.prescaled = prescaled;
+    p.skip_if = mve_skip_second_half();
+    MVE_CHECK(!p.skip_if || B % 2 == 0, MVE_ERR_ARG, "attention: the second-half predicate needs an even batch (B=%d)", B);
     if (dtype == MVE_F16) return dispatch_d<F16Tag>(p, head_dim, (hipStream_t)stream);
     if (dtype == MVE_BF16) return dispatch_d<BF16Tag>(p, head_dim, (hipStream_t)stream);
     mve_set_error("attention: unsupported dtype %d", dtype);
diff --git a/mvedit_amd/csrc/builder_unet.h b/mvedit_amd/csrc/builder_unet.h
--- a/mvedit_amd/csrc/builder_unet.h
+++ b/mvedit_amd/csrc/builder_unet.h
@@ -158,6 +158,8 @@
         conv(x_in, 8, Bb, H, W, 1, 0, wt("conv_in.w"), c.ch[0], x, wt("conv_in.b"), Ref(), 0, Ref(), 0, "conv_in");
     }
     rel(x_in);
+    if (!c.controlnet && pl.ao.cfg_prefix && Bb % 2 == 0 && (Bb / 2) % n_img == 0 && pl.ao.ref_mode == 0)
+        begin_prefix((size_t)(Bb / 2) * c.in_ch * H * W * esz(io_dtype), (size_t)(Bb / 2) * ld_temb * 4);
     skips.push_back({x, c.ch[0], H, W});
     int h = H, w = W, cin = c.ch[0];
     for (int i = 0; i < n; ++i) {
@@ -182,6 +184,7 @@
             skips.push_back({x, cin, h, w});
         }
     }
+    end_prefix();
     pl.enc_end = pl.ops.size();
     if (c.controlnet) {
         const int C = c.ch[n - 1];
@@ -283,6 +286,7 @@
         op(OC_OTHER, 0, "nhwc->nchw", [=](const Run& r) { return mve_nhwc_to_nchw(io_dtype, MVE_F32, r.p(o8), 8, Bb, oc, H, W, r.p(dst), r.stream); });
     }
     pl.ws_bytes = ar.peak + 256;
+    if (pl.cfg_prefix) { *pfx_flag = ar.peak; pl.cfg_flag_off = ar.peak; }
     pl.ref_store_bytes = ref_off;
     if (!u.err.empty()) { mve_set_error("unet plan: %s", u.err.c_str()); u.err.clear(); return MVE_ERR_STATE; }
     return MVE_OK;
diff --git a/mvedit_amd/csrc/common.h b/mvedit_amd/csrc/common.h
--- a/mvedit_amd/csrc/common.h
+++ b/mvedit_amd/csrc/common.h
@@ -38,6 +38,15 @@
             return MVE_ERR_HIP;                                        \
         }                                                              \
     } while (0)
+
+const int* mve_skip_second_half();
+void mve_set_skip_second_half(const int* d_flag);
+struct MveSkipScope {
+    explicit MveSkipScope(const int* d_flag) { mve_set_skip_second_half(d_flag); }
+    ~MveSkipScope() { mve_set_skip_second_half(nullptr); }
+    MveSkipScope(const MveSkipScope&) = delete;
+    MveSkipScope& operator=(const MveSkipScope&) = delete;
+};
 
 static inline unsigned mve_cdiv(unsigned long long a, unsigned long long b) {
     return (unsigned)((a + b - 1) / b);
@@ -146,3 +155,12 @@
     const unsigned base = (xcd < r) ? xcd * (q + 1u) : r * (q + 1u) + (xcd - r) * q;
     return base + k;
 }
+
+__device__ __forceinline__ unsigned mve_xcd_remap_halves(unsigned bid, unsigned nblk, unsigned n1) {
+    return bid < n1 ? mve_xcd_remap(bid, n1) : n1 + mve_xcd_remap(bid - n1, nblk - n1);
+}
+
+__device__ __forceinline__ bool mve_second_half_skipped(const int* skip_if, bool in_second_half) {
+    if (!skip_if || !__builtin_amdgcn_readfirstlane((int)in_second_half)) return false;
+    return __builtin_amdgcn_readfirstlane(*skip_if) != 0;
+}
diff --git a/mvedit_amd/csrc/common.hip b/mvedit_amd/csrc/common.hip
--- a/mvedit_amd/csrc/common.hip
+++ b/mvedit_amd/csrc/common.hip
@@ -8,6 +8,10 @@
     vsnprintf(g_err, sizeof(g_err), fmt, ap);
     va_end(ap);
 }
+
+static thread_local const int* g_skip_flag = nullptr;
+const int* mve_skip_second_half() { return g_skip_flag; }
+void mve_set_skip_second_half(const int* d_flag) { g_skip_flag = d_flag; }
 
 extern "C" {
 
diff --git a/mvedit_amd/csrc/executor.h b/mvedit_amd/csrc/executor.h
--- a/mvedit_amd/csrc/executor.h
+++ b/mvedit_amd/csrc/executor.h
@@ -180,9 +180,10 @@
     int ref_mode = 0, ref_H = 0, ref_W = 0, ref_skip = 0;
     int residual_pair = 0;
     int cn_cond_repeat = 1;
+    int cfg_prefix = 1;
     bool operator==(const AttnOpts& o) const {
         return ip_tokens == o.ip_tokens && ip_scale == o.ip_scale && ref_mode == o.ref_mode && ref_H == o.ref_H && ref_W == o.ref_W &&
-               ref_skip == o.ref_skip && residual_pair == o.residual_pair && cn_cond_repeat == o.cn_cond_repeat;
+               ref_skip == o.ref_skip && residual_pair == o.residual_pair && cn_cond_repeat == o.cn_cond_repeat && cfg_prefix == o.cfg_prefix;
     }
 };
 
@@ -196,6 +197,8 @@
     std::vector<Op> ops;
     size_t enc_end = 0;
     size_t ws_bytes = 0;
+    bool cfg_prefix = false;
+    size_t cfg_flag_off = 0;
     double flops[OC_COUNT] = {0, 0, 0, 0, 0};
 };
 
@@ -266,6 +269,8 @@
         hipGraphExec_t exec = nullptr;
         unsigned long long last_use = 0;
     };
+    const int* cfg_flag = nullptr;
+    hipStream_t cfg_stream = nullptr;
     bool graph_mode = false;
     std::vector<GraphEntry> graphs;
     unsigned long long plan_counter = 0;
diff --git a/mvedit_amd/csrc/executor_builder.h b/mvedit_amd/csrc/executor_builder.h
--- a/mvedit_amd/csrc/executor_builder.h
+++ b/mvedit_amd/csrc/executor_builder.h
@@ -2,6 +2,41 @@
 #include "executor_params.h"
 
 namespace {
+
+__global__ void k_cfg_probe_init(int* __restrict__ flag) { *flag = 1; }
+
+__device__ __forceinline__ bool cfg_halves_differ(const unsigned char* __restrict__ x, size_t half, size_t t, size_t nt) {
+    const unsigned char* y = x + half;
+    unsigned d = 0;
+    if ((((size_t)x | half) & 15) == 0) {
+        const u32x4* X = reinterpret_cast<const u32x4*>(x);
+        const u32x4* Y = reinterpret_cast<const u32x4*>(y);
+        for (size_t i = t; i < half / 16; i += nt) {
+            const u32x4 a = X[i], b = Y[i];
+            d |= (a[0] ^ b[0]) | (a[1] ^ b[1]) | (a[2] ^ b[2]) | (a[3] ^ b[3]);
+        }
+    } else {
+        for (size_t i = t; i < half; i += nt) d |= (unsigned)(x[i] ^ y[i]);
+    }
+    return d != 0;
+}
+
+__global__ __launch_bounds__(256) void k_cfg_probe(const unsigned char* __restrict__ sample, size_t sample_half, const unsigned char* __restrict__ tproj,
+                                                   size_t tproj_half, int* __restrict__ flag) {
+    const size_t t = (size_t)blockIdx.x * 256 + threadIdx.x, nt = (size_t)gridDim.x * 256;
+    if (cfg_halves_differ(sample, sample_half, t, nt) || cfg_halves_differ(tproj, tproj_half, t, nt)) *flag = 0;
+}
+
+constexpr int CFG_BCAST_MAX = 8;
+struct CfgBcast { unsigned char* p[CFG_BCAST_MAX]; unsigned long long half[CFG_BCAST_MAX]; };
+
+__global__ __launch_bounds__(256) void k_cfg_broadcast(const CfgBcast c, const int* __restrict__ flag) {
+    if (__builtin_amdgcn_readfirstlane(*flag) == 0) return;
+    const unsigned long long half = c.half[blockIdx.y], n16 = half / 16;
+    const u32x4* __restrict__ src = reinterpret_cast<const u32x4*>(c.p[blockIdx.y]);
+    u32x4* __restrict__ dst = reinterpret_cast<u32x4*>(c.p[blockIdx.y] + half);
+    for (unsigned long long i = (unsigned long long)blockIdx.x * 256 + threadIdx.x; i < n16; i += (unsigned long long)gridDim.x * 256) dst[i] = src[i];
+}
 
 struct Builder {
     Unet& u;
@@ -18,7 +53,11 @@
 
     Builder(Unet& u_, Plan& p) : u(u_), pl(p), c(u_.cfg) {}
 
-    Ref ws(size_t bytes) { Ref r; r.kind = Ref::WS; r.off = ar.alloc(bytes); return r; }
+    Ref ws(size_t bytes) {
+        Ref r; r.kind = Ref::WS; r.off = ar.alloc(bytes);
+        if (pfx_on) pfx_live[r.off] = bytes;
+        return r;
+    }
     std::map<size_t, Ref> lo_of;
     Ref ws_stream(size_t bytes) {
         Ref r = ws(bytes);
@@ -33,8 +72,9 @@
     void rel(const Ref& r) {
         if (r.kind != Ref::WS) return;
         auto it = lo_of.find(r.off);
-        if (it != lo_of.end()) { ar.release(it->second.off); lo_of.erase(it); }
+        if (it != lo_of.end()) { ar.release(it->second.off); pfx_live.erase(it->second.off); lo_of.erase(it); }
         ar.release(r.off);
+        pfx_live.erase(r.off);
     }
     Ref wt(const std::string& n, size_t elem_off = 0) {
         auto it = u.params.find(n);
@@ -54,6 +94,66 @@
     void op(int cls, double flops, const char* what, std::function<int(const Run&)> fn) {
         pl.ops.push_back({cls, flops, what, std::move(fn)});
         pl.flops[cls] += flops;
+    }
+
+    bool pfx_on = false;
+    size_t pfx_first = 0;
+    std::map<size_t, size_t> pfx_live;
+    std::shared_ptr<size_t> pfx_flag;
+    size_t pfx_sample_half = 0, pfx_tproj_half = 0;
+    void begin_prefix(size_t sample_half_bytes, size_t tproj_half_bytes) {
+        pfx_on = true;
+        pfx_first = pl.ops.size();
+        pfx_live.clear();
+        pfx_flag = std::make_shared<size_t>(0);
+        pfx_sample_half = sample_half_bytes; pfx_tproj_half = tproj_half_bytes;
+    }
+    void end_prefix() {
+        if (!pfx_on) return;
+        pfx_on = false;
+        const size_t first = pfx_first, end = pl.ops.size();
+        if (end == first) return;
+        std::vector<std::pair<Ref, size_t>> bt;
+        for (auto& kv : pfx_live) {
+            if (kv.second % 32 != 0 && u.err.empty()) u.err = "cfg prefix: a boundary tensor does not split into 16-byte aligned halves";
+            Ref r; r.kind = Ref::WS; r.off = kv.first;
+            bt.push_back({r, kv.second / 2});
+        }
+        pfx_live.clear();
+        pl.cfg_prefix = true;
+        const std::shared_ptr<size_t> fo = pfx_flag;
+        const Ref tp = tproj;
+        const size_t sh = pfx_sample_half, th = pfx_tproj_half;
+        for (size_t i = first; i < end; ++i) {
+            const std::function<int(const Run&)> inner = std::move(pl.ops[i].fn);
+            const bool is_first = i == first, is_last = i + 1 == end;
+            pl.ops[i].fn = [=](const Run& r) -> int {
+                int* flag = reinterpret_cast<int*>(r.ws + *fo);
+                if (is_first) {
+                    const size_t units = (sh > th ? sh : th) / 16 + 1;
+                    k_cfg_probe_init<<<1, 1, 0, r.stream>>>(flag);
+                    k_cfg_probe<<<units > 64 * 256 ? 64u : mve_cdiv(units, 256), 256, 0, r.stream>>>((const unsigned char*)r.sample, sh, (const unsigned char*)r.p(tp), th, flag);
+                    MVE_LAUNCH_CHECK();
+                }
+                int rc;
+                { MveSkipScope scope(flag); rc = inner(r); }
+                if (rc || !is_last) return rc;
+                for (size_t j = 0; j < bt.size(); j += CFG_BCAST_MAX) {
+                    CfgBcast cb;
+                    memset(&cb, 0, sizeof(cb));
+                    const size_t n = bt.size() - j < (size_t)CFG_BCAST_MAX ? bt.size() - j : (size_t)CFG_BCAST_MAX;
+                    size_t most = 0;
+                    for (size_t k = 0; k < n; ++k) {
+                        cb.p[k] = (unsigned char*)r.p(bt[j + k].first); cb.half[k] = bt[j + k].second;
+                        most = bt[j + k].second > most ? bt[j + k].second : most;
+                    }
+                    const unsigned gx = most / 16 > 2048ull * 256 ? 2048u : mve_cdiv(most / 16 + 1, 256);
+                    k_cfg_broadcast<<<dim3(gx, (unsigned)n), 256, 0, r.stream>>>(cb, flag);
+                    MVE_LAUNCH_CHECK();
+                }
+                return (int)MVE_OK;
+            };
+        }
     }
 
     int rows_img = 0;
@@ -294,6 +394,7 @@
             Ref q = ws((size_t)M * C * e);
             gemm(n2, C, wt(b + ".q2.w"), C, q, C, M, C, C, Ref(), Ref(), 0, 0, Ref(), 0, 0, "attn2.to_q");
             rel(n2);
+            end_prefix();
             Ref a2 = ws((size_t)M * C * e);
             const size_t ko = (size_t)u.kv_off[b] * e;
             attn(prescaled(q, b + ".q2.w", hd), C, at(ctxkv, ko), ld_kv, at(ctxkv, ko + (size_t)C * e), ld_kv, a2, C, nb, L, Lt, heads, hd);
diff --git a/mvedit_amd/csrc/gemm.hip b/mvedit_amd/csrc/gemm.hip
--- a/mvedit_amd/csrc/gemm.hip
+++ b/mvedit_amd/csrc/gemm.hip
@@ -45,7 +45,7 @@
     const int tiles_n = (p.N + BN - 1) / BN;
     const int tiles_m = (p.M + BM - 1) / BM;
     const int S = p.splitk > 1 ? p.splitk : 1;
-    const unsigned lin = mve_xcd_remap(blockIdx.x, (unsigned)(tiles_m * tiles_n * S));
+    const unsigned lin = gemm_block_lin(p, (unsigned)(tiles_m * tiles_n * S), tiles_n, S, BM);
     int kslice, tm, tn;
     if (p.w_major) {
         tm = (int)(lin % (unsigned)tiles_m);
@@ -58,6 +58,7 @@
         tm = tile / tiles_n; tn = tile % tiles_n;
     }
     const int m0 = tm * BM, n0 = tn * BN;
+    if (mve_second_half_skipped(p.skip_if, m0 >= p.skip_from)) return;
 
     const int lr = tid >> 3;
     const int lc = (tid & 7) ^ ((lr >> 1) & 7);
@@ -367,6 +368,7 @@
     const size_t i = (size_t)blockIdx.x * 256 + threadIdx.x;
     if (i >= (size_t)p.M * chunks_n) return;
     const int m = (int)(i / chunks_n), n = (int)(i - (size_t)m * chunks_n) * 8;
+    if (p.skip_if && m >= p.skip_from && *p.skip_if != 0) return;
     float v[8] = {0.f, 0.f, 0.f, 0.f, 0.f, 0.f, 0.f, 0.f};
     for (int s = 0; s < p.splitk; ++s) {
         const float* pp = p.partial + ((size_t)s * p.M + m) * p.N + n;
@@ -865,6 +867,10 @@
     if (rc) return rc;
     MVE_CHECK(A && lda % 8 == 0 && lda >= K, MVE_ERR_ARG, "gemm: bad A/lda (%d)", lda);
     p.w_major = gemm_w_major_on() && M < N;
+    if (const int* skip = mve_skip_second_half()) {
+        MVE_CHECK(M % 2 == 0, MVE_ERR_ARG, "gemm: the second-half predicate needs an even number of rows (M=%d)", M);
+        p.skip_if = skip; p.skip_from = M / 2; p.w_major = 0;
+    }
     p.splitk = 1;
     if (workspace && !(flags & MVE_GEMM_NO_SPLITK)) {
         const int sk = choose_splitk(rows_per_image, N, K);
@@ -921,6 +927,10 @@
     int rc = check_common(p, "conv3x3");
     if (rc) return rc;
     p.w_major = gemm_w_major_on() && (long long)p.M * (C1 + C2) < (long long)p.N * p.K;
+    if (const int* skip = mve_skip_second_half()) {
+        MVE_CHECK(B % 2 == 0, MVE_ERR_ARG, "conv3x3: the second-half predicate needs an even batch (B=%d)", B);
+        p.skip_if = skip; p.skip_from = p.M / 2; p.w_major = 0;
+    }
     p.splitk = 1;
     if (workspace && !(flags & MVE_GEMM_NO_SPLITK)) {
         const int sk = choose_splitk(p.g.Ho * p.g.Wo, p.N, p.K);
diff --git a/mvedit_amd/csrc/gemm_big.hip b/mvedit_amd/csrc/gemm_big.hip
--- a/mvedit_amd/csrc/gemm_big.hip
+++ b/mvedit_amd/csrc/gemm_big.hip
@@ -30,11 +30,12 @@
     const int tiles_n = (p.N + BN2 - 1) / BN2;
     const int tiles_m = (p.M + BM2 - 1) / BM2;
     const int S = p.splitk > 1 ? p.splitk : 1;
-    const unsigned lin = mve_xcd_remap(blockIdx.x, (unsigned)(tiles_m * tiles_n * S));
+    const unsigned lin = gemm_block_lin(p, (unsigned)(tiles_m * tiles_n * S), tiles_n, S, BM2);
     const int kslice = lin % S;
     const unsigned tile = lin / S;
     const int tm = tile / tiles_n, tn = tile % tiles_n;
     const int m0 = tm * BM2, n0 = tn * BN2;
+    if (mve_second_half_skipped(p.skip_if, m0 >= p.skip_from)) return;
 
     const int lr = tid >> 3;
     const int lc = (tid & 7) ^ ((lr >> 1) & 7);
diff --git a/mvedit_amd/csrc/gemm_pp.hip b/mvedit_amd/csrc/gemm_pp.hip
--- a/mvedit_amd/csrc/gemm_pp.hip
+++ b/mvedit_amd/csrc/gemm_pp.hip
@@ -183,7 +183,7 @@
     const int tiles_n = (p.N + BN2 - 1) / BN2;
     const int tiles_m = (p.M + PBM - 1) / PBM;
     const int S = p.splitk > 1 ? p.splitk : 1;
-    const unsigned lin = mve_xcd_remap(blockIdx.x, (unsigned)(tiles_m * tiles_n * S));
+    const unsigned lin = gemm_block_lin(p, (unsigned)(tiles_m * tiles_n * S), tiles_n, S, PBM);
     int kslice, tm, tn;
     if (p.w_major) {
         tm = __builtin_amdgcn_readfirstlane((int)(lin % (unsigned)tiles_m));
@@ -197,6 +197,7 @@
     }
     const unsigned tile = (unsigned)(tm * tiles_n + tn);
     const int m0 = tm * PBM, n0 = tn * BN2;
+    if (__builtin_expect(mve_second_half_skipped(p.skip_if, m0 >= p.skip_from), 0)) return;
 
     const int nk_all = p.K / BK;
     const int kt_begin = __builtin_amdgcn_readfirstlane((int)((long long)nk_all * kslice / S));
diff --git a/mvedit_amd/csrc/gemm_shared.h b/mvedit_amd/csrc/gemm_shared.h
--- a/mvedit_amd/csrc/gemm_shared.h
+++ b/mvedit_amd/csrc/gemm_shared.h
@@ -60,8 +60,16 @@
     const float* ln_beta;
     float ln_eps;
     int ld_ln;
+    const int* skip_if;
+    int skip_from;
     ConvGeom g;
 };
+
+__device__ __forceinline__ unsigned gemm_block_lin(const GemmParams& p, unsigned nblk, int tiles_n, int S, int BMT) {
+    if (!p.skip_if) return mve_xcd_remap(blockIdx.x, nblk);
+    const unsigned n1 = (unsigned)((p.skip_from + BMT - 1) / BMT) * (unsigned)(tiles_n * S);
+    return mve_xcd_remap_halves(blockIdx.x, nblk, n1 < nblk ? n1 : nblk);
+}
 
 __device__ __forceinline__ int swz(int row, int chunk) { return row * ROW_BYTES + ((chunk ^ ((row >> 1) & 7)) << 4); }
 
diff --git a/mvedit_amd/csrc/norm.hip b/mvedit_amd/csrc/norm.hip
--- a/mvedit_amd/csrc/norm.hip
+++ b/mvedit_amd/csrc/norm.hip
@@ -17,6 +17,7 @@
     int C1, C2;
     int HW, B;
     const void* x1_lo; const void* x2_lo;
+    const int* skip_if;
 };
 
 template <class Tag>
@@ -54,6 +55,7 @@
     const int C = s.C1 + s.C2;
     const int chunk = blockIdx.y * GN_TX + threadIdx.x;
     const int b = blockIdx.z, split = blockIdx.x;
+    if (mve_second_half_skipped(s.skip_if, 2 * b >= s.B)) return;
     const int rows_per = (s.HW + nsplit - 1) / nsplit;
     const int r0 = split * rows_per, r1 = min(s.HW, r0 + rows_per);
     float sum[8], sq[8];
@@ -95,9 +97,10 @@
 }
 
 __global__ void k_gn_finalize(const float* __restrict__ partial, int B, int nsplit, int C, int G, int HW, float eps,
-                              float* __restrict__ stats ) {
+                              float* __restrict__ stats , const int* __restrict__ skip_if) {
     const int i = blockIdx.x * (blockDim.x >> 6) + (threadIdx.x >> 6);
     if (i >= B * G) return;
+    if (mve_second_half_skipped(skip_if, 2 * (i / G) >= B)) return;
     const int lane = threadIdx.x & 63;
     const int b = i / G, g = i - b * G, cpg = C / G;
     double a = 0.0, q = 0.0;
@@ -129,6 +132,7 @@
     const int chunk = blockIdx.y * GN_TX + threadIdx.x;
     if (chunk * 8 >= C) return;
     const int b = (int)gridDim.z - 1 - (int)blockIdx.z, split = (int)gridDim.x - 1 - (int)blockIdx.x;
+    if (mve_second_half_skipped(s.skip_if, 2 * b >= s.B)) return;
     const int rows_per = (s.HW + nsplit - 1) / nsplit;
     const int r0 = split * rows_per, r1 = min(s.HW, r0 + rows_per);
     const int cpg = C / G;
@@ -207,6 +211,7 @@
         b = blockIdx.x / nchunk;
         chunk = blockIdx.x - b * nchunk;
     }
+    if (mve_second_half_skipped(s.skip_if, 2 * b >= s.B)) return;
     const int total = s.HW * W8;
     V8 raw[MAXI];
     auto vals = [&](int it, int row, int c8, float (&v)[8]) {
@@ -334,7 +339,7 @@
 template <class Tag, int NT, bool PAIR = false>
 int gnf_launch(const GNSrc& s, int G, int W8, int maxi, float eps, const float* gamma, const float* beta, int silu, void* out, hipStream_t st) {
     const int nchunk = (s.C1 + s.C2) / (W8 * 8);
-    const int xcd = (s.B % 8 == 0) ? 1 : 0;
+    const int xcd = (s.B % 8 == 0 && !s.skip_if) ? 1 : 0;
     const unsigned grid = (unsigned)(s.B * nchunk);
     switch (maxi) {
         case 4: k_gn_fused<Tag, NT, 4, PAIR><<<grid, NT, 0, st>>>(s, G, W8, nchunk, xcd, eps, gamma, beta, silu, out); break;
@@ -350,12 +355,13 @@
 template <class Tag, int MAXC8, int R>
 __global__ __launch_bounds__(256) void k_layernorm(const void* __restrict__ x, int ldx, void* __restrict__ y, int ldy, int M,
                                                    int C, const float* __restrict__ gamma, const float* __restrict__ beta,
-                                                   float eps, const void* __restrict__ x_lo) {
+                                                   float eps, const void* __restrict__ x_lo, const int* __restrict__ skip_if) {
     typedef typename Tag::T T;
     typedef typename Tag::V8 V8;
     const int lane = threadIdx.x & 63;
     const int row0 = (blockIdx.x * 4 + (threadIdx.x >> 6)) * R;
     if (row0 >= M) return;
+    if (mve_second_half_skipped(skip_if, 2 * row0 >= M)) return;
     const int nchunk = C / 8;
     V8 raw[R][MAXC8];
     u32x2 rawl[R][MAXC8];
@@ -451,7 +457,7 @@
         else if (tx == 32) k_gn_partial<Tag, 32, true><<<grid, block, 0, st>>>(s, ns, partial);
         else k_gn_partial<Tag, 64, true><<<grid, block, 0, st>>>(s, ns, partial);
         MVE_LAUNCH_CHECK();
-        k_gn_finalize<<<mve_cdiv(s.B * G, 4), 256, 0, st>>>(partial, s.B, ns, C, G, s.HW, eps, stats);
+        k_gn_finalize<<<mve_cdiv(s.B * G, 4), 256, 0, st>>>(partial, s.B, ns, C, G, s.HW, eps, stats, s.skip_if);
         MVE_LAUNCH_CHECK();
         if (tx == 40) k_gn_apply<Tag, 40, true><<<grid, block, 0, st>>>(s, ns, G, stats, gamma, beta, silu, out);
         else if (tx == 16) k_gn_apply<Tag, 16, true><<<grid, block, 0, st>>>(s, ns, G, stats, gamma, beta, silu, out);
@@ -474,7 +480,7 @@
     else if (tx == 32) k_gn_partial<Tag, 32><<<grid, block, 0, st>>>(s, ns, partial);
     else k_gn_partial<Tag, 64><<<grid, block, 0, st>>>(s, ns, partial);
     MVE_LAUNCH_CHECK();
-    k_gn_finalize<<<mve_cdiv(s.B * G, 4), 256, 0, st>>>(partial, s.B, ns, C, G, s.HW, eps, stats);
+    k_gn_finalize<<<mve_cdiv(s.B * G, 4), 256, 0, st>>>(partial, s.B, ns, C, G, s.HW, eps, stats, s.skip_if);
     MVE_LAUNCH_CHECK();
     if (tx == 40) k_gn_apply<Tag, 40><<<grid, block, 0, st>>>(s, ns, G, stats, gamma, beta, silu, out);
     else if (tx == 16) k_gn_apply<Tag, 16><<<grid, block, 0, st>>>(s, ns, G, stats, gamma, beta, silu, out);
@@ -487,11 +493,13 @@
 template <class Tag>
 int ln_run(const void* x, int ldx, void* y, int ldy, int M, int C, const float* gamma, const float* beta, float eps,
            hipStream_t st, const void* x_lo) {
+    const int* skip = mve_skip_second_half();
+    MVE_CHECK(!skip || M % 2 == 0, MVE_ERR_ARG, "layernorm: the second-half predicate needs an even number of rows (M=%d)", M);
     const int per_lane = (C / 8 + 63) / 64;
-    if (per_lane <= 1) k_layernorm<Tag, 1, 4><<<mve_cdiv(M, 16), 256, 0, st>>>(x, ldx, y, ldy, M, C, gamma, beta, eps, x_lo);
-    else if (per_lane == 2) k_layernorm<Tag, 2, 2><<<mve_cdiv(M, 8), 256, 0, st>>>(x, ldx, y, ldy, M, C, gamma, beta, eps, x_lo);
-    else if (per_lane == 3) k_layernorm<Tag, 3, 1><<<mve_cdiv(M, 4), 256, 0, st>>>(x, ldx, y, ldy, M, C, gamma, beta, eps, x_lo);
-    else k_layernorm<Tag, 4, 1><<<mve_cdiv(M, 4), 256, 0, st>>>(x, ldx, y, ldy, M, C, gamma, beta, eps, x_lo);
+    if (per_lane <= 1) k_layernorm<Tag, 1, 4><<<mve_cdiv(M, 16), 256, 0, st>>>(x, ldx, y, ldy, M, C, gamma, beta, eps, x_lo, skip);
+    else if (per_lane == 2) k_layernorm<Tag, 2, 2><<<mve_cdiv(M, 8), 256, 0, st>>>(x, ldx, y, ldy, M, C, gamma, beta, eps, x_lo, skip);
+    else if (per_lane == 3) k_layernorm<Tag, 3, 1><<<mve_cdiv(M, 4), 256, 0, st>>>(x, ldx, y, ldy, M, C, gamma, beta, eps, x_lo, skip);
+    else k_layernorm<Tag, 4, 1><<<mve_cdiv(M, 4), 256, 0, st>>>(x, ldx, y, ldy, M, C, gamma, beta, eps, x_lo, skip);
     MVE_LAUNCH_CHECK();
     return MVE_OK;
 }
@@ -530,6 +538,8 @@
     GNSrc s;
     s.x1 = x1; s.x2 = x2; s.C1 = C1; s.C2 = C2; s.HW = HW; s.B = B;
     s.x1_lo = x1_lo; s.x2_lo = C2 ? x2_lo : nullptr;
+    s.skip_if = mve_skip_second_half();
+    MVE_CHECK(!s.skip_if || B % 2 == 0, MVE_ERR_ARG, "groupnorm: the second-half predicate needs an even batch (B=%d)", B);
     if (dtype == MVE_F16) return gn_run<F16Tag>(s, G, eps, gamma, beta, silu, out, (float*)workspace, (hipStream_t)stream);
     if (dtype == MVE_BF16) return gn_run<BF16Tag>(s, G, eps, gamma, beta, silu, out, (float*)workspace, (hipStream_t)stream);
     mve_set_error("groupnorm: unsupported dtype %d", dtype);
diff --git a/mvedit_amd/csrc/unet.hip b/mvedit_amd/csrc/unet.hip
--- a/mvedit_amd/csrc/unet.hip
+++ b/mvedit_amd/csrc/unet.hip
@@ -426,6 +426,8 @@
     if (phase != 2) {
         rc = take_added_cond(*u, B, r, "unet_forward");
         if (rc) return rc;
+        u->cfg_flag = pl.cfg_prefix ? reinterpret_cast<const int*>(r.ws + pl.cfg_flag_off) : nullptr;
+        u->cfg_stream = r.stream;
     }
     const size_t lo = phase == 2 ? pl.enc_end : 0, hi = phase == 1 ? pl.enc_end : pl.ops.size();
     if (u->graph_mode && !op_ms) {
@@ -520,6 +522,25 @@
     const int old = u->ao.residual_pair;
     if (pair >= 0) u->ao.residual_pair = pair ? 1 : 0;
     return old;
+}
+
+int mve_unet_tune_cfg_prefix(void* handle, int on) {
+    MVE_CHECK(handle, MVE_ERR_ARG, "unet_tune_cfg_prefix: null handle");
+    Unet* u = (Unet*)handle;
+    MVE_CHECK(!u->cfg.controlnet && !u->cfg.vae && !u->cfg.sr && !u->cfg.lpips, MVE_ERR_ARG, "unet_tune_cfg_prefix: a UNet handle is needed");
+    const int old = u->ao.cfg_prefix;
+    if (on >= 0) u->ao.cfg_prefix = on ? 1 : 0;
+    return old;
+}
+
+int mve_unet_cfg_prefix_state(void* handle) {
+    MVE_CHECK(handle, MVE_ERR_STATE, "unet_cfg_prefix_state: null handle");
+    Unet* u = (Unet*)handle;
+    if (!u->cfg_flag) return -1;
+    int v = 0;
+    MVE_HIP(hipStreamSynchronize(u->cfg_stream));
+    MVE_HIP(hipMemcpy(&v, u->cfg_flag, sizeof(int), hipMemcpyDeviceToHost));
+    return v != 0 ? 1 : 0;
 }
 
 int mve_unet_set_addition_embed(void* handle, int addition_type, int addition_time_embed_dim, int projection_input_dim) {
diff --git a/mvedit_amd/unet.py b/mvedit_amd/unet.py
--- a/mvedit_amd/unet.py
+++ b/mvedit_amd/unet.py
@@ -133,6 +133,19 @@
     @property
     def residual_pair(self):
         return bool(_lib.raw('mve_unet_set_residual_mode')(self._h, -1))
+
+    def set_cfg_prefix(self, flag=True):
+        return bool(_lib.raw('mve_unet_tune_cfg_prefix')(self._h, int(bool(flag))))
+
+    @property
+    def cfg_prefix(self):
+        return bool(_lib.raw('mve_unet_tune_cfg_prefix')(self._h, -1))
+
+    def cfg_prefix_state(self):
+        rc = int(_lib.raw('mve_unet_cfg_prefix_state')(self._h))
+        if rc < -1:
+            raise RuntimeError('mve_unet_cfg_prefix_state: ' + _lib.last_error())
+        return rc
 
     def enable_graph(self, flag=True):
         return bool(_lib.raw('mve_unet_graph')(self._h, int(bool(flag))))
```

Measured after the change: 16.88 denoise-steps/s, median of 6. +2.9%, better.
